# pedropro/UrsoNet

Measured on AMD Instinct MI355X. Metric: images/sec fwd+bwd ResNet50 640x512 bs32/GPU, higher is better.
Workload: dtype bf16; 1 GPU; resnet50 bottleneck=32 ori_resolution=16 soft-class head + loc regression, batch 32/GPU x 512x640x3, full training step (prep+fwd+loss+bwd+clip+SGD); global_batch=32, parallelism=dp1, comm_cus=0, hipgraph=True, runner=Engine, input=uint8 frames in HBM, mean subtraction + cast in the step (molding kernel), gradient_norm_from_finalisation_blocks=True, weight_gradients_on_forked_stream=True

## Files before the change

### ursonet_amd/csrc/common.h

```cpp
#pragma once
#include <hip/hip_runtime.h>
#include <stdint.h>
#include <stdio.h>
#include "../../include/ursonet_hip.h"

typedef __attribute__((ext_vector_type(8))) __bf16 bf16x8_t;
typedef __attribute__((ext_vector_type(8))) _Float16 f16x8_t;
typedef __attribute__((ext_vector_type(4))) float f32x4_t;
typedef __attribute__((ext_vector_type(4))) int i32x4_t;
typedef __attribute__((ext_vector_type(2))) int i32x2_t;

void urso_set_error(const char* fmt, ...);
int  urso_check_launch(const char* what);

#define URSO_OPTION_TABLE(X) \
    X(pw_kernel, 3)         \
    X(pw_small, 5)          \
    X(wgrad_narrow, 1)      \
    X(wgrad_blocks, 512)    \
    X(wgrad_pipe, 1)        \
    X(wgrad_big, 1)         \
    X(wgrad_ring, 0)        \
    X(grid_cap, 0)          \
    X(hconv, 1)             \
    X(pair, 1)              \
    X(pair_single, 3)       \
    X(c3, 1)                \
    X(c3v, 1)               \
    X(stem, 1)              \
    X(stem_pool, 1)         \
    X(cus, 0)               \
    X(hconv2, 1)            \
    X(hconv2_shape, 0)      \
    X(hconv_streamk, 1)     \
    X(hconv_dbg, 0)         \
    X(hwgrad, 1)            \
    X(dense, 1)             \
    X(pwx, 1)               \
    X(pwx_dbg, 0)           \
    X(pwx_bn, 0)            \
    X(mold_scalar, 0)       \
    X(bneck, 3)
struct UrsoOptions {
#define URSO_OPT_FIELD(name, dflt) int name = dflt;
    URSO_OPTION_TABLE(URSO_OPT_FIELD)
#undef URSO_OPT_FIELD
};
extern UrsoOptions g_urso_opt;
int urso_device_cus();
int urso_usable_cus();

#define URSO_FUSE_REDUCE_MAX 16
static __host__ __device__ inline bool urso_fuse_reduce(int splits) { return splits > 1 && splits <= URSO_FUSE_REDUCE_MAX; }

#define URSO_REDUCE_COLS 256
static __host__ __device__ inline int urso_reduce_lanes(int splits) { return splits > 384 ? 16 : (splits > 192 ? 8 : (splits > 96 ? 4 : (splits > 48 ? 2 : 1))); }

void urso_prof_before(hipStream_t s, int kernel_id, double flops, double bytes);
void urso_prof_after(hipStream_t s);

void urso_prof_l2(double l2_bytes);
void urso_prof_symbol(const void* host_fn);
#define URSO_KLAUNCH(kern, grid, blk, shm, st, ...) do { urso_prof_symbol((const void*)(kern)); hipLaunchKernelGGL(kern, grid, blk, shm, st, ##__VA_ARGS__); } while (0)

struct ProfScope {
    hipStream_t s;
    ProfScope(hipStream_t st, int id, double flops, double bytes) : s(st) { urso_prof_before(s, id, flops, bytes); }
    ~ProfScope() { urso_prof_after(s); }
};

static inline size_t dt_size(int dt) { return dt == URSO_F32 ? 4 : 2; }
static __host__ __device__ inline int ceil_div(int a, int b) { return (a + b - 1) / b; }

template <typename T> struct Elem;
template <> struct Elem<float> {
    static constexpr int VE = 4;
    static __device__ __forceinline__ float to_f(float v) { return v; }
    static __device__ __forceinline__ float from_f(float v) { return v; }
};
template <> struct Elem<__bf16> {
    static constexpr int VE = 8;
    static constexpr int ONES = 0x3F803F80;
    static __device__ __forceinline__ float to_f(__bf16 v) { return (float)v; }
    static __device__ __forceinline__ __bf16 from_f(float v) { return (__bf16)v; }
};
template <> struct Elem<_Float16> {
    static constexpr int VE = 8;
    static constexpr int ONES = 0x3C003C00;
    static __device__ __forceinline__ float to_f(_Float16 v) { return (float)v; }
    static __device__ __forceinline__ _Float16 from_f(float v) { return (_Float16)v; }
};

template <typename T> struct Mma;
template <> struct Mma<__bf16> {
// ... 80 lines not shown
```

### ursonet_amd/csrc/conv_c3.hip

```cpp
#include "lds_mfma.h"
#include "internal.h"
#include <utility>

struct C3Args {
    const void* src; const void* wgt; const float* bias; const void* mask; void* dst;
    uint32_t bytes;
    int B, H, W, tiles_x, tiles_y, ntiles;
    int relu;
};

constexpr int C3_TH = 4, C3_TW = 32, C3_HW = C3_TW + 2, C3_HROWS = (C3_TH + 2) * C3_HW;
constexpr int C3_NA = 7;
constexpr int C3_ABUF = 224 * 128, C3_OOFF = 2 * C3_ABUF, C3_BOFF = C3_OOFF + C3_TH * C3_TW * 128, C3_LDS = C3_BOFF + 256;

__device__ __forceinline__ uint32_t c3_rd(int row, int h, int j) {
    const int s = (row >> 1) & 7;
    return (uint32_t)(row * 128 + ((((2 * j + h) ^ s)) << 4));
}

template <typename T, bool MASK>
__global__ __launch_bounds__(256, 2) void c3_kernel(const C3Args a) {
    static_assert(sizeof(T) == 2, "16-bit element types only");
    __shared__ __attribute__((aligned(1024))) char smem[C3_LDS];
    const uint32_t lds0 = (uint32_t)(uintptr_t)(__attribute__((address_space(3))) char*)smem;
    const int tid = threadIdx.x, lane = tid & 63, wave = __builtin_amdgcn_readfirstlane(tid >> 6);
    const int cw = wave & 1, pw = wave >> 1;
    int l31 = lane & 31;
    const int h = lane >> 5;

    const UrsoTileStream ts = urso_tile_stream(a.ntiles);
    const int t_end = ts.t_end, bpx = ts.bpx;
    int tile = ts.tile;
    if (tile >= t_end) return;

    const i32x4_t rs = raw_rsrc(a.src, a.bytes);
    const __amdgpu_buffer_rsrc_t rds = make_rsrc(a.dst, a.bytes);
    const __amdgpu_buffer_rsrc_t rmk = make_rsrc(MASK ? a.mask : a.dst, MASK ? a.bytes : 0u);

    int lane_d = lane;
    auto tile_origin = [&](int t, int& b, int& y0, int& x0) {
        const int tx = t % a.tiles_x, q = t / a.tiles_x;
        const int ty = q % a.tiles_y;
        b = q / a.tiles_y; y0 = ty * C3_TH; x0 = tx * C3_TW;
    };
    auto dma_tile = [&](int t, int buf) {
        int b, y0, x0;
        tile_origin(t, b, y0, x0);
        const int base = ((b * a.H + y0 - 1) * a.W + x0 - 1) * 128;
        asm volatile("" : "+v"(lane_d));
#pragma unroll
        for (int i = 0; i < C3_NA; ++i) {
            const int hr = 8 * (wave + 4 * i) + (lane_d >> 3);
            const int hy = (hr * 241) >> 13, hx = hr - hy * C3_HW;
            const int y = y0 - 1 + hy, x = x0 - 1 + hx;
            const bool ok = hr < C3_HROWS && y >= 0 && y < a.H && x >= 0 && x < a.W;
            const uint32_t off = (uint32_t)(base + (hy * a.W + hx) * 128 + (((lane_d & 7) ^ ((hx >> 1) & 7)) << 4));
            lds_dma16(rs, lds0 + buf * C3_ABUF + (wave + 4 * i) * 1024, ok ? off : URSO_OOB_SHIFT);
        }
    };

    i32x4_t wfr[9][4];
    {
        const int lg = 16 * ((l31 >> 2) & 1) + 4 * (l31 >> 3) + (l31 & 3);
        const char* wrow = (const char*)a.wgt + (size_t)(32 * cw + lg) * (9 * 64 * 2);
#pragma unroll
        for (int t = 0; t < 9; ++t)
#pragma unroll
            for (int j = 0; j < 4; ++j) wfr[t][j] = *(const i32x4_t*)(wrow + (t * 64 + 16 * j + 8 * h) * 2);
    }
    if (tid < 64) *(float*)(smem + C3_BOFF + tid * 4) = a.bias ? a.bias[tid] : 0.f;

    constexpr int NST = 4;
    uint32_t ea[3];
#pragma unroll
    for (int kx = 0; kx < 3; ++kx) ea[kx] = (uint32_t)(l31 * 128 + ((h ^ (((l31 + kx) >> 1) & 7)) << 4));

    dma_tile(tile, 0);
    int buf = 0;
    bool first = true;
    while (true) {
        const bool has_next = tile + bpx < t_end;
        if (first) wait_vm<0>(); else wait_vm<NST>();
        first = false;
        lds_barrier_asm();
        if (has_next) dma_tile(tile + bpx, buf ^ 1);

        f32x16_t acc[2];
        {
            const f32x4_t* bp = (const f32x4_t*)(smem + C3_BOFF + (32 * cw + 16 * h) * 4);
#pragma unroll
            for (int q = 0; q < 4; ++q) {
                const f32x4_t b4 = bp[q];
#pragma unroll
                for (int r = 0; r < 2; ++r) { acc[r][4 * q] = b4.x; acc[r][4 * q + 1] = b4.y; acc[r][4 * q + 2] = b4.z; acc[r][4 * q + 3] = b4.w; }
            }
        }
        i32x4_t f[4];
        uint32_t eb[3];
#pragma unroll
        for (int kx = 0; kx < 3; ++kx) eb[kx] = ea[kx] + (uint32_t)(buf * C3_ABUF + 2 * pw * C3_HW * 128);
        auto rd = [&](i32x4_t& fs, int s) {
            const int hr = s / 12, kx = (s / 4) % 3, j = s & 3;
            if (j == 0) asm volatile("" : "+v"(eb[kx]));
            fs = *(const i32x4_t*)(smem + (hr * C3_HW + kx) * 128 + (eb[kx] ^ (uint32_t)(j << 5)));
        };
        rd(f[0], 0);
        rd(f[1], 1);
        rd(f[2], 2);
#pragma unroll
        for (int s = 0; s < 48; ++s) {
            if (s + 3 < 48) rd(f[(s + 3) & 3], s + 3);
            __builtin_amdgcn_sched_barrier(0);
            const int hr = s / 12, kx = (s / 4) % 3, j = s & 3;
            if (hr <= 2) Mma32<T>::run(wfr[3 * hr + kx][j], f[s & 3], acc[0]);
            if (hr >= 1) Mma32<T>::run(wfr[3 * (hr - 1) + kx][j], f[s & 3], acc[1]);
            __builtin_amdgcn_sched_barrier(0);
        }

        char* sO = smem + C3_OOFF;
#pragma unroll
        for (int r = 0; r < 2; ++r) {
            const int px = (2 * pw + r) * 32 + l31;
#pragma unroll
            for (int v = 0; v < 2; ++v) {
                T o[8];
#pragma unroll
                for (int e = 0; e < 8; ++e) { float y = acc[r][8 * v + e]; y = a.relu ? fmaxf(y, 0.f) : y; o[e] = Elem<T>::from_f(y); }
                i32x4_t ov; __builtin_memcpy(&ov, o, 16);
                *(i32x4_t*)(sO + px * 128 + (((4 * cw + 2 * h + v) ^ ((px >> 1) & 7)) << 4)) = ov;
            }
        }
        int b, y0, x0;
        tile_origin(tile, b, y0, x0);
        uint32_t so[NST];
        i32x4_t mv[NST];
#pragma unroll
        for (int i = 0; i < NST; ++i) {
            const int row = 8 * (wave + 4 * i) + (lane >> 3);
            const int y = y0 + (row >> 5), x = x0 + (row & 31);
            so[i] = (y < a.H && x < a.W) ? (uint32_t)(((b * a.H + y) * a.W + x) * 128 + (((lane & 7) ^ ((row >> 1) & 7)) << 4)) : URSO_OOB_SHIFT;
            if constexpr (MASK) mv[i] = buf_load16(rmk, so[i]);
        }
        lds_barrier_asm();
#pragma unroll
        for (int i = 0; i < NST; ++i) {
            i32x4_t v = *(const i32x4_t*)(sO + (wave + 4 * i) * 1024 + lane * 16);
            if constexpr (MASK) {
                T x[8], m[8];
                __builtin_memcpy(x, &v, 16); __builtin_memcpy(m, &mv[i], 16);
#pragma unroll
                for (int e = 0; e < 8; ++e) x[e] = Elem<T>::to_f(m[e]) > 0.f ? x[e] : Elem<T>::from_f(0.f);
                __builtin_memcpy(&v, x, 16);
            }
            buf_store16(rds, so[i], v);
        }
        if (!has_next) break;
        tile += bpx; buf ^= 1;
    }
}

constexpr int C3W_PATCH = 2 * C3_ABUF;
constexpr int C3W_EOFF = 2 * C3W_PATCH, C3W_BOFF = C3W_EOFF + 8192, C3W_LDS = C3W_BOFF + 512;
constexpr int C3W_NA = 7;

template <typename T, bool MASK, int TW>
__global__ __launch_bounds__(512, 2) void c3w_kernel(const C3Args a) {
    constexpr int TH = 128 / TW, HW = TW + 2, HROWS = (TH + 2) * HW;
    static_assert(TW == 32 || TW == 16, "tile width");
    static_assert(sizeof(T) == 2, "16-bit element types only");
    __shared__ __attribute__((aligned(1024))) char smem[C3W_LDS];
    const uint32_t lds0 = (uint32_t)(uintptr_t)(__attribute__((address_space(3))) char*)smem;
    const int tid = threadIdx.x, lane = tid & 63, wave = __builtin_amdgcn_readfirstlane(tid >> 6);
    const int fq = wave & 3, ch = wave >> 2;
    int l31 = lane & 31;
    const int h = lane >> 5;

    const UrsoTileStream ts = urso_tile_stream(a.ntiles);
    const int t_end = ts.t_end, bpx = ts.bpx;
    int tile = ts.tile;
    if (tile >= t_end) return;

    const i32x4_t rs = raw_rsrc(a.src, a.bytes);
    const __amdgpu_buffer_rsrc_t rds = make_rsrc(a.dst, a.bytes);
    const __amdgpu_buffer_rsrc_t rmk = make_rsrc(MASK ? a.mask : a.dst, MASK ? a.bytes : 0u);

    int lane_d = lane;
    auto tile_origin = [&](int t, int& b, int& y0, int& x0) {
        const int tx = t % a.tiles_x, q = t / a.tiles_x;
        const int ty = q % a.tiles_y;
        b = q / a.tiles_y; y0 = ty * TH; x0 = tx * TW;
    };
    auto dma_tile = [&](int t, int buf) {
        int b, y0, x0;
        tile_origin(t, b, y0, x0);
        const int base = ((b * a.H + y0 - 1) * a.W + x0 - 1) * 256;
        asm volatile("" : "+v"(lane_d));
#pragma unroll
        for (int i = 0; i < C3W_NA; ++i) {
            const int ii = wave + 8 * i, half = ii >= 26 ? 1 : 0, rb = ii - 26 * half;
            const int hr = 8 * rb + (lane_d >> 3);
            const int hy = TW == 32 ? ((hr * 241) >> 13) : ((hr * 3641) >> 16), hx = hr - hy * HW;
            const int y = y0 - 1 + hy, x = x0 - 1 + hx;
            const bool ok = ii < 52 && hr < HROWS && y >= 0 && y < a.H && x >= 0 && x < a.W;
            const int sw = (hx >> 1) & 7;
            const uint32_t off = (uint32_t)(base + (hy * a.W + hx) * 256 + half * 128 + (((lane_d & 7) ^ sw) << 4));
            if (ii < 54) lds_dma16(rs, lds0 + buf * C3W_PATCH + half * C3_ABUF + rb * 1024, ok ? off : URSO_OOB_SHIFT);
        }
    };

    i32x4_t wfr[9][4];
    {
        const int lg = 16 * ((l31 >> 2) & 1) + 4 * (l31 >> 3) + (l31 & 3);
        const char* wrow = (const char*)a.wgt + (size_t)(32 * fq + lg) * (9 * 128 * 2);
#pragma unroll
        for (int t = 0; t < 9; ++t)
#pragma unroll
            for (int j = 0; j < 4; ++j) wfr[t][j] = *(const i32x4_t*)(wrow + (t * 128 + 64 * ch + 16 * j + 8 * h) * 2);
    }
    if (tid < 128) *(float*)(smem + C3W_BOFF + tid * 4) = a.bias ? a.bias[tid] : 0.f;

    constexpr int NST = 4;
    uint32_t ea[3];
    {
        const int prow = TW == 32 ? l31 : (l31 >> 4) * HW + (l31 & 15);
#pragma unroll
        for (int kx = 0; kx < 3; ++kx) ea[kx] = (uint32_t)(prow * 128 + ((h ^ ((((l31 & (TW - 1)) + kx) >> 1) & 7)) << 4));
    }
    dma_tile(tile, 0);
    int buf = 0;
    bool first = true;
    while (true) {
        const bool has_next = tile + bpx < t_end;
        if (first) wait_vm<0>(); else wait_vm<NST>();
        first = false;
        lds_barrier_asm();
        if (has_next) dma_tile(tile + bpx, buf ^ 1);
        f32x16_t acc[4];
// ... 99 lines not shown
        for (int i = 0; i < NST; ++i) {
            const int p = (wave + 8 * i) * 64 + lane, px = p >> 4;
            const int y = y0 + px / TW, x = x0 + px % TW;
            so[i] = (y < a.H && x < a.W) ? (uint32_t)(((b * a.H + y) * a.W + x) * 256 + (((p & 15) ^ (px & 15)) << 4)) : URSO_OOB_SHIFT;
            if constexpr (MASK) mv[i] = buf_load16(rmk, so[i]);
        }
        lds_barrier_asm();
#pragma unroll
        for (int i = 0; i < NST; ++i) {
            i32x4_t v = *(const i32x4_t*)(sO + (wave + 8 * i) * 1024 + lane * 16);
            if constexpr (MASK) {
                T x[8], m[8];
                __builtin_memcpy(x, &v, 16); __builtin_memcpy(m, &mv[i], 16);
#pragma unroll
                for (int e = 0; e < 8; ++e) x[e] = Elem<T>::to_f(m[e]) > 0.f ? x[e] : Elem<T>::from_f(0.f);
                __builtin_memcpy(&v, x, 16);
            }
            buf_store16(rds, so[i], v);
        }
        if (!has_next) break;
        tile += bpx; buf ^= 1;
    }
}


#ifdef C3V_OLD_SWZ
__device__ __forceinline__ uint32_t c3v_swz(int col) { return (uint32_t)(col & 15); }
#else
__device__ __forceinline__ uint32_t c3v_swz(int col) { return (uint32_t)(0xfe64dcba98643210ull >> (4 * (col & 15))) & 15u; }
#endif
constexpr int C3V_HW = 18, C3V_HPIX = 10 * C3V_HW, C3V_PATCH = C3V_HPIX * 256;
constexpr int C3V_NA = 6;
#ifndef C3V_PF
#define C3V_PF 3
#endif
#ifndef C3V_DBG
#define C3V_DBG 0
#endif
#ifdef C3V_SEQ
__host__ __device__ constexpr int c3v_step(int t) { return t; }
#else
__host__ __device__ constexpr int c3v_step(int t) { return (t >> 1) + (t & 1) * 60; }
#endif
#ifdef C3V_NOSB
#define C3V_SB() do {} while (0)
#else
#define C3V_SB() __builtin_amdgcn_sched_barrier(0)
#endif
constexpr int C3V_OOFF = 2 * C3V_PATCH, C3V_BOFF = C3V_OOFF + 2 * 128 * 256, C3V_LDS = C3V_BOFF + 512;

template <class F, int... I> __device__ __forceinline__ void c3_static_for_impl(F&& f, std::integer_sequence<int, I...>) { (f(std::integral_constant<int, I>{}), ...); }
template <int N, class F> __device__ __forceinline__ void c3_static_for(F&& f) { c3_static_for_impl(static_cast<F&&>(f), std::make_integer_sequence<int, N>{}); }

template <typename T, bool MASK>
__global__ __launch_bounds__(512, 2) void c3v_kernel(const C3Args a) {
    static_assert(sizeof(T) == 2, "16-bit element types only");
    __shared__ __attribute__((aligned(1024))) char smem[C3V_LDS];
    const uint32_t lds0 = (uint32_t)(uintptr_t)(__attribute__((address_space(3))) char*)smem;
    const int tid = threadIdx.x, lane = tid & 63, wave = __builtin_amdgcn_readfirstlane(tid >> 6);
    const int fr = lane & 15, fg = lane >> 4;

    const UrsoTileStream ts = urso_tile_stream(a.ntiles);
    const int t_end = ts.t_end, bpx = ts.bpx;
    int tile = ts.tile;
    if (tile >= t_end) return;

    const i32x4_t rs = raw_rsrc(a.src, a.bytes);
    const __amdgpu_buffer_rsrc_t rds = make_rsrc(a.dst, a.bytes);
    const __amdgpu_buffer_rsrc_t rmk = make_rsrc(MASK ? a.mask : a.dst, MASK ? a.bytes : 0u);

    int lane_d = lane;
    auto tile_origin = [&](int t, int& b, int& y0, int& x0) {
        const int tx = t % a.tiles_x, q = t / a.tiles_x;
        const int ty = q % a.tiles_y;
        b = q / a.tiles_y; y0 = ty * 8; x0 = tx * 16;
    };
    auto dma_tile = [&](int t, int buf) {
        int b, y0, x0;
        tile_origin(t, b, y0, x0);
        const int base = ((b * a.H + y0 - 1) * a.W + x0 - 1) * 256;
        asm volatile("" : "+v"(lane_d));
#pragma unroll
        for (int i = 0; i < C3V_NA; ++i) {
            const int ii = wave + 8 * i;
            const int hp = 4 * ii + (lane_d >> 4);
            const int hy = (hp * 3641) >> 16, hx = hp - hy * C3V_HW;
            const int y = y0 - 1 + hy, x = x0 - 1 + hx;
            const bool ok = ii < 45 && y >= 0 && y < a.H && x >= 0 && x < a.W;
            const uint32_t off = (uint32_t)(base + (hy * a.W + hx) * 256 + (((uint32_t)(lane_d & 15) ^ c3v_swz(hx)) << 4));
            if (ii < 45) lds_dma16(rs, lds0 + buf * C3V_PATCH + ii * 1024, ok ? off : URSO_OOB_SHIFT);
        }
    };

    i32x4_t wfr[9][4];
    {
        const char* wrow = (const char*)a.wgt + (size_t)(16 * wave + fr) * (9 * 128 * 2);
#pragma unroll
        for (int t = 0; t < 9; ++t)
#pragma unroll
            for (int j = 0; j < 4; ++j) wfr[t][j] = *(const i32x4_t*)(wrow + (t * 128 + 32 * j + 8 * fg) * 2);
    }
    if (tid < 128) *(float*)(smem + C3V_BOFF + tid * 4) = a.bias ? a.bias[tid] : 0.f;

    uint32_t ea[3];
#pragma unroll
    for (int kx = 0; kx < 3; ++kx) ea[kx] = (uint32_t)((fr + kx) * 256) + (((uint32_t)fg ^ c3v_swz(fr + kx)) << 4);
    constexpr int NST = 4;
    uint32_t so[NST] = {URSO_OOB_SHIFT, URSO_OOB_SHIFT, URSO_OOB_SHIFT, URSO_OOB_SHIFT};
    i32x4_t mv[NST];
    auto flush = [&](int ob) {
        const char* sO = smem + C3V_OOFF + ob * (128 * 256);
#pragma unroll
        for (int i = 0; i < NST; ++i) {
            i32x4_t v = *(const i32x4_t*)(sO + (wave + 8 * i) * 1024 + lane * 16);
            if constexpr (MASK) {
                T x[8], m[8];
                __builtin_memcpy(x, &v, 16); __builtin_memcpy(m, &mv[i], 16);
#pragma unroll
                for (int e = 0; e < 8; ++e) x[e] = Elem<T>::to_f(m[e]) > 0.f ? x[e] : Elem<T>::from_f(0.f);
                __builtin_memcpy(&v, x, 16);
            }
            buf_store16(rds, so[i], v);
        }
    };
    dma_tile(tile, 0);
    int buf = 0, ob = 0;
    bool pend = false;
    while (true) {
        const bool has_next = tile + bpx < t_end;
        wait_vm<0>();
        lds_barrier_asm();
        if (has_next) dma_tile(tile + bpx, buf ^ 1);
        if (pend) flush(ob ^ 1);
        f32x4_t acc[8];
#pragma unroll
        for (int r = 0; r < 8; ++r) acc[r] = f32x4_t{0.f, 0.f, 0.f, 0.f};
        uint32_t eb[3];
#pragma unroll
        for (int kx = 0; kx < 3; ++kx) eb[kx] = ea[kx] + (uint32_t)(buf * C3V_PATCH);
        constexpr int PF = C3V_PF, RING = PF + 1;
        i32x4_t f[RING];
        auto rd = [&](i32x4_t& fs, int s) {
            const int hr = s / 12, kx = (s / 4) % 3, j = s & 3;
            if ((s & 3) == 0) asm volatile("" : "+v"(eb[kx]));
            if (!(C3V_DBG & 2) || s < PF) fs = *(const i32x4_t*)(smem + hr * C3V_HW * 256 + (eb[kx] ^ (uint32_t)(j << 6)));
        };
#pragma unroll
        for (int t = 0; t < PF; ++t) rd(f[t], c3v_step(t));
        c3_static_for<120>([&](auto sc) {
            constexpr int t = decltype(sc)::value, s = c3v_step(t);
            if constexpr (t + PF < 120) rd(f[(t + PF) % RING], c3v_step(t + PF));
            C3V_SB();
            constexpr int hr = s / 12, kx = (s / 4) % 3, j = s & 3;
            if (!(C3V_DBG & 1)) {
                if constexpr (hr >= 0 && hr < 8) Mma<T>::run(wfr[kx][j], f[t % RING], acc[hr]);
                if constexpr (hr - 1 >= 0 && hr - 1 < 8) Mma<T>::run(wfr[3 + kx][j], f[t % RING], acc[hr - 1]);
                if constexpr (hr - 2 >= 0 && hr - 2 < 8) Mma<T>::run(wfr[6 + kx][j], f[t % RING], acc[hr - 2]);
            }
            C3V_SB();
        });
        if (C3V_DBG & 4) { if (!has_next) break; tile += bpx; buf ^= 1; continue; }

        {
            char* sO = smem + C3V_OOFF + ob * (128 * 256);
            const f32x4_t bq = *(const f32x4_t*)(smem + C3V_BOFF + (16 * wave + 4 * fg) * 4);
#pragma unroll
            for (int r = 0; r < 8; ++r) {
                const int px = 16 * r + fr;
                float y0v = acc[r].x + bq.x, y1v = acc[r].y + bq.y, y2v = acc[r].z + bq.z, y3v = acc[r].w + bq.w;
                if (a.relu) { y0v = fmaxf(y0v, 0.f); y1v = fmaxf(y1v, 0.f); y2v = fmaxf(y2v, 0.f); y3v = fmaxf(y3v, 0.f); }
                T o[4] = {Elem<T>::from_f(y0v), Elem<T>::from_f(y1v), Elem<T>::from_f(y2v), Elem<T>::from_f(y3v)};
                i32x2_t ov; __builtin_memcpy(&ov, o, 8);
                *(i32x2_t*)(sO + px * 256 + ((((2 * wave + (fg >> 1)) ^ (px & 15))) << 4) + (fg & 1) * 8) = ov;
            }
        }
        {
            int b, y0, x0;
            tile_origin(tile, b, y0, x0);
#pragma unroll
            for (int i = 0; i < NST; ++i) {
                const int p = (wave + 8 * i) * 64 + lane, px = p >> 4;
                const int y = y0 + (px >> 4), x = x0 + (px & 15);
                so[i] = (y < a.H && x < a.W) ? (uint32_t)(((b * a.H + y) * a.W + x) * 256 + (((p & 15) ^ (px & 15)) << 4)) : URSO_OOB_SHIFT;
                if constexpr (MASK) mv[i] = buf_load16(rmk, so[i]);
            }
        }
        pend = true;
        if (!has_next) break;
        tile += bpx; buf ^= 1; ob ^= 1;
    }
    if constexpr (MASK) wait_vm<0>();
    lds_barrier_asm();
    flush(ob);
}

static int c3w_util(int H, int W, int tw) {
    const int th = 128 / tw;
    return (int)((long long)H * W * 100 / ((long long)ceil_div(H, th) * th * ceil_div(W, tw) * tw));
}
static int c3w_best_tw(int H, int W) { return c3w_util(H, W, 16) > c3w_util(H, W, 32) ? 16 : 32; }

bool urso_c3_fits(const urso_conv_geom* g, int dt, int flags, const void* add) {
    if (!g_urso_opt.c3 || add || (dt != URSO_BF16 && dt != URSO_F16) || (flags & (URSO_EPI_OUT_F32 | URSO_EPI_MASK_BITS | URSO_EPI_EMIT_BITS))) return false;
    if (g->KH != 3 || g->KW != 3 || g->SH != 1 || g->SW != 1 || g->PH != 1 || g->PW != 1 || g->DH != 1 || g->DW != 1 || g->FH > 0) return false;
    if (!((g->C == 64 && g->N == 64) || (g->C == 128 && g->N == 128 && (g_urso_opt.c3 == 1 || g_urso_opt.c3 == 3))) || g->OH != g->H || g->OW != g->W) return false;
    if (g->C == 128 && g_urso_opt.c3 == 1) {
        if (c3w_util(g->H, g->W, c3w_best_tw(g->H, g->W)) < 88) return false;
    }
    return (long long)g->B * g->H * g->W * g->C * 2 < 0x7FFFFF00ll;
}

int urso_c3_launch(const urso_conv_geom* g, int dt, int relu, const void* src, const void* wgt, const float* bias, const void* mask,
                   void* dst, hipStream_t st) {
    C3Args a;
    a.src = src; a.wgt = wgt; a.bias = bias; a.mask = mask; a.dst = dst; a.relu = relu;
    a.B = g->B; a.H = g->H; a.W = g->W;
    a.bytes = (uint32_t)((size_t)g->B * g->H * g->W * g->C * 2);
    const bool wide = g->C == 128;
    const int tw = wide ? c3w_best_tw(g->H, g->W) : C3_TW, th = 128 / tw;
    a.tiles_x = ceil_div(g->W, tw); a.tiles_y = ceil_div(g->H, th); a.ntiles = g->B * a.tiles_y * a.tiles_x;
    const dim3 grid(urso_persistent_grid(a.ntiles, wide ? 1 : 2)), blk(wide ? 512 : 256);
    if (wide) {
#define URSO_C3W(TT, TWV) do { if (mask) URSO_KLAUNCH((c3w_kernel<TT, true, TWV>), grid, blk, 0, st, a); \
                               else URSO_KLAUNCH((c3w_kernel<TT, false, TWV>), grid, blk, 0, st, a); } while (0)
        if (tw == 16 && g_urso_opt.c3v) {
            if (dt == URSO_BF16) { if (mask) URSO_KLAUNCH((c3v_kernel<__bf16, true>), grid, blk, 0, st, a); else URSO_KLAUNCH((c3v_kernel<__bf16, false>), grid, blk, 0, st, a); }
            else { if (mask) URSO_KLAUNCH((c3v_kernel<_Float16, true>), grid, blk, 0, st, a); else URSO_KLAUNCH((c3v_kernel<_Float16, false>), grid, blk, 0, st, a); }
            return urso_check_launch("urso_conv_igemm(3x3, 128 channels, 16-filter waves)");
        }
        if (dt == URSO_BF16) { if (tw == 32) URSO_C3W(__bf16, 32); else URSO_C3W(__bf16, 16); }
        else { if (tw == 32) URSO_C3W(_Float16, 32); else URSO_C3W(_Float16, 16); }
#undef URSO_C3W
        return urso_check_launch("urso_conv_igemm(3x3, 128 channels)");
    }
    if (dt == URSO_BF16) {
        if (mask) URSO_KLAUNCH((c3_kernel<__bf16, true>), grid, blk, 0, st, a);
        else URSO_KLAUNCH((c3_kernel<__bf16, false>), grid, blk, 0, st, a);
    } else {
        if (mask) URSO_KLAUNCH((c3_kernel<_Float16, true>), grid, blk, 0, st, a);
        else URSO_KLAUNCH((c3_kernel<_Float16, false>), grid, blk, 0, st, a);
    }
    return urso_check_launch("urso_conv_igemm(3x3, 64 channels)");
}
```

### ursonet_amd/csrc/conv_halo.hip

```cpp
#include "lds_mfma.h"
#include "internal.h"

struct HcArgs {
    const void* src; const void* wgt; const float* bias; const void* add; const void* mask; void* dst;
    uint32_t src_bytes, wgt_bytes, dst_bytes;
    int H, W, C, N;
    int Vw, Vh, Mv;
    int nchunks;
    int tilesN, ntiles;
    int R, JA;
    int krow;
    float rcp_vw, rcp_vh;
    int relu;
    int dbg;
    int units;
    unsigned int* flags;
    float* part;
};

constexpr int HC_BM = 256, HC_BN = 128, HC_BSLOT = HC_BN * 128, HC_AROWS = 424, HC_ABUF = HC_AROWS * 128;
constexpr int HC_AOFF = 3 * HC_BSLOT, HC_XOFF = HC_AOFF + 2 * HC_ABUF, HC_LDS = 163840, HC_MAXN = (HC_LDS - HC_XOFF) / 4;
constexpr int HC_SC = 17;
constexpr int HC_NST = 8;

// ... 251 lines not shown
                        *(i32x4_t*)(smem + sbase + l31 * 128 + (((4 * j + 2 * hf + h) ^ ((l31 >> 1) & 7)) << 4)) = ov;
                    }
                i32x4_t ov[4], mv[4];
                uint32_t so[4];
#pragma unroll
                for (int q = 0; q < 4; ++q) {
                    const int row = 8 * q + r8;
                    ov[q] = *(const i32x4_t*)(smem + sbase + row * 128 + ((c8 ^ ((row >> 1) & 7)) << 4));
                    const bool ok = vb * a.Vh * a.Vw + vy * a.Vw + vx < a.Mv && vx < a.W && vy < a.H;
                    so[q] = ok ? (uint32_t)((vb * a.H + vy) * a.W + vx) * (uint32_t)a.N * 2u + (uint32_t)(n0 + 64 * wn + 8 * c8) * 2u : URSO_OOB_SHIFT;
                    if (a.mask) mv[q] = buf_load16(rmk, so[q]);
                    vx += 8;
                    if (vx >= a.Vw) { vx -= a.Vw; if (++vy == a.Vh) { vy = 0; ++vb; } }
                }
#pragma unroll
                for (int q = 0; q < 4; ++q) {
                    if (a.mask) {
                        T ev[8], em[8];
                        __builtin_memcpy(ev, &ov[q], 16); __builtin_memcpy(em, &mv[q], 16);
#pragma unroll
                        for (int e = 0; e < 8; ++e) ev[e] = (Elem<T>::to_f(em[e]) > 0.f) ? ev[e] : Elem<T>::from_f(0.f);
                        __builtin_memcpy(&ov[q], ev, 16);
                    }
                    buf_store16(rds, so[q], ov[q]);
                }
            }
        }
        if (!has_next) break;
        gcur += cend - cbeg;
        ++tile;
    }
}

bool urso_hconv_fits(const urso_conv_geom* g, int dt, int flags, const void* add) {
    if (!g_urso_opt.hconv || dt == URSO_F32 || add) return false;
    if (flags & (URSO_EPI_OUT_F32 | URSO_EPI_MASK_BITS | URSO_EPI_EMIT_BITS)) return false;
    if (g->KH != 3 || g->KW != 3 || g->SH != 1 || g->SW != 1 || g->PH != 1 || g->PW != 1 || g->DH != 1 || g->DW != 1) return false;
    if (g->OH != g->H || g->OW != g->W || g->FH > 0) return false;
    if (g->C % 128 || g->N % HC_BN || g->N > HC_MAXN) return false;
    if (HC_BM + 2 * (g->W + 2) > HC_AROWS || g->W + 1 < 8) return false;
    if ((size_t)g->B * (g->H + 1) * (g->W + 1) >= (1u << 24)) return false;
    if (urso_hconv2_pick(g, true)) return true;
    if (g_urso_opt.hconv == 1) {
        const int ntiles = ceil_div(g->B * (g->H + 1) * (g->W + 1), HC_BM) * (g->N / HC_BN), ncu = urso_usable_cus();
        const int blocks = ntiles < ncu ? ntiles : ncu, rounds = ceil_div(ntiles, blocks);
        if (ntiles * 20 < blocks * rounds * 13 && !(ntiles <= ncu && ntiles * 3 >= ncu * 2)) return false;
    }
    return true;
}

size_t urso_hconv_ws_bytes() { return 4096 + (size_t)urso_device_cus() * 512 * 64 * sizeof(float); }

int urso_hconv_launch(const urso_conv_geom* g, int dt, int relu, const void* src, const void* wgt, const float* bias, const void* add,
                      const void* mask, void* dst, uint32_t src_bytes, uint32_t wgt_bytes, uint32_t dst_bytes, void* ws, size_t ws_bytes,
                      hipStream_t st) {
    (void)add;
    {
        const int r2 = urso_hconv2_try_launch(g, dt, relu, src, wgt, bias, mask, dst, src_bytes, wgt_bytes, dst_bytes, ws,
                                              ws && ws_bytes >= urso_hconv_ws_bytes(), st);
        if (r2 != 0) return r2 > 0 ? URSO_OK : r2;
    }
    HcArgs a;
    a.src = src; a.wgt = wgt; a.bias = bias; a.add = add; a.mask = mask; a.dst = dst;
    a.src_bytes = src_bytes; a.wgt_bytes = wgt_bytes; a.dst_bytes = dst_bytes;
    a.H = g->H; a.W = g->W; a.C = g->C; a.N = g->N;
    a.Vw = g->W + 1; a.Vh = g->H + 1; a.Mv = g->B * a.Vh * a.Vw;
    a.nchunks = g->C / 64;
    a.tilesN = g->N / HC_BN; a.ntiles = ceil_div(a.Mv, HC_BM) * a.tilesN;
    a.R = HC_BM + 2 * (a.Vw + 1); a.JA = ceil_div(a.R, 64);
    a.krow = 9 * g->C * 2;
    a.rcp_vw = 1.0f / (float)a.Vw; a.rcp_vh = 1.0f / (float)a.Vh;
    a.relu = relu; a.dbg = g_urso_opt.hconv_dbg;
    dim3 grid(urso_persistent_grid(a.ntiles, 1)); const dim3 blk(512);
    int G = (int)grid.x;
    if (ws && ws_bytes >= urso_hconv_ws_bytes() && !(a.dbg & 4) && g_urso_opt.hconv_streamk && g_urso_opt.grid_cap <= 0 && G < urso_usable_cus()) {
        int G2 = urso_usable_cus(); const int units = a.ntiles * a.nchunks;
        if (G2 > units) G2 = units;
        G2 = G2 / 8 * 8;
        if (G2 > G && G2 <= 1024 && ceil_div(units, G2) < ceil_div(a.ntiles, G) * a.nchunks) { G = G2; grid = dim3(G2); }
    }
    const bool can = ws && ws_bytes >= urso_hconv_ws_bytes() && G <= urso_usable_cus() && G <= 1024 && !(a.dbg & 4) && g_urso_opt.hconv_streamk;
    const bool streamk = can && ((a.dbg & 8) || ceil_div(a.ntiles * a.nchunks, G) < ceil_div(a.ntiles, G) * a.nchunks);
    a.flags = streamk ? (unsigned int*)ws : nullptr;
    a.part = streamk ? (float*)((char*)ws + 4096) : nullptr;
    a.units = streamk ? a.ntiles * a.nchunks : a.ntiles;
    urso_prof_l2((double)a.ntiles * a.nchunks * (9.0 * HC_BSLOT + (double)a.R * 128));
    if (a.dbg & 16) {
        if (dt == URSO_BF16) URSO_KLAUNCH((hconv_kernel<__bf16, 4>), grid, blk, 0, st, a);
        else URSO_KLAUNCH((hconv_kernel<_Float16, 4>), grid, blk, 0, st, a);
    } else {
        if (dt == URSO_BF16) URSO_KLAUNCH((hconv_kernel<__bf16, 8>), grid, blk, 0, st, a);
        else URSO_KLAUNCH((hconv_kernel<_Float16, 8>), grid, blk, 0, st, a);
    }
    return urso_check_launch("urso_conv_igemm(halo)");
}
```

### ursonet_amd/csrc/conv_halo2.hip

```cpp
#include "lds_mfma.h"
#include "internal.h"
#include <type_traits>
#ifndef URSO_HX2_NS1
#define URSO_HX2_NS1 4
#endif

struct Hx2Args {
    const void* src; const void* wgt; const float* bias; const void* mask; void* dst;
    uint32_t src_bytes, wgt_bytes, dst_bytes;
    int H, W, C, N;
    int Vw, Vh, Mv;
    int nchunks;
    int tilesN, ntiles;
    int R, JA;
    int abuf;
    int krow;
    float rcp_vw, rcp_vh;
    int relu;
    unsigned long long* clk;
    int dbg;
};

constexpr int HX_LDS = 163840;
constexpr int HX_ABUF1 = 61440, HX_FOFF = 2 * HX_ABUF1;

template <typename T, int MI, int NJ, int PROBE = 0>
__global__ __launch_bounds__(512, 2) void hconv2_kernel(const Hx2Args a) {
    static_assert(sizeof(T) == 2, "16-bit element types only");
#ifndef URSO_HX2_NS1
#define URSO_HX2_NS1 4
#endif
    constexpr int NS = (NJ == 1) ? URSO_HX2_NS1 : 2;
    constexpr int BM = 128 * MI, BN = 64 * NJ, BSLOT = BN * 128, XOFF = HX_FOFF + NS * BSLOT;
    constexpr int NQ = NJ;
    constexpr int LPR = 4 * NJ, RPI = 64 / LPR, NSI = 32 / RPI;
    constexpr int NST = MI * NSI;
    __shared__ __attribute__((aligned(1024))) char smem[HX_LDS];
    const uint32_t lds0 = (uint32_t)(uintptr_t)(__attribute__((address_space(3))) char*)smem;


    const int tid = threadIdx.x, lane = tid & 63, wave = __builtin_amdgcn_readfirstlane(tid >> 6);
    const int wm = wave & 3, wn = wave >> 2;
    const int l31 = lane & 31, h = lane >> 5, c8 = lane & 7, r8 = lane >> 3;

    const int G = gridDim.x, lid = (blockIdx.x & 7) * (G >> 3) + (blockIdx.x >> 3);
    const int t_begin = (int)(((long long)lid * a.ntiles) / G), t_end = (int)(((long long)(lid + 1) * a.ntiles) / G);
    if (t_begin >= t_end || (a.dbg & 1024)) return;

    const i32x4_t rs = raw_rsrc(a.src, a.src_bytes), rw = raw_rsrc(a.wgt, a.wgt_bytes);
    const __amdgpu_buffer_rsrc_t rmk = make_rsrc(a.mask ? a.mask : a.dst, a.mask ? a.dst_bytes : 0u);
    const __amdgpu_buffer_rsrc_t rds = make_rsrc(a.dst, a.dst_bytes);

    if (tid * 4 < a.N) {
        f32x4_t b = f32x4_t{0.f, 0.f, 0.f, 0.f};
        if (a.bias) b = *(const f32x4_t*)(a.bias + tid * 4);
        *(f32x4_t*)(smem + XOFF + tid * 16) = b;
    }

    uint32_t fb, pb[9];
    fb = HX_FOFF + halo_rd(32 * NJ * wn + l31, h);
#pragma unroll
    for (int t = 0; t < 9; ++t) pb[t] = halo_rd(32 * MI * wm + l31 + (t / 3) * a.Vw + (t % 3), h);

    uint32_t bsrc0[NQ];
#pragma unroll
    for (int q = 0; q < NQ; ++q) {
        const int Rr = 8 * (wave + 8 * q) + r8;
        const int nl = (Rr & ~31) + halo_perm(Rr & 31);
        bsrc0[q] = (uint32_t)nl * (uint32_t)a.krow + (uint32_t)((c8 ^ ((Rr >> 1) & 7)) << 4);
    }

    auto divmod = [](int n, int d, float rcp, int& q, int& r) {
        q = (int)((float)n * rcp);
        r = n - q * d;
        const bool lo = r < 0, hi = r >= d;
        q += hi ? 1 : (lo ? -1 : 0);
        r += hi ? -d : (lo ? d : 0);
    };
    auto real_pixel = [&](int p) -> int {
        const bool in = p >= 0 && p < a.Mv;
        int q1, x, b, y;
        divmod(in ? p : 0, a.Vw, a.rcp_vw, q1, x);
        divmod(q1, a.Vh, a.rcp_vh, b, y);
        return (in && x < a.W && y < a.H) ? (b * a.H + y) * a.W + x : -1;
    };

    const uint32_t TOFF = XOFF + (uint32_t)a.N * 4u;
    auto fill_table = [&](int tile_, int which) {
        const int p0_ = (tile_ / a.tilesN) * BM;
        const int pix = (tid < a.R) ? real_pixel(p0_ - (a.Vw + 1) + tid) : -1;
        *(uint32_t*)(smem + TOFF + which * 2048 + tid * 4) = (pix >= 0) ? (uint32_t)pix * (uint32_t)(a.C * 2) : URSO_OOB_SHIFT;
    };
    const uint32_t aswz = (uint32_t)((c8 ^ ((4 * wave + (r8 >> 1)) & 7)) << 4);
    auto table_entry = [&](int which, int j) -> uint32_t {
        return *(const uint32_t*)(smem + TOFF + which * 2048 + (8 * (wave + 8 * j) + r8) * 4);
    };
    auto dma_a = [&](int j, int cc, int buf, uint32_t rowoff) {
        if (8 * (wave + 8 * j) < a.R)
            lds_dma16_sgpr(rs, lds0 + buf * HX_ABUF1 + (wave + 8 * j) * 1024, rowoff + aswz + (uint32_t)cc * 128u);
    };
    auto dma_b = [&](int n0_, int cc, int t, int slot) {
        const uint32_t koff = (uint32_t)n0_ * (uint32_t)a.krow + (uint32_t)(t * a.C + cc * 64) * 2u;
#pragma unroll
// ... 90 lines not shown
                if constexpr (NS == 2) {
                    if (t == 0 && first_wait_after_epilogue) asm volatile("s_waitcnt vmcnt(%0) lgkmcnt(0)" :: "n"(NST) : "memory");
                    else asm volatile("s_waitcnt vmcnt(0) lgkmcnt(0)" ::: "memory");
                } else {
                    static_assert(NQ == 1, "the four-slot ring is the NJ = 1 form");
                    if (t < 3 && first_wait_after_epilogue) asm volatile("s_waitcnt vmcnt(%0) lgkmcnt(0)" :: "n"(NST + 2) : "memory");
                    else if (t >= 6 && !more_a) { if (t == 6) asm volatile("s_waitcnt vmcnt(1) lgkmcnt(0)" ::: "memory"); else asm volatile("s_waitcnt vmcnt(0) lgkmcnt(0)" ::: "memory"); }
                    else asm volatile("s_waitcnt vmcnt(2) lgkmcnt(0)" ::: "memory");
                }
                if (!(a.dbg & 64)) asm volatile("s_barrier" ::: "memory");
                if (!(a.dbg & 32)) {
                    if constexpr (NS == 2) {
                        if (t < 8 && t < a.JA && more_a) dma_a(t, cca, par ^ 1, acur0);
                        if (t < 7) acur0 = table_entry(tw, t + 1);
                    } else {
                        if (t < 6 && more_a) {
                            const int j0 = piece(t, 0), j1 = piece(t, 1);
                            if (j0 < a.JA) dma_a(j0, cca, par ^ 1, acur0);
                            if (j1 < a.JA) dma_a(j1, cca, par ^ 1, acur1);
                        }
                        if (t < 5) { acur0 = table_entry(tw, min(piece(t + 1, 0), 7)); acur1 = table_entry(tw, min(piece(t + 1, 1), 7)); }
                    }
                    const int t2 = (t + NS) % 9;
                    const bool wrap = t + NS >= 9;
                    const bool okb = !wrap || more_a;
                    if (okb) dma_b((wrap && last) ? n0n : n0, wrap ? cca : cc, t2, (S + sb) & (NS - 1));
                }
                __builtin_amdgcn_sched_barrier(0);
                if (t < 8) rd(fwA, fpA, S1, par, t + 1, 0);
                else rd(fwA, fpA, S1, par ^ 1, 0, 0);
                region_end(); mma(fwB, fpB); region_end();
            }
        };
        if (!(a.dbg & 2))
            for (int cc = 0; cc < a.nchunks; cc += 2) {
                chunk(std::integral_constant<int, 0>{}, cc);
                chunk(std::integral_constant<int, 1>{}, cc + 1);
                if constexpr (NS == 4) { sb ^= 2; set_fbs(); }
            }

        stores_pending = false;
        if (!(a.dbg & 1)) {
            stores_pending = true;
            int lane_e = lane;
            asm volatile("" : "+v"(lane_e));
            const int cl = lane_e % LPR, rl = lane_e / LPR, l31e = lane_e & 31, he = lane_e >> 5;
            const uint32_t sbase = HX_ABUF1 + wave * (32 * 64 * NJ);
            int vx, vy, vb;
            {
                int q1;
                divmod(p0 + 32 * MI * wm + rl, a.Vw, a.rcp_vw, q1, vx);
                divmod(q1, a.Vh, a.rcp_vh, vb, vy);
            }
#pragma unroll
            for (int i = 0; i < MI; ++i) {
#pragma unroll
                for (int j = 0; j < NJ; ++j)
#pragma unroll
                    for (int hf = 0; hf < 2; ++hf) {
                        const int nb = n0 + 32 * NJ * wn + 32 * j + 16 * hf + 8 * he;
                        const f32x4_t b0 = *(const f32x4_t*)(smem + XOFF + nb * 4), b1 = *(const f32x4_t*)(smem + XOFF + nb * 4 + 16);
                        const float bv[8] = {b0.x, b0.y, b0.z, b0.w, b1.x, b1.y, b1.z, b1.w};
                        T eo[8];
#pragma unroll
                        for (int e = 0; e < 8; ++e) {
                            float y = acc[i][j][8 * hf + e] + bv[e];
                            y = a.relu ? fmaxf(y, 0.f) : y;
                            eo[e] = Elem<T>::from_f(y);
                        }
                        i32x4_t ov; __builtin_memcpy(&ov, eo, 16);
                        *(i32x4_t*)(smem + sbase + l31e * (64 * NJ) + (((4 * j + 2 * hf + he) ^ ((l31e >> 1) & (LPR - 1))) << 4)) = ov;
                    }
                i32x4_t ov[NSI], mv[NSI];
                uint32_t so[NSI];
#pragma unroll
                for (int q = 0; q < NSI; ++q) {
                    const int row = RPI * q + rl;
                    ov[q] = *(const i32x4_t*)(smem + sbase + row * (64 * NJ) + ((cl ^ ((row >> 1) & (LPR - 1))) << 4));
                    const bool ok = vb * a.Vh * a.Vw + vy * a.Vw + vx < a.Mv && vx < a.W && vy < a.H;
                    so[q] = ok ? (uint32_t)((vb * a.H + vy) * a.W + vx) * (uint32_t)a.N * 2u + (uint32_t)(n0 + 32 * NJ * wn + 8 * cl) * 2u : URSO_OOB_SHIFT;
                    if (a.mask) mv[q] = buf_load16(rmk, so[q]);
                    vx += RPI;
                    if (vx >= a.Vw) { vx -= a.Vw; if (++vy == a.Vh) { vy = 0; ++vb; } }
                }
#pragma unroll
                for (int q = 0; q < NSI; ++q) {
                    if (a.mask) {
                        T ev[8], em[8];
                        __builtin_memcpy(ev, &ov[q], 16); __builtin_memcpy(em, &mv[q], 16);
#pragma unroll
                        for (int e = 0; e < 8; ++e) ev[e] = (Elem<T>::to_f(em[e]) > 0.f) ? ev[e] : Elem<T>::from_f(0.f);
                        __builtin_memcpy(&ov[q], ev, 16);
                    }
                    buf_store16(rds, so[q], ov[q]);
                }
            }
        }
        if (!has_next) break;
        ++tile;
    }
    if (a.clk && tid == 0) {
        a.clk[2 * lid] = __builtin_readcyclecounter() - clk0;
        a.clk[2 * lid + 1] = __builtin_amdgcn_s_memrealtime() - rt0;
    }
}

struct Hx2Shape { int mi, nj; };
static const Hx2Shape HX2_SHAPES[] = {{3, 2}, {3, 1}, {2, 2}, {2, 1}, {1, 2}, {1, 1}};

static size_t hx2_abuf(int R, int nj) { const size_t a = (size_t)ceil_div(R, 8) * 1024, e = (size_t)8 * 32 * 64 * nj; return a > e ? a : e; }

static bool hx2_shape_fits(const urso_conv_geom* g, int mi, int nj) {
    const int BM = 128 * mi, BN = 64 * nj, Vw = g->W + 1;
    if (g->N % BN) return false;
    const int R = BM + 2 * (Vw + 1), JA = ceil_div(R, 64);
    if (JA > 8) return false;
    if (Vw < 64 / (4 * nj)) return false;
    if (hx2_abuf(R, nj) > (size_t)HX_ABUF1) return false;
    if (R > 512) return false;
    return (size_t)HX_FOFF + (size_t)(nj == 1 ? URSO_HX2_NS1 : 2) * BN * 128 + (size_t)g->N * 4 + 2 * 2048 <= (size_t)HX_LDS;
}

static double hx2_cost(const urso_conv_geom* g, int mi, int nj, int ncu) {
    const int Mv = g->B * (g->H + 1) * (g->W + 1);
    const int tiles = ceil_div(Mv, 128 * mi) * (g->N / (64 * nj));
    const int blocks = tiles < ncu ? tiles : ncu, rounds = ceil_div(tiles, blocks);
    const double kib = (128.0 * nj * 64.0 + (128.0 * mi + 2.0 * (g->W + 2)) * 128.0 / 9.0) / 1024.0;
    const double step = (0.037 * 4.0 * mi * nj + 0.07 + 0.003 * kib) * (0.7 + 0.3 * (double)blocks / ncu);
    return 9.0 + rounds * (g->C / 64) * 9.0 * step + (rounds - 1) * 3.0;
}
static double hx2_cost_halo1(const urso_conv_geom* g, int ncu, bool streamk) {
    const int Mv = g->B * (g->H + 1) * (g->W + 1), tiles = ceil_div(Mv, 256) * (g->N / 128), nch = g->C / 64;
    const int blocks = tiles < ncu ? tiles : ncu;
    double c = 14.0 + ceil_div(tiles, blocks) * nch * 9.0 * 0.75;
    if (streamk) { const double sk = 20.0 + ceil_div(tiles * nch, ncu) * 9.0 * 0.75; if (sk < c) c = sk; }
    return c;
}

int urso_hconv2_pick(const urso_conv_geom* g, bool has_ws) {
    if (!g_urso_opt.hconv2 || g->C % 128) return 0;
    const int ncu = urso_usable_cus();
    int best = -1; double best_cost = 1e30;
    for (int s = 0; s < (int)(sizeof(HX2_SHAPES) / sizeof(HX2_SHAPES[0])); ++s) {
        const int mi = HX2_SHAPES[s].mi, nj = HX2_SHAPES[s].nj;
        if (g_urso_opt.hconv2_shape && g_urso_opt.hconv2_shape != 10 * mi + nj) continue;
        if (!hx2_shape_fits(g, mi, nj)) continue;
        const double c = hx2_cost(g, mi, nj, ncu);
        if (c < best_cost) { best_cost = c; best = s; }
    }
    if (best < 0) return 0;
    if (g_urso_opt.hconv2 == 1 && !g_urso_opt.hconv2_shape && best_cost >= hx2_cost_halo1(g, ncu, has_ws && g_urso_opt.hconv_streamk)) return 0;
    return 10 * HX2_SHAPES[best].mi + HX2_SHAPES[best].nj;
}

int urso_hconv2_try_launch(const urso_conv_geom* g, int dt, int relu, const void* src, const void* wgt, const float* bias, const void* mask,
                           void* dst, uint32_t src_bytes, uint32_t wgt_bytes, uint32_t dst_bytes, void* ws, bool has_ws, hipStream_t st) {
    const int shape = urso_hconv2_pick(g, has_ws);
    if (!shape) return 0;
    const int mi = shape / 10, nj = shape % 10;
    Hx2Args a;
    a.src = src; a.wgt = wgt; a.bias = bias; a.mask = mask; a.dst = dst;
    a.src_bytes = src_bytes; a.wgt_bytes = wgt_bytes; a.dst_bytes = dst_bytes;
    a.H = g->H; a.W = g->W; a.C = g->C; a.N = g->N;
    a.Vw = g->W + 1; a.Vh = g->H + 1; a.Mv = g->B * a.Vh * a.Vw;
    a.nchunks = g->C / 64;
    a.tilesN = g->N / (64 * nj); a.ntiles = ceil_div(a.Mv, 128 * mi) * a.tilesN;
    a.R = 128 * mi + 2 * (a.Vw + 1); a.JA = ceil_div(a.R, 64); a.abuf = (int)hx2_abuf(a.R, nj);
    a.krow = 9 * g->C * 2;
    a.rcp_vw = 1.0f / (float)a.Vw; a.rcp_vh = 1.0f / (float)a.Vh;
    a.relu = relu; a.dbg = g_urso_opt.hconv_dbg;
    a.clk = (ws && has_ws && (a.dbg & 2048)) ? (unsigned long long*)((char*)ws + 8192) : nullptr;
    const dim3 grid(urso_persistent_grid(a.ntiles, 1)), blk(512);
    urso_prof_l2((double)a.ntiles * a.nchunks * (9.0 * 64 * nj * 128 + (double)a.R * 128));
#define HX2_GO(MI_, NJ_) do { if (dt == URSO_BF16) URSO_KLAUNCH((hconv2_kernel<__bf16, MI_, NJ_>), grid, blk, 0, st, a); \
                              else URSO_KLAUNCH((hconv2_kernel<_Float16, MI_, NJ_>), grid, blk, 0, st, a); } while (0)
    if (10 * mi + nj == 32 && dt == URSO_BF16 && (a.dbg & 384)) {
        if (a.dbg & 128) URSO_KLAUNCH((hconv2_kernel<__bf16, 3, 2, 1>), grid, blk, 0, st, a);
        else URSO_KLAUNCH((hconv2_kernel<__bf16, 3, 2, 2>), grid, blk, 0, st, a);
        return urso_check_launch("urso_conv_igemm(halo2 probe)") == URSO_OK ? 1 : URSO_EINVAL;
    }
    switch (10 * mi + nj) {
        case 32: HX2_GO(3, 2); break; case 31: HX2_GO(3, 1); break;
        case 22: HX2_GO(2, 2); break; case 21: HX2_GO(2, 1); break;
        case 12: HX2_GO(1, 2); break; case 11: HX2_GO(1, 1); break;
        default: return 0;
    }
#undef HX2_GO
    const int rc = urso_check_launch("urso_conv_igemm(halo2)");
    return rc == URSO_OK ? 1 : rc;
}
```

### ursonet_amd/csrc/conv_igemm.hip

```cpp
#include "common.h"
#include "internal.h"
#include <stdlib.h>

struct IgemmArgs {
    const void* src; const void* wgt; const float* bias; const void* add; const void* mask; void* dst;
    uint32_t src_bytes, wgt_bytes, dst_bytes;
    int B, H, W, C, OH, OW, N, KH, KW, SH, SW, PH, PW, DHs, DWs;
    int M;
    int Cc;
    int Kc;
    int nkt;
    int tilesN, ntiles;
    int pointwise;
    int FH, FW, OSH, OSW;
    int ksplit, kps;
    float* part;
    int flags;
    void* bits_out;
    uint32_t bits_bytes;
};

template <typename T, int BM, int BN, bool HAS_ADD, int MASK, bool SPLIT, bool EMIT = false>
__global__ __launch_bounds__(256, 2) void igemm_kernel(const IgemmArgs a) {
    constexpr bool HAS_MASK = MASK == 1;
// ... 357 lines not shown
        case 4: if constexpr (sizeof(T) == 2) URSO_IG(BN_, false, 2, false, false); break; \
        case 5: if constexpr (sizeof(T) == 2) URSO_IG(BN_, true, 2, false, false); break; \
        case 8: if constexpr (sizeof(T) == 2) URSO_IG(BN_, false, 0, false, true); break; \
        case 9: if constexpr (sizeof(T) == 2) URSO_IG(BN_, true, 0, false, true); break; \
        default: urso_set_error("urso_conv_igemm: unsupported epilogue combination"); return URSO_EINVAL; }
    if (a.ksplit > 1) { if (small) URSO_IG(64, false, 0, true, false); else URSO_IG(128, false, 0, true, false); }
    else if (small) { URSO_SEL(64) }
    else { URSO_SEL(128) }
#undef URSO_SEL
#undef URSO_IG
    if (a.ksplit > 1) {
        const size_t elems = (size_t)a.M * g->N, n4 = elems / 4;
        int blocks = (int)((n4 + 255) / 256); if (blocks > 2048) blocks = 2048; if (blocks < 1) blocks = 1;
        URSO_KLAUNCH((splitk_finish_kernel<T>), dim3(blocks), dim3(256), 0, st, n4, g->N, a.ksplit, elems, (const float*)a.part, a.bias,
                           (const T*)a.add, (const T*)a.mask, a.dst, flags);
    }
    return urso_check_launch("urso_conv_igemm");
}

extern "C" int urso_conv_igemm_halo_ok(const urso_conv_geom* g, int dt, int flags, int has_add) {
    return (g && urso_hconv_fits(g, dt, flags, has_add ? (const void*)g : nullptr)) ? 1 : 0;
}

extern "C" size_t urso_conv_igemm_halo_ws_bytes(void) { return urso_hconv_ws_bytes(); }

extern "C" int urso_conv_igemm_halo2_shape(const urso_conv_geom* g, int dt, int flags, int has_add, int has_ws) {
    if (!g || !urso_hconv_fits(g, dt, flags, has_add ? (const void*)g : nullptr)) return 0;
    return urso_hconv2_pick(g, has_ws != 0);
}

extern "C" size_t urso_conv_igemm_ws_bytes(const urso_conv_geom* g, int dt) {
    if (!g || g->FH > 0 || (g->N & 3)) return 0;
    const int VE = 16 / (int)dt_size(dt);
    if (g->C % VE) return 0;
    const int M = g->B * g->OH * g->OW, nkt = ceil_div(g->KH * g->KW * (g->C / VE), 8);
    const int bn = (g->N <= 64) ? 64 : 128;
    int S, kps; plan_splitk(ceil_div(M, 128) * ceil_div(g->N, bn), nkt, urso_usable_cus(), S, kps);
    return S > 1 ? (size_t)S * M * g->N * sizeof(float) : 0;
}

extern "C" int urso_conv_igemm(const urso_conv_geom* g, int dt, int flags,
                               const void* src_d, const void* wgt_d, const float* bias_d,
                               const void* add_d, const void* mask_d, void* dst_d, void* stream) {
    return urso_conv_igemm_ws(g, dt, flags, src_d, wgt_d, bias_d, add_d, mask_d, dst_d, nullptr, 0, stream);
}

extern "C" int urso_conv_igemm_ws(const urso_conv_geom* g, int dt, int flags,
                                  const void* src_d, const void* wgt_d, const float* bias_d,
                                  const void* add_d, const void* mask_d, void* dst_d, void* ws_d, size_t ws_bytes, void* stream) {
    return urso_conv_igemm_ex(g, dt, flags & ~(URSO_EPI_MASK_BITS | URSO_EPI_EMIT_BITS), src_d, wgt_d, bias_d, add_d, mask_d, dst_d, nullptr,
                              ws_d, ws_bytes, stream);
}

extern "C" int urso_conv_igemm_bits_ok(const urso_conv_geom* g, int dt, int flags, size_t ws_bytes) {
    if (!g || dt == URSO_F32 || (flags & URSO_EPI_OUT_F32) || (g->N % 8) || (g->C % 8)) return 0;
    if (ws_bytes && urso_conv_igemm_ws_bytes(g, dt)) return 0;
    return 1;
}

extern "C" int urso_conv_igemm_algorithmic(const urso_conv_geom* g, int dt, int flags, int has_add, int has_mask, double* flops_out, double* bytes_out) {
    if (!g || (dt != URSO_F32 && dt != URSO_BF16 && dt != URSO_F16)) { urso_set_error("urso_conv_igemm_algorithmic: bad argument"); return URSO_EINVAL; }
    const double es = (double)dt_size(dt);
    const double M = (double)g->B * g->OH * g->OW;
    double flops = 2.0 * M * (double)g->N * g->KH * g->KW * g->C;
    if (g->DH > 1 || g->DW > 1) flops /= (double)(g->DH * g->DW);
    if (g->C == 8 && g->KH == 7 && g->KW == 4 && g->SH == 2) flops *= 147.0 / 224.0;
    const double src_bytes = (double)g->B * g->H * g->W * g->C * es, wgt_bytes = (double)g->N * g->KH * g->KW * g->C * es;
    const double src_alg = (g->KH == 1 && g->KW == 1 && (g->SH > 1 || g->SW > 1)) ? M * g->C * es : src_bytes;
    const double wr_elems = M * g->N;
    const double bytes = src_alg + wgt_bytes + wr_elems * ((flags & URSO_EPI_OUT_F32) ? 4 : es) +
                         (has_add ? wr_elems * es : 0) + (has_mask ? ((flags & URSO_EPI_MASK_BITS) ? wr_elems / 8 : wr_elems * es) : 0) +
                         ((flags & URSO_EPI_EMIT_BITS) ? wr_elems / 8 : 0);
    if (flops_out) *flops_out = flops;
    if (bytes_out) *bytes_out = bytes;
    return URSO_OK;
}

extern "C" int urso_conv_igemm_ex(const urso_conv_geom* g, int dt, int flags,
                                  const void* src_d, const void* wgt_d, const float* bias_d,
                                  const void* add_d, const void* mask_d, void* dst_d, void* bits_out_d,
                                  void* ws_d, size_t ws_bytes, void* stream) {
    if (!g || !src_d || !wgt_d || !dst_d) { urso_set_error("urso_conv_igemm: null argument"); return URSO_EINVAL; }
    if (dt != URSO_F32 && dt != URSO_BF16 && dt != URSO_F16) { urso_set_error("urso_conv_igemm: bad dtype %d", dt); return URSO_EINVAL; }
    const size_t es = dt_size(dt);
    const int VE = 16 / (int)es;
    if (g->B <= 0 || g->H <= 0 || g->W <= 0 || g->C <= 0 || g->OH <= 0 || g->OW <= 0 || g->N <= 0 || g->KH <= 0 || g->KW <= 0 ||
        g->SH <= 0 || g->SW <= 0) { urso_set_error("urso_conv_igemm: non-positive dimension"); return URSO_EINVAL; }
    if (g->C % VE) { urso_set_error("urso_conv_igemm: C=%d is not a multiple of %d (16-byte vectors)", g->C, VE); return URSO_EINVAL; }
    int dhs = ilog2_exact(g->DH), dws = ilog2_exact(g->DW);
    if (dhs < 0 || dws < 0) { urso_set_error("urso_conv_igemm: D must be 1, 2 or 4"); return URSO_EINVAL; }
    const size_t src_bytes = (size_t)g->B * g->H * g->W * g->C * es;
    const size_t wgt_bytes = (size_t)g->N * g->KH * g->KW * g->C * es;
    const bool scatter = g->FH > 0;
    if (scatter && (g->FW <= 0 || g->OSH <= 0 || g->OSW <= 0 || (g->OH - 1) * g->OSH >= g->FH || (g->OW - 1) * g->OSW >= g->FW)) {
        urso_set_error("urso_conv_igemm: bad destination scatter"); return URSO_EINVAL; }
    const size_t dst_elems = scatter ? (size_t)g->B * g->FH * g->FW * g->N : (size_t)g->B * g->OH * g->OW * g->N;
    if (src_bytes >= 0x7FFFFF00ull || wgt_bytes >= 0x7FFFFF00ull || dst_elems * ((flags & URSO_EPI_OUT_F32) ? 4 : es) >= 0x7FFFFF00ull) {
        urso_set_error("urso_conv_igemm: tensor exceeds the 2 GiB buffer-addressing limit"); return URSO_EINVAL; }
    IgemmArgs a;
    a.src = src_d; a.wgt = wgt_d; a.bias = bias_d; a.add = add_d; a.mask = mask_d; a.dst = dst_d;
    a.src_bytes = (uint32_t)src_bytes; a.wgt_bytes = (uint32_t)wgt_bytes;
    a.dst_bytes = (uint32_t)(dst_elems * ((flags & URSO_EPI_OUT_F32) ? 4 : es));
    a.B = g->B; a.H = g->H; a.W = g->W; a.C = g->C; a.OH = g->OH; a.OW = g->OW; a.N = g->N;
    a.KH = g->KH; a.KW = g->KW; a.SH = g->SH; a.SW = g->SW; a.PH = g->PH; a.PW = g->PW; a.DHs = dhs; a.DWs = dws;
    a.M = g->B * g->OH * g->OW; a.Cc = g->C / VE; a.Kc = g->KH * g->KW * a.Cc; a.nkt = ceil_div(a.Kc, 8);
    a.flags = flags;
    a.bits_out = bits_out_d; a.bits_bytes = (uint32_t)(dst_elems / 8);
    a.FH = scatter ? g->FH : 0; a.FW = g->FW; a.OSH = g->OSH; a.OSW = g->OSW;
    a.pointwise = (g->KH == 1 && g->KW == 1 && g->SH == 1 && g->SW == 1 && g->PH == 0 && g->PW == 0 && g->DH == 1 && g->DW == 1 &&
                   g->H == g->OH && g->W == g->OW) ? 1 : 0;
    hipStream_t st = (hipStream_t)stream;
    double flops, bytes;
    urso_conv_igemm_algorithmic(g, dt, flags, add_d ? 1 : 0, mask_d ? 1 : 0, &flops, &bytes);
    ProfScope ps(st, URSO_K_IGEMM, flops, bytes);
    if (urso_dense_fits(g, dt, flags, a.pointwise, a.M))
        return urso_dense_launch(g, dt, flags, src_d, wgt_d, bias_d, add_d, mask_d, dst_d, a.src_bytes, a.wgt_bytes, a.dst_bytes, st);
    if (urso_bneck_fwd_fits(g, dt, flags, add_d, mask_d))
        return urso_bneck_fwd_launch(g, dt, flags, src_d, wgt_d, bias_d, dst_d, st);
    if (urso_bneck_dgrad_fits(g, dt, flags, add_d, mask_d))
        return urso_bneck_dgrad_launch(g, dt, flags, src_d, wgt_d, mask_d, dst_d, st);
    {
        const int use_pw = g_urso_opt.pw_kernel;
        const bool halo_layer = dt != URSO_F32 && urso_hconv_fits(g, dt, flags, add_d);
        const bool split = ws_d && !halo_layer && urso_conv_igemm_ws_bytes(g, dt) != 0 && urso_conv_igemm_ws_bytes(g, dt) <= ws_bytes;
        const bool wants_bits = (flags & (URSO_EPI_MASK_BITS | URSO_EPI_EMIT_BITS)) != 0;
        const bool s1x1 = g->KH == 1 && g->KW == 1 && g->PH == 0 && g->PW == 0 && g->DH == 1 && g->DW == 1 && g->FH <= 0;
        const bool add_src = (flags & URSO_EPI_ADD_SRCGRID) != 0;
        if (add_src && (!add_d || !s1x1 || dt == URSO_F32 || mask_d || (flags & (URSO_EPI_OUT_F32 | URSO_EPI_MASK_BITS)) || (a.Cc & 7) || (g->N % 8) ||
                        (g->OH - 1) * g->SH >= g->H || (g->OW - 1) * g->SW >= g->W || use_pw < 2 || (size_t)g->B * g->H * g->W * g->N * es >= 0x7FFFFF00ull)) {
            urso_set_error("urso_conv_igemm: ADD_SRCGRID needs a 16-bit unpadded 1x1 layer with C %% 64 == 0, a residual operand on the input grid and no mask");
            return URSO_EINVAL;
        }
        const bool bits_fit = !wants_bits || ((a.pointwise || (s1x1 && !(flags & URSO_EPI_MASK_BITS) && (a.Cc & 7) == 0)) && !((flags & URSO_EPI_EMIT_BITS) && (mask_d || (g->N % 32))) &&
                                              !((flags & URSO_EPI_MASK_BITS) && (!mask_d || (g->N % 32))) && !((flags & URSO_EPI_EMIT_BITS) && !bits_out_d));
        const bool fits = dt != URSO_F32 && !(flags & URSO_EPI_OUT_F32) && bits_fit && (g->N % 8) == 0 &&
                          !split && (size_t)a.M < (1u << 24);
        if (fits && urso_pair_single_fits(g, dt, flags, add_d, mask_d))
            return urso_pair_single_launch(g, dt, flags, src_d, wgt_d, bias_d, add_d, mask_d, dst_d,
                                           (flags & URSO_EPI_EMIT_BITS) ? bits_out_d : nullptr, st);
        if (fits && urso_c3_fits(g, dt, flags, add_d))
            return urso_c3_launch(g, dt, (flags & URSO_EPI_RELU) ? 1 : 0, src_d, wgt_d, bias_d, mask_d, dst_d, st);
        if (fits && urso_hconv_fits(g, dt, flags, add_d))
            return urso_hconv_launch(g, dt, (flags & URSO_EPI_RELU) ? 1 : 0, src_d, wgt_d, bias_d, add_d, mask_d, dst_d,
                                     a.src_bytes, a.wgt_bytes, a.dst_bytes, ws_d, ws_bytes, st);
        const int mbits = (flags & URSO_EPI_MASK_BITS) ? 1 : 0;
        void* bout = (flags & URSO_EPI_EMIT_BITS) ? bits_out_d : nullptr;
        const bool taps_ok = (a.Cc & 7) == 0 && g->DH == 1 && g->DW == 1 && g->KH <= 3 && g->KW <= 3;
        const bool stem_ok = a.Cc == 1 && g->KW == 4 && g->KH <= 8 && g->DH == 1 && g->DW == 1 && g->N <= 64 && !add_d && !mask_d;
        if (fits && !wants_bits && urso_stem_fits(g, dt, flags, add_d, mask_d))
            return urso_stem_launch(g, dt, (flags & URSO_EPI_RELU) ? 1 : 0, src_d, wgt_d, bias_d, dst_d, st);
        if (fits && !wants_bits && use_pw >= 3 && stem_ok)
            return urso_pw_launch(g, dt, 2, dhs, dws, (flags & URSO_EPI_RELU) ? 1 : 0,
                                  src_d, wgt_d, bias_d, add_d, mask_d, dst_d, a.src_bytes, a.wgt_bytes, a.dst_bytes, 0, nullptr, 0, st);
        if (add_src && !fits) { urso_set_error("urso_conv_igemm: ADD_SRCGRID layer does not fit the DMA kernel (split-K workspace given, M >= 2^24 ...)"); return URSO_EINVAL; }
        if (fits && ((use_pw >= 1 && a.pointwise && (a.Cc & 7) == 0) || (use_pw >= 2 && taps_ok && (!wants_bits || s1x1))))
            return urso_pw_launch(g, dt, a.pointwise ? 0 : 1, dhs, dws, (flags & URSO_EPI_RELU) ? 1 : 0,
                                  src_d, wgt_d, bias_d, add_d, mask_d, dst_d, a.src_bytes, a.wgt_bytes, a.dst_bytes, mbits, bout, add_src, st);
    }
    if (dt == URSO_F32) return launch_igemm<float>(g, flags, a, ws_d, ws_bytes, st);
    if (dt == URSO_BF16) return launch_igemm<__bf16>(g, flags, a, ws_d, ws_bytes, st);
    return launch_igemm<_Float16>(g, flags, a, ws_d, ws_bytes, st);
}
```

### ursonet_amd/csrc/conv_pair.hip

```cpp
#include "lds_mfma.h"
#include "internal.h"

struct PairArgs {
    const void* src; const void* w1; const float* bias1; const void* add; void* bits; void* mid;
    const void* w2; const float* bias2; const void* mask2; void* dst;
    uint32_t nar_bytes, wide_bytes, bits_bytes;
    int ntiles;
    int relu1;
    int sp_h, sp_w; uint32_t add_bytes; float rcp_hw, rcp_w;
    void* cmp; uint32_t cmp_bytes;
    uint32_t wide_pitch, bits_pitch, g_w1, g_bias, g_wide, g_bits;
};

template <int CM_, int NW_, int BM_, int NBUF_, int CW_ = 4 * CM_> struct PairShape {
    static constexpr int CM = CM_, CW = CW_, NW = NW_, BM = BM_, NBUF = NBUF_, D = NBUF_ - 1;
    static constexpr int AROW = CM * 2, RROW = CW * 2, BROW = CW / 8;
    static constexpr int ABUF = BM * AROW, RBUF = BM * RROW, ROFF = NBUF * ABUF, LDS = NBUF * (ABUF + RBUF);
    static constexpr int NA = ABUF / (1024 * NW), NR = RBUF / (1024 * NW);
    static constexpr int PT1 = BM / 32, KS1 = CM / 16, PT2 = BM / 16, KS2 = CW / 32;
    static constexpr int C2T = CW / (32 * NW);
    static_assert((C2T == 1 || C2T == 2) && CW == 32 * C2T * NW && NA >= 1 && NR >= 1 && PT1 >= 1, "wave roles");
    static __device__ __forceinline__ int aswz(int row) { return AROW == 128 ? ((row >> 1) & 7) : (row & 15); }
};
using PairS2 = PairShape<64, 4, 64, 2>;
using PairS3 = PairShape<128, 8, 32, 3>;
using PairS4 = PairShape<256, 8, 32, 3, 512>;
using PairS5 = PairShape<512, 8, 32, 3, 256>;

#ifndef PAIR_DBG
#define PAIR_DBG 0
#endif
template <typename T, int MODE, bool EMIT, typename S, int VAR, bool SPARSE = false>
__global__ __launch_bounds__(S::NW * 64, 2) void pair_kernel(const PairArgs a) {
    static_assert(!SPARSE || (MODE == 1 && VAR == 0) || (MODE == 0 && VAR != 0), "SPARSE: compact add operand of the backward pair, or sampled second output of a single forward layer");
    constexpr bool SPADD = SPARSE && MODE == 1, CMPW = SPARSE && MODE == 0;
    static_assert(sizeof(T) == 2, "16-bit element types only");
    constexpr bool G2 = VAR == 0, HAS_ADD = VAR != 2;
    static_assert(!G2 || (S::CM / S::NW == 16 && S::CW == 4 * S::CM), "pair: every wave owns 16 of the CM output channels of GEMM 2");
    static_assert(VAR != 2 || MODE == 0, "the form without a residual operand is forward-only");
    constexpr int BM = S::BM, CM = S::CM, CW = S::CW, NW = S::NW, AROW = S::AROW, RROW = S::RROW, BROW = S::BROW;
    constexpr int NA = S::NA, NR = S::NR, PT1 = S::PT1, KS1 = S::KS1, PT2 = S::PT2, KS2 = S::KS2, D = S::D, NBUF = S::NBUF, C2T = S::C2T;
    static_assert(!G2 || C2T == 2, "pair: every wave owns 64 of the wide channels");
    __shared__ __attribute__((aligned(1024))) char smem[S::LDS];
    const uint32_t lds0 = (uint32_t)(uintptr_t)(__attribute__((address_space(3))) char*)smem;
    const int tid = threadIdx.x, lane = tid & 63, wave = __builtin_amdgcn_readfirstlane(tid >> 6);
    const int l31 = lane & 31, h = lane >> 5, l15 = lane & 15, g = lane >> 4;

    const UrsoTileStream ts = urso_tile_stream(a.ntiles);
    const int t_end = ts.t_end, bpx = ts.bpx;
    int tile = ts.tile;
    if (tile >= t_end) return;

    const uint32_t grp = blockIdx.y, gwide = grp * a.g_wide, gbits = grp * a.g_bits;
    const uint32_t pitch = a.wide_pitch, bpitch = a.bits_pitch;
    const i32x4_t rs = raw_rsrc(a.src, a.nar_bytes), ra = raw_rsrc((const char*)a.add + gwide, (SPADD ? a.add_bytes : a.wide_bytes) - gwide);
    const __amdgpu_buffer_rsrc_t rmid = make_rsrc((char*)a.mid + gwide, a.wide_bytes - gwide), rdst = make_rsrc(a.dst, a.nar_bytes);
    const __amdgpu_buffer_rsrc_t rbit = make_rsrc(a.bits ? (char*)a.bits + gbits : (char*)a.mid, a.bits ? a.bits_bytes - gbits : 0u);
    const __amdgpu_buffer_rsrc_t rmk2 = make_rsrc(MODE == 1 ? a.mask2 : a.dst, MODE == 1 ? a.nar_bytes : 0u);

    uint32_t aoff[NA], roff[NR];
#pragma unroll
    for (int i = 0; i < NA; ++i) {
        const int row = (1024 / AROW) * (wave + NW * i) + lane / (AROW / 16), p = lane % (AROW / 16);
        aoff[i] = (uint32_t)(row * AROW + ((p ^ S::aswz(row)) << 4));
    }
#pragma unroll
    for (int i = 0; i < NR; ++i) {
        const int row = (1024 / RROW) * (wave + NW * i) + lane / (RROW / 16), p = lane % (RROW / 16);
        roff[i] = (uint32_t)(row * RROW + ((p ^ (row & 15)) << 4));
    }
    uint32_t rgo[NR];
#pragma unroll
    for (int i = 0; i < NR; ++i) rgo[i] = (roff[i] / (uint32_t)RROW) * pitch + (roff[i] & (uint32_t)(RROW - 1));
    auto dma_tile = [&](int t, int buf) {
        const uint32_t nb = (uint32_t)t * (uint32_t)(BM * AROW), wb = (uint32_t)t * (uint32_t)BM * pitch;
#pragma unroll
        for (int i = 0; i < NA; ++i) lds_dma16(rs, lds0 + buf * S::ABUF + (wave + NW * i) * 1024, nb + aoff[i]);
        if constexpr (HAS_ADD && !SPADD) {
#pragma unroll
            for (int i = 0; i < NR; ++i) lds_dma16(ra, lds0 + S::ROFF + buf * S::RBUF + (wave + NW * i) * 1024, (PAIR_DBG & 4) ? URSO_OOB_SHIFT : wb + rgo[i]);
        }
        if constexpr (SPADD) {
            const int hw = a.sp_h * a.sp_w, w2 = a.sp_w >> 1, hw4 = (a.sp_h >> 1) * w2;
#pragma unroll
            for (int i = 0; i < NR; ++i) {
                const int row = (1024 / RROW) * (wave + NW * i) + lane / (RROW / 16);
                const int p = t * BM + row;
                int b = (int)((float)p * a.rcp_hw), rem = p - b * hw;
                { const bool lo = rem < 0, hi = rem >= hw; b += hi ? 1 : (lo ? -1 : 0); rem += hi ? -hw : (lo ? hw : 0); }
                int y = (int)((float)rem * a.rcp_w), x = rem - y * a.sp_w;
                { const bool lo = x < 0, hi = x >= a.sp_w; y += hi ? 1 : (lo ? -1 : 0); x += hi ? -a.sp_w : (lo ? a.sp_w : 0); }
                const uint32_t off = (uint32_t)((b * hw4 + (y >> 1) * w2 + (x >> 1)) * RROW) + (roff[i] & (uint32_t)(RROW - 1));
                lds_dma16(ra, lds0 + S::ROFF + buf * S::RBUF + (wave + NW * i) * 1024, ((y | x) & 1) ? URSO_OOB_SHIFT : off);
            }
        }
    };
    constexpr int NDMA = NA + (HAS_ADD ? NR : 0);

    i32x4_t w1f[C2T][KS1], w2f[KS2];
    {
        const int lg = 16 * ((l31 >> 2) & 1) + 4 * (l31 >> 3) + (l31 & 3);
#pragma unroll
        for (int c2 = 0; c2 < C2T; ++c2)
#pragma unroll
            for (int j = 0; j < KS1; ++j)
                w1f[c2][j] = *(const i32x4_t*)((const char*)a.w1 + (size_t)grp * a.g_w1 + ((size_t)(32 * C2T * wave + 32 * c2 + lg) * CM + 16 * j + 8 * h) * 2);
        if constexpr (G2) {
#pragma unroll
            for (int j = 0; j < KS2; ++j)
                w2f[j] = *(const i32x4_t*)((const char*)a.w2 + ((size_t)(16 * wave + l15) * CW + 32 * j + 8 * g) * 2);
        }
    }
    float b1[C2T][16], b2[4];
    if constexpr (MODE == 0) {
#pragma unroll
        for (int c2 = 0; c2 < C2T; ++c2)
#pragma unroll
            for (int r = 0; r < 16; ++r) b1[c2][r] = a.bias1 ? a.bias1[grp * a.g_bias + 32 * C2T * wave + 32 * c2 + 16 * h + r] : 0.f;
        if constexpr (G2) {
#pragma unroll
            for (int r = 0; r < 4; ++r) b2[r] = a.bias2 ? a.bias2[16 * wave + 4 * g + r] : 0.f;
        }
    }

    uint32_t g1rd[PT1][2];
#pragma unroll
    for (int pt = 0; pt < PT1; ++pt) {
        const int row = 32 * pt + l31;
        g1rd[pt][0] = (uint32_t)(row * AROW);
        g1rd[pt][1] = (uint32_t)S::aswz(row);
    }
    uint32_t e1[PT1][C2T];
#pragma unroll
    for (int pt = 0; pt < PT1; ++pt)
#pragma unroll
        for (int c2 = 0; c2 < C2T; ++c2)
            e1[pt][c2] = (uint32_t)((32 * pt + l31) * RROW + (((4 * C2T * wave + 4 * c2 + 2 * h) ^ (l31 & 15)) << 4));
    uint32_t g2rd[PT2];
#pragma unroll
    for (int pt = 0; pt < PT2; ++pt) g2rd[pt] = (uint32_t)((16 * pt + l15) * RROW + ((g ^ l15) << 4));
    uint32_t e2[PT2];
#pragma unroll
    for (int pt = 0; pt < PT2; ++pt) {
        const int row = 16 * pt + l15, slot = 2 * wave + (g >> 1);
        e2[pt] = (uint32_t)(row * AROW + ((slot ^ S::aswz(row)) << 4) + 8 * (g & 1));
    }
    const uint32_t bitoff = (uint32_t)l31 * bpitch + 4u * C2T * wave;

    constexpr int NST = NR + (G2 ? NA : 0) + ((MODE == 0 && EMIT) ? PT1 : 0) + (CMPW ? NR : 0);

    i32x2_t pbits[PT1];
    i32x4_t pm2[NA];
    auto prefetch = [&](int t) {
        if constexpr (MODE == 1) {
#pragma unroll
            for (int pt = 0; pt < PT1; ++pt)
            {
                const uint32_t bo = (uint32_t)t * (uint32_t)BM * bpitch + pt * 32u * bpitch + bitoff;
                if constexpr (C2T == 2) pbits[pt] = __builtin_bit_cast(i32x2_t, __builtin_amdgcn_raw_buffer_load_b64(rbit, bo, 0, 0));
                else pbits[pt] = i32x2_t{(int)__builtin_amdgcn_raw_buffer_load_b32(rbit, bo, 0, 0), 0};
            }
            if constexpr (G2) {
#pragma unroll
                for (int i = 0; i < NA; ++i) pm2[i] = buf_load16(rmk2, (uint32_t)t * (uint32_t)(BM * AROW) + aoff[i]);
            }
        }
    };

    prefetch(tile);
    dma_tile(tile, 0);
    if constexpr (D == 2) { if (tile + bpx < t_end) dma_tile(tile + bpx, 1); }
    int buf = 0;
    bool first = true;
    while (true) {
        const bool has_next = tile + bpx < t_end;
        const bool has_far = tile + D * bpx < t_end;
        if constexpr (D == 1) { if (first) wait_vm<0>(); else wait_vm<NST>(); }
        else {
            if (first) { if (has_next) wait_vm<NDMA>(); else wait_vm<0>(); }
            else { if (has_next) wait_vm<NST + NDMA>(); else wait_vm<NST>(); }
        }
        first = false;
        lds_barrier_asm();
        i32x2_t cbits[PT1]; i32x4_t cm2[NA];
        if constexpr (MODE == 1) {
#pragma unroll
            for (int i = 0; i < PT1; ++i) { cbits[i] = pbits[i]; asm volatile("" : "+v"(cbits[i])); }
            if constexpr (G2) {
#pragma unroll
                for (int i = 0; i < NA; ++i) { cm2[i] = pm2[i]; asm volatile("" : "+v"(cm2[i])); }
            }
        }
        if (has_next) prefetch(tile + bpx);
        if (has_far) { int nb_ = buf + D; if (nb_ >= NBUF) nb_ -= NBUF; dma_tile(tile + D * bpx, nb_); }
        const char* sA = smem + buf * S::ABUF;
        char* sR = smem + S::ROFF + buf * S::RBUF;

        f32x16_t acc[PT1][C2T];
#pragma unroll
        for (int pt = 0; pt < PT1; ++pt)
#pragma unroll
            for (int c2 = 0; c2 < C2T; ++c2)
// ... 71 lines not shown
                    { const bool lo = x < 0, hi = x >= a.sp_w; y += hi ? 1 : (lo ? -1 : 0); x += hi ? -a.sp_w : (lo ? a.sp_w : 0); }
                    const uint32_t off = (uint32_t)(b * hw4 + (y >> 1) * w2 + (x >> 1)) * pitch + (roff[i] & (uint32_t)(RROW - 1));
                    buf_store16(rcmp, ((y | x) & 1) ? URSO_OOB_SHIFT : off, v[i]);
                }
            }
        }
        if constexpr (!G2) {
            if (!has_next) break;
            tile += bpx;
            buf = (buf + 1 == NBUF) ? 0 : buf + 1;
            continue;
        }
        f32x4_t acc2[PT2];
#pragma unroll
        for (int pt = 0; pt < PT2; ++pt)
#pragma unroll
            for (int r = 0; r < 4; ++r) acc2[pt][r] = (MODE == 0) ? b2[r] : 0.f;
#pragma unroll
        for (int j = 0; j < KS2; ++j) {
            i32x4_t px[PT2];
#pragma unroll
            for (int pt = 0; pt < PT2; ++pt) px[pt] = *(const i32x4_t*)(sR + (g2rd[pt] ^ (uint32_t)(j << 6)));
#pragma unroll
            for (int pt = 0; pt < PT2; ++pt) Mma<T>::run(w2f[j], px[pt], acc2[pt]);
        }
        char* sO = smem + buf * S::ABUF;
#pragma unroll
        for (int pt = 0; pt < PT2; ++pt) {
            T out[4];
#pragma unroll
            for (int r = 0; r < 4; ++r) {
                float x = acc2[pt][r];
                if constexpr (MODE == 0) x = fmaxf(x, 0.f);
                out[r] = Elem<T>::from_f(x);
            }
            i32x2_t pk;
            __builtin_memcpy(&pk, out, 8);
            *(i32x2_t*)(sO + e2[pt]) = pk;
        }
        lds_barrier_asm();
        {
            const uint32_t nb = (uint32_t)tile * (uint32_t)(BM * AROW);
#pragma unroll
            for (int i = 0; i < NA; ++i) {
                i32x4_t v = *(const i32x4_t*)(sO + (wave + NW * i) * 1024 + lane * 16);
                if constexpr (MODE == 1) {
                    T x[8], m[8];
                    __builtin_memcpy(x, &v, 16); __builtin_memcpy(m, &cm2[i], 16);
#pragma unroll
                    for (int e = 0; e < 8; ++e) x[e] = Elem<T>::to_f(m[e]) > 0.f ? x[e] : Elem<T>::from_f(0.f);
                    __builtin_memcpy(&v, x, 16);
                }
                buf_store16(rdst, nb + aoff[i], v);
            }
        }
        if (!has_next) break;
        tile += bpx;
        buf = (buf + 1 == NBUF) ? 0 : buf + 1;
    }
}

extern "C" int urso_conv_pair_ok(long long M, int dt, int c_narrow, int c_wide) {
    if (M <= 0 || !(dt == URSO_BF16 || dt == URSO_F16) || c_wide != 4 * c_narrow) return 0;
    const int bm = c_narrow == PairS2::CM ? PairS2::BM : (c_narrow == PairS3::CM ? PairS3::BM : 0);
    return (bm && M % bm == 0 && M * c_wide * 2 < 0x7FFFFF00ll) ? 1 : 0;
}

template <typename S, int VAR>
static void pr_launch(const PairArgs& a, int dt, int mode, bool emit, int blocks_per_cu, hipStream_t st, bool sparse = false, int groups = 1) {
    const dim3 grid(urso_persistent_grid(a.ntiles, blocks_per_cu, groups), groups), blk(S::NW * 64);
    if constexpr (VAR == 0) {
        if (sparse && mode == 1) {
            if (dt == URSO_BF16) URSO_KLAUNCH((pair_kernel<__bf16, 1, false, S, 0, true>), grid, blk, 0, st, a);
            else URSO_KLAUNCH((pair_kernel<_Float16, 1, false, S, 0, true>), grid, blk, 0, st, a);
        } else if (dt == URSO_BF16) {
            if (mode == 1) URSO_KLAUNCH((pair_kernel<__bf16, 1, false, S, 0>), grid, blk, 0, st, a);
            else if (emit) URSO_KLAUNCH((pair_kernel<__bf16, 0, true, S, 0>), grid, blk, 0, st, a);
            else URSO_KLAUNCH((pair_kernel<__bf16, 0, false, S, 0>), grid, blk, 0, st, a);
        } else {
            if (mode == 1) URSO_KLAUNCH((pair_kernel<_Float16, 1, false, S, 0>), grid, blk, 0, st, a);
            else if (emit) URSO_KLAUNCH((pair_kernel<_Float16, 0, true, S, 0>), grid, blk, 0, st, a);
            else URSO_KLAUNCH((pair_kernel<_Float16, 0, false, S, 0>), grid, blk, 0, st, a);
        }
    } else {
        if (mode == 1) {
            if constexpr (VAR == 1) {
                if (dt == URSO_BF16) URSO_KLAUNCH((pair_kernel<__bf16, 1, false, S, 1>), grid, blk, 0, st, a);
                else URSO_KLAUNCH((pair_kernel<_Float16, 1, false, S, 1>), grid, blk, 0, st, a);
            }
        } else if (sparse) {
            if (dt == URSO_BF16) { if (emit) URSO_KLAUNCH((pair_kernel<__bf16, 0, true, S, VAR, true>), grid, blk, 0, st, a); else URSO_KLAUNCH((pair_kernel<__bf16, 0, false, S, VAR, true>), grid, blk, 0, st, a); }
            else { if (emit) URSO_KLAUNCH((pair_kernel<_Float16, 0, true, S, VAR, true>), grid, blk, 0, st, a); else URSO_KLAUNCH((pair_kernel<_Float16, 0, false, S, VAR, true>), grid, blk, 0, st, a); }
        } else if (dt == URSO_BF16) {
            if (emit) URSO_KLAUNCH((pair_kernel<__bf16, 0, true, S, VAR>), grid, blk, 0, st, a);
            else URSO_KLAUNCH((pair_kernel<__bf16, 0, false, S, VAR>), grid, blk, 0, st, a);
        } else {
            if (emit) URSO_KLAUNCH((pair_kernel<_Float16, 0, true, S, VAR>), grid, blk, 0, st, a);
            else URSO_KLAUNCH((pair_kernel<_Float16, 0, false, S, VAR>), grid, blk, 0, st, a);
        }
    }
}

bool urso_pair_single_fits(const urso_conv_geom* g, int dt, int flags, const void* add, const void* mask) {
    if (!g_urso_opt.pair || (flags & URSO_EPI_OUT_F32) || (dt != URSO_BF16 && dt != URSO_F16)) return false;
    const bool mbits = (flags & URSO_EPI_MASK_BITS) != 0;
    if (mask && !mbits) return false;
    if (mbits && (!mask || !add || (flags & (URSO_EPI_EMIT_BITS | URSO_EPI_RELU)))) return false;
    if (g->KH != 1 || g->KW != 1 || g->SH != 1 || g->SW != 1 || g->PH || g->PW || g->DH != 1 || g->DW != 1 || g->FH > 0 ||
        g->OH != g->H || g->OW != g->W) return false;
    const long long M = (long long)g->B * g->OH * g->OW;
    if (M <= 0 || M * g->N * 2 >= 0x7FFFFF00ll) return false;
    if (g->C == PairS4::CM) return (g_urso_opt.pair_single & 1) && g->N >= PairS4::CW && g->N % PairS4::CW == 0 && M % PairS4::BM == 0;
    if (g->C == PairS5::CM) return (g_urso_opt.pair_single & 2) && g->N >= PairS5::CW && g->N % PairS5::CW == 0 && M % PairS5::BM == 0;
    if (mbits) return false;
    return g->N == 4 * g->C && urso_conv_pair_ok(M, dt, g->C, g->N) != 0;
}
static int pair_single_launch(const urso_conv_geom* g, int dt, int flags, const void* src, const void* wgt, const float* bias, const void* add,
                              const void* mask_bits, void* dst, void* bits_out, void* dst_sampled, hipStream_t st) {
    const long long M = (long long)g->B * g->OH * g->OW;
    const int cm = g->C, cw = g->N;
    const int mode = (flags & URSO_EPI_MASK_BITS) ? 1 : 0;
    PairArgs a;
    a.src = src; a.w1 = wgt; a.bias1 = bias; a.add = add ? add : dst; a.bits = mode ? const_cast<void*>(mask_bits) : bits_out; a.mid = dst;
    a.w2 = nullptr; a.bias2 = nullptr; a.mask2 = nullptr; a.dst = dst; a.relu1 = (flags & URSO_EPI_RELU) ? 1 : 0;
    a.sp_h = a.sp_w = 0; a.add_bytes = 0; a.rcp_hw = a.rcp_w = 0.f;
    a.nar_bytes = (uint32_t)(M * cm * 2); a.wide_bytes = (uint32_t)(M * cw * 2); a.bits_bytes = (uint32_t)(M * (cw / 8));
    a.wide_pitch = (uint32_t)cw * 2u; a.bits_pitch = (uint32_t)cw / 8u; a.g_w1 = a.g_bias = a.g_wide = a.g_bits = 0;
    const bool emit = !mode && bits_out != nullptr;
    const bool smp = dst_sampled != nullptr;
    a.cmp = dst_sampled; a.cmp_bytes = (uint32_t)(M / 4 * cw * 2);
    if (smp) { a.sp_h = g->OH; a.sp_w = g->OW; a.rcp_hw = 1.0f / (float)(g->OH * g->OW); a.rcp_w = 1.0f / (float)g->OW; }
    if (cm == PairS4::CM) {
        const int groups = cw / PairS4::CW;
        a.g_w1 = (uint32_t)PairS4::CW * cm * 2u; a.g_bias = PairS4::CW; a.g_wide = PairS4::CW * 2u; a.g_bits = PairS4::CW / 8u;
        a.ntiles = (int)(M / PairS4::BM);
        if (add) pr_launch<PairS4, 1>(a, dt, mode, emit, 1, st, smp, groups); else pr_launch<PairS4, 2>(a, dt, 0, emit, 1, st, smp, groups);
    } else if (cm == PairS5::CM) {
        const int groups = cw / PairS5::CW;
        a.g_w1 = (uint32_t)PairS5::CW * cm * 2u; a.g_bias = PairS5::CW; a.g_wide = PairS5::CW * 2u; a.g_bits = PairS5::CW / 8u;
        a.ntiles = (int)(M / PairS5::BM);
        if (add) pr_launch<PairS5, 1>(a, dt, mode, emit, 1, st, smp, groups); else pr_launch<PairS5, 2>(a, dt, 0, emit, 1, st, smp, groups);
    } else if (cm == PairS2::CM) {
        a.ntiles = (int)(M / PairS2::BM);
        if (add) pr_launch<PairS2, 1>(a, dt, 0, emit, 2, st, smp); else pr_launch<PairS2, 2>(a, dt, 0, emit, 2, st, smp);
    } else {
        a.ntiles = (int)(M / PairS3::BM);
        if (add) pr_launch<PairS3, 1>(a, dt, 0, emit, 1, st, smp); else pr_launch<PairS3, 2>(a, dt, 0, emit, 1, st, smp);
    }
    return urso_check_launch("urso_conv_igemm(wide pointwise)");
}
int urso_pair_single_launch(const urso_conv_geom* g, int dt, int flags, const void* src, const void* wgt, const float* bias, const void* add,
                            const void* mask_bits, void* dst, void* bits_out, hipStream_t st) {
    return pair_single_launch(g, dt, flags, src, wgt, bias, add, mask_bits, dst, bits_out, nullptr, st);
}

extern "C" int urso_conv_pointwise_sampled_ok(const urso_conv_geom* g, int dt, int flags, int has_add) {
    if (!g || (flags & URSO_EPI_MASK_BITS) || (g->OH & 1) || (g->OW & 1) || g->C >= PairS5::CM) return 0;
    return urso_pair_single_fits(g, dt, flags, has_add ? (const void*)g : nullptr, nullptr) ? 1 : 0;
}
extern "C" int urso_conv_pointwise_sampled(const urso_conv_geom* g, int dt, int flags, const void* src_d, const void* wgt_d, const float* bias_d,
                                           const void* add_d, void* dst_d, void* bits_out_d, void* dst_sampled_d, void* stream) {
    if (!g || !src_d || !wgt_d || !dst_d || !dst_sampled_d || ((flags & URSO_EPI_EMIT_BITS) && !bits_out_d)) { urso_set_error("urso_conv_pointwise_sampled: null argument"); return URSO_EINVAL; }
    if (!urso_conv_pointwise_sampled_ok(g, dt, flags, add_d != nullptr)) { urso_set_error("urso_conv_pointwise_sampled: the layer does not take the register-filter kernel (urso_conv_pointwise_sampled_ok)"); return URSO_EINVAL; }
    if ((((uintptr_t)src_d) | ((uintptr_t)wgt_d) | ((uintptr_t)add_d) | ((uintptr_t)dst_d) | ((uintptr_t)bits_out_d) | ((uintptr_t)dst_sampled_d)) & 15) {
        urso_set_error("urso_conv_pointwise_sampled: pointers must be 16-byte aligned"); return URSO_EINVAL;
    }
    hipStream_t st = (hipStream_t)stream;
    const double M = (double)g->B * g->OH * g->OW;
    ProfScope ps(st, URSO_K_IGEMM, 2.0 * M * g->C * g->N, M * 2.0 * (g->C + g->N * (add_d ? 2.25 : 1.25)) + ((flags & URSO_EPI_EMIT_BITS) ? M * g->N / 8 : 0.0));
    return pair_single_launch(g, dt, flags, src_d, wgt_d, bias_d, add_d, nullptr, dst_d, (flags & URSO_EPI_EMIT_BITS) ? bits_out_d : nullptr, dst_sampled_d, st);
}

extern "C" int urso_conv_pair(long long M, int c_narrow, int dt, int mode, const void* src_d, const void* w1_d, const float* bias1_d,
                              const void* add_d, void* bits_d, void* mid_d, const void* w2_d, const float* bias2_d, const void* mask2_d,
                              void* dst_d, int add_h, int add_w, void* stream) {
    const int cm = c_narrow, cw = 4 * c_narrow;
    if (!urso_conv_pair_ok(M, dt, cm, cw)) {
        urso_set_error("urso_conv_pair: needs 16-bit dt, (64, 256) channels with M %% 64 == 0 or (128, 512) with M %% 32 == 0, tensors < 2 GiB");
        return URSO_EINVAL;
    }
    if (!src_d || !w1_d || !add_d || !mid_d || !w2_d || !dst_d || (mode != 0 && mode != 1) || (mode == 1 && (!bits_d || !mask2_d))) {
        urso_set_error("urso_conv_pair: bad argument"); return URSO_EINVAL;
    }
    const bool sparse = add_h > 0 || add_w > 0;
    if (sparse && (mode != 1 || add_h <= 0 || add_w <= 0 || (add_h & 1) || (add_w & 1) || M % ((long long)add_h * add_w))) {
        urso_set_error("urso_conv_pair: a compact add operand needs mode 1, even add_h / add_w and M = B * add_h * add_w"); return URSO_EINVAL;
    }
    if ((((uintptr_t)src_d) | ((uintptr_t)w1_d) | ((uintptr_t)add_d) | ((uintptr_t)mid_d) | ((uintptr_t)w2_d) | ((uintptr_t)dst_d) |
         ((uintptr_t)bits_d) | ((uintptr_t)mask2_d)) & 15) { urso_set_error("urso_conv_pair: pointers must be 16-byte aligned"); return URSO_EINVAL; }
    hipStream_t st = (hipStream_t)stream;
    PairArgs a;
    a.src = src_d; a.w1 = w1_d; a.bias1 = bias1_d; a.add = add_d; a.bits = bits_d; a.mid = mid_d; a.w2 = w2_d; a.bias2 = bias2_d;
    a.mask2 = mask2_d; a.dst = dst_d; a.relu1 = 1;
    a.sp_h = add_h; a.sp_w = add_w; a.add_bytes = (uint32_t)(M / 4 * cw * 2);
    a.wide_pitch = (uint32_t)cw * 2u; a.bits_pitch = (uint32_t)cw / 8u; a.g_w1 = a.g_bias = a.g_wide = a.g_bits = 0;
    a.rcp_hw = sparse ? 1.0f / (float)(add_h * add_w) : 0.f; a.rcp_w = sparse ? 1.0f / (float)add_w : 0.f;
    a.nar_bytes = (uint32_t)(M * cm * 2); a.wide_bytes = (uint32_t)(M * cw * 2); a.bits_bytes = (uint32_t)(M * (cw / 8));
    const double flops = 2.0 * (double)M * cm * cw * 2.0;
    const double bytes = (double)M * (2.0 * cm * 2 + (sparse ? 1.25 : 2.0) * cw * 2) + (double)M * (cw / 8) * ((mode == 1 || bits_d) ? 1 : 0) +
                         (mode == 1 ? (double)M * cm * 2 : 0.0) + 2.0 * cm * cw * 2;
    ProfScope ps(st, URSO_K_IGEMM, flops, bytes);
    if (cm == PairS2::CM) { a.ntiles = (int)(M / PairS2::BM); pr_launch<PairS2, 0>(a, dt, mode, bits_d != nullptr, 2, st, sparse); }
    else { a.ntiles = (int)(M / PairS3::BM); pr_launch<PairS3, 0>(a, dt, mode, bits_d != nullptr, 1, st, sparse); }
    return urso_check_launch("urso_conv_pair");
}
```

### ursonet_amd/csrc/conv_pwx.hip

```cpp
#include "lds_mfma.h"
#include "internal.h"
#include <string.h>

struct PxArgs {
    const void* src; const void* wgt; const float* bias; const void* add; const void* mask; void* dst; void* bits_out;
    uint32_t src_bytes, wgt_bytes, dst_bytes;
    int M, C, N, Kc, nkt, tilesN, ntiles;
    int OH, OW, FH, FW, OSH, OSW;
    float rcp_ohw, rcp_ow;
    int relu;
    int dbg;
    const void* src1; const void* wgt1; uint32_t src1_bytes, wgt1_bytes; int C1, Kc1, nkt0;
};

template <typename T, int TMW, int BN, int NST, bool HAS_ADD, int MASKK, bool EMIT, bool SEG2 = false>
__global__ __launch_bounds__(512, 2) void pwx_kernel(const PxArgs a) {
    static_assert(sizeof(T) == 2, "16-bit element types only");
    constexpr bool HAS_MASK = MASKK == 1;
    constexpr int VE = 8;
    constexpr int WM = 16 * TMW, BM = 2 * WM, WN = BN / 4, TM = TMW, TN = WN / 16;
    constexpr int GA = BM / 8, RA = (GA + 7) / 8, RB = BN / 64, NDMA = RA + RB;
    static_assert(GA % 8 == 0 || GA % 8 == 4, "pixel-tile row groups: whole or half rounds of the 8 waves");
    constexpr int STAGE = (BM + BN) * 128, BIAS_OFF = NST * STAGE, LDS = BIAS_OFF + 4 * 1024;
    static_assert(LDS <= 163840, "LDS budget");
// ... 221 lines not shown
                    eo[e] = Elem<T>::from_f(y);
                    if constexpr (EMIT) mbits |= (Elem<T>::to_f(eo[e]) > 0.f) ? (1u << e) : 0u;
                }
                i32x4_t ov; __builtin_memcpy(&ov, eo, 16);
                const uint32_t so = voff(eo_cur[i], tile, v);
                buf_store16(rds, so, ov);
                if constexpr (EMIT) {
                    const uint32_t x = (uint32_t)__shfl_xor((int)mbits, 16, 64);
                    const uint32_t pr = (fg & 1) ? (x | (mbits << 8)) : (mbits | (x << 8));
                    const uint32_t y2 = (uint32_t)__shfl_xor((int)pr, 32, 64);
                    const uint32_t dw = (fg & 2) ? (y2 | (pr << 16)) : (pr | (y2 << 16));
                    __builtin_amdgcn_raw_buffer_store_b32(dw, rmo, (fg == 0) ? (so >> 4) : URSO_OOB_SHIFT, 0, 0);
                }
                {
                    const uint32_t o = voff(eo_nxt[i], next, v);
                    if constexpr (HAS_ADD) radd[i * NV + v] = buf_load16(rad, o);
                    if constexpr (HAS_MASK) rmsk[i * NV + v] = buf_load16(rmk, o);
                    if constexpr (MASKK == 2) rbit[i * NV + v] = __builtin_amdgcn_raw_buffer_load_b32(rmk, (o >> 4) & ~3u, 0, 0);
                }
            }
        }
        if (!has_next) break;
        tile = next; ++tcnt;
#pragma unroll
        for (int i = 0; i < TM; ++i) eo_cur[i] = eo_nxt[i];
    }
    wait_vm<0>();
}

static int pwx_try_impl(const urso_conv_geom* g, int dt, int relu, const void* src, const void* wgt, const float* bias, const void* add,
                        const void* mask, void* dst, uint32_t src_bytes, uint32_t wgt_bytes, uint32_t dst_bytes, int mask_bits, void* bits_out,
                        const void* src1, const void* wgt1, int C1, uint32_t src1_bytes, uint32_t wgt1_bytes, bool dry, hipStream_t st);
int urso_pwx_try(const urso_conv_geom* g, int dt, int relu, const void* src, const void* wgt, const float* bias, const void* add,
                 const void* mask, void* dst, uint32_t src_bytes, uint32_t wgt_bytes, uint32_t dst_bytes, int mask_bits, void* bits_out,
                 hipStream_t st) {
    return pwx_try_impl(g, dt, relu, src, wgt, bias, add, mask, dst, src_bytes, wgt_bytes, dst_bytes, mask_bits, bits_out, nullptr, nullptr, 0, 0, 0, false, st);
}
int urso_pwx_try2(const urso_conv_geom* g, int dt, int relu, const void* src, const void* wgt, const void* src1, const void* wgt1, int C1,
                  const float* bias, const void* mask, void* dst, uint32_t src_bytes, uint32_t wgt_bytes, uint32_t src1_bytes, uint32_t wgt1_bytes,
                  uint32_t dst_bytes, int mask_bits, void* bits_out, bool dry, hipStream_t st) {
    if (C1 <= 0 || (C1 % 64) || (mask && !mask_bits) || (mask && bits_out)) return 0;
    return pwx_try_impl(g, dt, relu, src, wgt, bias, nullptr, mask, dst, src_bytes, wgt_bytes, dst_bytes, mask_bits, bits_out, src1, wgt1, C1, src1_bytes, wgt1_bytes, dry, st);
}
static int pwx_try_impl(const urso_conv_geom* g, int dt, int relu, const void* src, const void* wgt, const float* bias, const void* add,
                        const void* mask, void* dst, uint32_t src_bytes, uint32_t wgt_bytes, uint32_t dst_bytes, int mask_bits, void* bits_out,
                        const void* src1, const void* wgt1, int C1, uint32_t src1_bytes, uint32_t wgt1_bytes, bool dry, hipStream_t st) {
    const int mode = g_urso_opt.pwx;
    if (!mode) return 0;
    const bool seg2 = C1 > 0;
    const int maskk = mask ? (mask_bits ? 2 : 1) : 0;
    const bool emit = bits_out != nullptr;
    const int form = (!add && !maskk && !emit) ? 0 : (add && !maskk && emit) ? 1 : (!add && maskk == 1 && !emit) ? 2 :
                     (add && maskk == 2 && !emit) ? 3 : (!add && maskk == 2 && !emit) ? 4 : (add && !maskk && !emit) ? 5 :
                     (seg2 && !add && !maskk && emit) ? 6 : -1;
    if (form < 0 || (g->C % 64) || (g->N % 8)) return 0;
    if (seg2 && form != 0 && form != 4 && form != 6) return 0;
    if (emit && (g->N % 32)) return 0;
    const long long M = (long long)g->B * g->OH * g->OW;
    const int K = g->C + (seg2 ? C1 : 0), N = g->N;
    if (mode == 1) {
        const bool s4_wide = K == 256 && N >= 1024 && !(g_urso_opt.pair_single & 1);
        if ((K < 512 && !s4_wide) || N < 128 || M < 160 * 32) return 0;
    }
    if (dry) return 1;
    PxArgs a;
    a.src = src; a.wgt = wgt; a.bias = bias; a.add = add; a.mask = mask; a.dst = dst; a.bits_out = bits_out;
    a.src_bytes = src_bytes; a.wgt_bytes = wgt_bytes; a.dst_bytes = dst_bytes;
    a.M = (int)M; a.C = g->C; a.N = N; a.Kc = g->C / 8; a.nkt = a.Kc / 8;
    a.src1 = src1; a.wgt1 = wgt1; a.src1_bytes = src1_bytes; a.wgt1_bytes = wgt1_bytes; a.C1 = C1; a.Kc1 = C1 / 8; a.nkt0 = a.nkt;
    if (seg2) a.nkt += a.Kc1 / 8;
    a.OH = g->OH; a.OW = g->OW; a.FH = g->FH > 0 ? g->FH : 0; a.FW = g->FW; a.OSH = g->OSH; a.OSW = g->OSW;
    a.rcp_ohw = 1.0f / (float)(g->OH * g->OW); a.rcp_ow = 1.0f / (float)g->OW; a.relu = relu; a.dbg = g_urso_opt.pwx_dbg;
    const int cus = urso_usable_cus();
    const int tm = ceil_div((int)M, 160);
    auto cost = [&](int bn) { const long long nt = (long long)tm * ceil_div(N, bn); return ((nt + cus - 1) / cus) * (long long)bn; };
    int bn = (N > 128 && cost(256) <= cost(128)) ? 256 : 128;
    if (g_urso_opt.pwx_bn == 128 || g_urso_opt.pwx_bn == 256) bn = g_urso_opt.pwx_bn;
    a.tilesN = ceil_div(N, bn); a.ntiles = tm * a.tilesN;
    const dim3 grid(urso_persistent_grid(a.ntiles, 1)), blk(512);
    urso_prof_l2((double)a.ntiles * K * 2.0 * (160 + bn));
#define URSO_PX(TT, BN_, NST_, AD_, MK_, EM_) URSO_KLAUNCH((pwx_kernel<TT, 5, BN_, NST_, AD_, MK_, EM_>), grid, blk, 0, st, a)
#define URSO_PXF(TT, BN_, NST_) switch (form) { case 0: URSO_PX(TT, BN_, NST_, false, 0, false); break; case 1: URSO_PX(TT, BN_, NST_, true, 0, true); break; \
                                                case 2: URSO_PX(TT, BN_, NST_, false, 1, false); break; case 3: URSO_PX(TT, BN_, NST_, true, 2, false); break; \
                                                case 4: URSO_PX(TT, BN_, NST_, false, 2, false); break; default: URSO_PX(TT, BN_, NST_, true, 0, false); }
#define URSO_PX2(TT, BN_, NST_) do { if (form == 4) URSO_KLAUNCH((pwx_kernel<TT, 5, BN_, NST_, false, 2, false, true>), grid, blk, 0, st, a); \
                                     else if (form == 6) URSO_KLAUNCH((pwx_kernel<TT, 5, BN_, NST_, false, 0, true, true>), grid, blk, 0, st, a); \
                                     else URSO_KLAUNCH((pwx_kernel<TT, 5, BN_, NST_, false, 0, false, true>), grid, blk, 0, st, a); } while (0)
    if (seg2) {
        if (dt == URSO_BF16) { if (bn == 256) URSO_PX2(__bf16, 256, 3); else URSO_PX2(__bf16, 128, 4); }
        else { if (bn == 256) URSO_PX2(_Float16, 256, 3); else URSO_PX2(_Float16, 128, 4); }
    }
    else if (dt == URSO_BF16) { if (bn == 256) { URSO_PXF(__bf16, 256, 3) } else { URSO_PXF(__bf16, 128, 4) } }
    else { if (bn == 256) { URSO_PXF(_Float16, 256, 3) } else { URSO_PXF(_Float16, 128, 4) } }
#undef URSO_PX2
#undef URSO_PXF
#undef URSO_PX
    const int rc = urso_check_launch("urso_conv_igemm(pwx)");
    return rc == URSO_OK ? 1 : rc;
}

static int pw2_check(int B, int OH, int OW, int C0, int C1, int N, int dt, int flags, const void* mask_d, const void* bits_out_d) {
    if (B <= 0 || OH <= 0 || OW <= 0 || C0 <= 0 || C1 <= 0 || N <= 0) return URSO_EINVAL;
    if ((dt != URSO_BF16 && dt != URSO_F16) || (C0 % 64) || (C1 % 64) || (N % 8)) return URSO_EINVAL;
    if (flags & ~(URSO_EPI_RELU | URSO_EPI_MASK_BITS | URSO_EPI_EMIT_BITS)) return URSO_EINVAL;
    if ((flags & URSO_EPI_MASK_BITS) && (flags & URSO_EPI_EMIT_BITS)) return URSO_EINVAL;
    if ((mask_d != nullptr) != ((flags & URSO_EPI_MASK_BITS) != 0) || (bits_out_d != nullptr) != ((flags & URSO_EPI_EMIT_BITS) != 0)) return URSO_EINVAL;
    if ((flags & (URSO_EPI_MASK_BITS | URSO_EPI_EMIT_BITS)) && (N % 32)) return URSO_EINVAL;
    const size_t M = (size_t)B * OH * OW;
    if (M * (size_t)(C0 > C1 ? C0 : C1) * 2 >= 0x7FFFFF00ull || M * (size_t)N * 2 >= 0x7FFFFF00ull) return URSO_EINVAL;
    return URSO_OK;
}
static urso_conv_geom pw2_geom(int B, int OH, int OW, int C0, int N) {
    urso_conv_geom g;
    memset(&g, 0, sizeof(g));
    g.B = B; g.H = OH; g.W = OW; g.C = C0; g.OH = OH; g.OW = OW; g.N = N; g.KH = g.KW = 1; g.SH = g.SW = 1; g.DH = g.DW = 1;
    return g;
}
extern "C" int urso_conv_pointwise2_ok(int B, int OH, int OW, int C0, int C1, int N, int dt, int flags) {
    const void* one = (const void*)1;
    if (pw2_check(B, OH, OW, C0, C1, N, dt, flags, (flags & URSO_EPI_MASK_BITS) ? one : nullptr, (flags & URSO_EPI_EMIT_BITS) ? one : nullptr) != URSO_OK) return 0;
    const urso_conv_geom g = pw2_geom(B, OH, OW, C0, N);
    return urso_pwx_try2(&g, dt, 0, nullptr, nullptr, nullptr, nullptr, C1, nullptr, (flags & URSO_EPI_MASK_BITS) ? one : nullptr, nullptr,
                         0, 0, 0, 0, 0, (flags & URSO_EPI_MASK_BITS) ? 1 : 0, (flags & URSO_EPI_EMIT_BITS) ? (void*)1 : nullptr, true, nullptr) == 1;
}
extern "C" int urso_conv_pointwise2(int B, int OH, int OW, int C0, int C1, int N, int dt, int flags,
                                    const void* src0_d, const void* wgt0_d, const void* src1_d, const void* wgt1_d,
                                    const float* bias_d, const void* mask_d, void* dst_d, void* bits_out_d, void* stream) {
    if (!src0_d || !wgt0_d || !src1_d || !wgt1_d || !dst_d) { urso_set_error("urso_conv_pointwise2: null argument"); return URSO_EINVAL; }
    const int rc0 = pw2_check(B, OH, OW, C0, C1, N, dt, flags, mask_d, bits_out_d);
    if (rc0 != URSO_OK) { urso_set_error("urso_conv_pointwise2: unsupported arguments (16-bit, C0 %% 64 == C1 %% 64 == 0, N %% 8 == 0 (32 with a bit mask), flags RELU | MASK_BITS | EMIT_BITS)"); return rc0; }
    hipStream_t st = (hipStream_t)stream;
    const urso_conv_geom g = pw2_geom(B, OH, OW, C0, N);
    const size_t M = (size_t)B * OH * OW;
    const double es = 2.0;
    ProfScope ps(st, URSO_K_IGEMM, 2.0 * (double)M * N * (C0 + C1),
                 (double)M * (C0 + C1) * es + (double)N * (C0 + C1) * es + (double)M * N * es + ((mask_d || bits_out_d) ? (double)M * N / 8 : 0.0));
    const int rc = urso_pwx_try2(&g, dt, (flags & URSO_EPI_RELU) ? 1 : 0, src0_d, wgt0_d, src1_d, wgt1_d, C1, bias_d, mask_d, dst_d,
// ... 6 lines not shown
```

### ursonet_amd/csrc/internal.h

```cpp
#pragma once
#include "common.h"

int urso_pw_launch(const urso_conv_geom* g, int dt, int conv, int dhs, int dws, int relu,
                   const void* src, const void* wgt, const float* bias, const void* add, const void* mask, void* dst,
                   uint32_t src_bytes, uint32_t wgt_bytes, uint32_t dst_bytes, int mask_bits, void* bits_out, int add_src, hipStream_t st);
int urso_pwx_try(const urso_conv_geom* g, int dt, int relu, const void* src, const void* wgt, const float* bias, const void* add,
                 const void* mask, void* dst, uint32_t src_bytes, uint32_t wgt_bytes, uint32_t dst_bytes, int mask_bits, void* bits_out,
                 hipStream_t st);
bool urso_pair_single_fits(const urso_conv_geom* g, int dt, int flags, const void* add, const void* mask);
int urso_pair_single_launch(const urso_conv_geom* g, int dt, int flags, const void* src, const void* wgt, const float* bias, const void* add,
                            const void* mask_bits, void* dst, void* bits_out, hipStream_t st);
bool urso_stem_fits(const urso_conv_geom* g, int dt, int flags, const void* add, const void* mask);
int urso_stem_launch(const urso_conv_geom* g, int dt, int relu, const void* src, const void* wgt, const float* bias, void* dst, hipStream_t st);
bool urso_c3_fits(const urso_conv_geom* g, int dt, int flags, const void* add);
int urso_c3_launch(const urso_conv_geom* g, int dt, int relu, const void* src, const void* wgt, const float* bias, const void* mask,
                   void* dst, hipStream_t st);
bool urso_hconv_fits(const urso_conv_geom* g, int dt, int flags, const void* add);
int urso_hconv_launch(const urso_conv_geom* g, int dt, int relu, const void* src, const void* wgt, const float* bias, const void* add,
                      const void* mask, void* dst, uint32_t src_bytes, uint32_t wgt_bytes, uint32_t dst_bytes, void* ws, size_t ws_bytes,
                      hipStream_t st);
size_t urso_hconv_ws_bytes();
int urso_hconv2_pick(const urso_conv_geom* g, bool has_ws);
int urso_hconv2_try_launch(const urso_conv_geom* g, int dt, int relu, const void* src, const void* wgt, const float* bias, const void* mask,
                           void* dst, uint32_t src_bytes, uint32_t wgt_bytes, uint32_t dst_bytes, void* ws, bool has_ws, hipStream_t st);
bool urso_bneck_fwd_fits(const urso_conv_geom* g, int dt, int flags, const void* add, const void* mask);
int urso_bneck_fwd_launch(const urso_conv_geom* g, int dt, int flags, const void* src, const void* wgt, const float* bias, void* dst, hipStream_t st);
bool urso_bneck_dgrad_fits(const urso_conv_geom* g, int dt, int flags, const void* add, const void* mask);
int urso_bneck_dgrad_launch(const urso_conv_geom* g, int dt, int flags, const void* dz, const void* wd, const void* mask, void* dst, hipStream_t st);
bool urso_dense_fits(const urso_conv_geom* g, int dt, int flags, int pointwise, long long M);
int urso_dense_launch(const urso_conv_geom* g, int dt, int flags, const void* src, const void* wgt, const float* bias, const void* add,
                      const void* mask, void* dst, uint32_t src_bytes, uint32_t wgt_bytes, uint32_t dst_bytes, hipStream_t st);

bool urso_c3g_fits(const urso_conv_geom* g, int dt);
int urso_c3g_splits(const urso_conv_geom* g);
int urso_c3g_launch(const urso_conv_geom* g, int dt, const void* x, const void* dz, float* part, float* colpart, size_t part_stride, hipStream_t st);
bool urso_hwg_fits(const urso_conv_geom* g, int dt);
int urso_hwg_splits(const urso_conv_geom* g);
int urso_hwg_launch(const urso_conv_geom* g, int dt, const void* x, const void* dz, float* part, float* colpart, size_t part_stride, hipStream_t st);
bool urso_hwg_pair_splits(const urso_conv_geom* g0, const urso_conv_geom* g1, int dt, int* s0, int* s1);
int urso_hwg_launch2(const urso_conv_geom* g0, const urso_conv_geom* g1, int dt, const void* x0, const void* dz0, float* part0, float* colpart0,
                     const void* x1, const void* dz1, float* part1, float* colpart1, hipStream_t st);
bool urso_stemw_fits(const urso_conv_geom* g, int dt);
int urso_stemw_splits(const urso_conv_geom* g, bool pooled);
int urso_stemw_launch(const urso_conv_geom* g, int dt, const void* x, const void* dz, const void* dpool, const uint8_t* am,
                      float* part, float* colpart, size_t part_stride, hipStream_t st);
void urso_reduce_partials_batch_launch(const urso_param_desc* descs_d, const int32_t* blockmap_d, int nblocks, hipStream_t st);
```

### ursonet_amd/csrc/lds_mfma.h

```cpp
#pragma once
#include "common.h"

typedef __attribute__((ext_vector_type(16))) float f32x16_t;
typedef short s16x4_t __attribute__((ext_vector_type(4)));

template <typename T> struct Mma32;
template <> struct Mma32<__bf16> {
    static __device__ __forceinline__ void run(const i32x4_t& a, const i32x4_t& b, f32x16_t& c) {
        c = __builtin_amdgcn_mfma_f32_32x32x16_bf16(__builtin_bit_cast(bf16x8_t, a), __builtin_bit_cast(bf16x8_t, b), c, 0, 0, 0);
    }
    static __device__ __forceinline__ f32x16_t mad(const i32x4_t& a, const i32x4_t& b, const f32x16_t& c) {
        return __builtin_amdgcn_mfma_f32_32x32x16_bf16(__builtin_bit_cast(bf16x8_t, a), __builtin_bit_cast(bf16x8_t, b), c, 0, 0, 0);
    }
};
template <> struct Mma32<_Float16> {
    static __device__ __forceinline__ void run(const i32x4_t& a, const i32x4_t& b, f32x16_t& c) {
        c = __builtin_amdgcn_mfma_f32_32x32x16_f16(__builtin_bit_cast(f16x8_t, a), __builtin_bit_cast(f16x8_t, b), c, 0, 0, 0);
    }
    static __device__ __forceinline__ f32x16_t mad(const i32x4_t& a, const i32x4_t& b, const f32x16_t& c) {
        return __builtin_amdgcn_mfma_f32_32x32x16_f16(__builtin_bit_cast(f16x8_t, a), __builtin_bit_cast(f16x8_t, b), c, 0, 0, 0);
    }
};

__device__ __forceinline__ void lds_dma16(const i32x4_t& rsrc, uint32_t lds_byte, uint32_t voff) {
    asm volatile("s_mov_b32 m0, %1\n\ts_nop 0\n\tbuffer_load_dwordx4 %0, %2, 0 offen lds" :: "v"(voff), "s"(lds_byte), "s"(rsrc) : "memory");
}
__device__ __forceinline__ void lds_dma16_sgpr(const i32x4_t& rsrc, uint32_t lds_byte, uint32_t voff) {
    asm volatile("s_mov_b32 m0, %1\n\ts_nop 0\n\tbuffer_load_dwordx4 %0, %2, 0 offen lds" :: "v"(voff), "s"(__builtin_amdgcn_readfirstlane(lds_byte)), "s"(rsrc) : "memory");
}

__device__ __forceinline__ i32x4_t raw_rsrc(const void* p, uint32_t bytes) {
    const uint64_t a = (uint64_t)p;
    return i32x4_t{(int)(uint32_t)a, (int)(uint32_t)((a >> 32) & 0xFFFFu), (int)bytes, 0x00020000};
}
__device__ __forceinline__ i32x4_t raw_rsrc_sgpr(const void* p, uint32_t bytes) {
    const uint64_t a = (uint64_t)p;
    return i32x4_t{__builtin_amdgcn_readfirstlane((int)(uint32_t)a), __builtin_amdgcn_readfirstlane((int)(uint32_t)((a >> 32) & 0xFFFFu)),
                   __builtin_amdgcn_readfirstlane((int)bytes), 0x00020000};
}

template <int N> __device__ __forceinline__ void wait_vm() { asm volatile("s_waitcnt vmcnt(%0)" :: "n"(N) : "memory"); }

__device__ __forceinline__ void lds_barrier_asm() { asm volatile("s_waitcnt lgkmcnt(0)\n\ts_barrier" ::: "memory"); }

__device__ __forceinline__ i32x2_t lds_read_tr16(const char* p) {
    return __builtin_bit_cast(i32x2_t, __builtin_amdgcn_ds_read_tr16_b64_v4i16((__attribute__((address_space(3))) s16x4_t*)p));
}

__device__ __forceinline__ uint32_t halo_rd(int row, int h) {
    const int s = (row >> 1) & 7;
    return (uint32_t)(row * 128 + ((s >> 1) << 5) + ((h ^ (s & 1)) << 4));
}
__device__ __forceinline__ int halo_perm(int rho) {
    const int g = rho >> 3, hh = (rho >> 2) & 1, e = rho & 3;
    return 16 * (g >> 1) + 8 * hh + 4 * (g & 1) + e;
}
```

### ursonet_amd/engine.py

```python
import math
import os
import re
from collections import OrderedDict

import numpy as np
import torch

from . import grad_accum, hip, lars, loss_scale, loss_weights, weight_ema
from .config import compute_dtype_name
from .graph import BN_EPS, build_graph, conv_flops
from .plan_state import _Act, _Conv, _Launch, _PendingLaunches, _round_up

BN_MOMENTUM = 0.99

_DT = {"float32": hip.F32, "bfloat16": hip.BF16, "float16": hip.F16}


_SIDE_STREAMS = {}


def _side_stream(device):
    key = torch.device(device).index or 0
    if key not in _SIDE_STREAMS:
        _SIDE_STREAMS[key] = torch.cuda.Stream(device=device)
# ... 600 lines not shown
        if node.name in self._last_of_group:
            q.flush_bucket()
            k = self._last_of_group[node.name]
            for kind in self._BUCKET_PHASES:
                self.bwd_ops.append(_Launch(None, kind, "%s:bucket%d" % (kind, k), done=tuple(self._bucket_groups[k]), bucket=k))

    def _plan_residual_handover(self, c, Gsum):
        if c.res is None or not self.grad_needed[c.res.spec.id]:
            return
        B, node = self.B, c.node
        R = c.res
        if R.grad_written or R.pending is not None:
            raise AssertionError("unexpected second residual consumer for %s" % node.name)
        if R.spec.relu and c.dst.compact is not None and c.dst.residual_needs_dense:
            c.dst.grad_dense = torch.zeros(c.dst.numel, dtype=self.tdt, device=self.device)
            self.bwd_ops.append(_Launch(lambda X=c.dst: hip.rows_scatter2(B, X.compact[0], X.compact[1], X.spec.c * 2, X.grad, X.grad_dense),
                                        "expand", "expand:" + node.name))
            R.pending = c.dst.grad_dense
        elif R.spec.relu:
            R.pending = Gsum
            R.pending_hw = c.dst.compact
        else:
            assert c.dst.compact is None
            R.grad, R.grad_written = Gsum, True

    def _plan_dgrad(self, c, G, q, lvl_n):
        node = c.node
        if c.dgrad_done_by_pair or node.stem or not self.grad_needed[c.src.spec.id]:
            return
        B, dt = self.B, self.dt
        X = c.src
        add = X.grad if X.grad_written else X.pending
        if c.solo:
            assert add is None
            dstg = X.grad_buf()
            self.bwd_ops.append(_Launch(lambda c=c, G=G, X=X, dstg=dstg, Ms=B * node.dst.h * node.dst.w:
                                        hip.conv_dgrad_wgrad_pw(Ms, dt, G, c.wd, X.data, X.spec.relu, dstg, c.wg_ws, c.wg_ws[c.wg_npart:],
                                                                c.K_raw * c.npad + hip.WGRAD_PART_PAD),
                                        "dgrad+wgrad", "dgrad+wgrad:" + node.name, dgrad=(node.name,), wgrad=(node.name,), done=(node.name,)))
            X.grad_written = True
            return
        if X.compact is not None:
            self._dgrad_compact(c, G, X)
            return
        A = self.pair_first.get(node.name)
        if (A is not None and X.spec.relu and X.bits is not None and X.pending is not None and not X.grad_written and
                self.grad_needed[A.src.spec.id] and A.src.spec.relu and A.src.bits is None and not A.src.grad_written and A.src.pending is None):
            self._dgrad_pair(c, A, G, X, add)
            return
        assert X.pending_hw is None or X.grad_written, "compact residual gradient reached a non-fused data gradient (%s)" % node.name
        dstg = X.grad_buf()
        mask = (X.bits if X.bits is not None else X.data) if X.spec.relu else None
        mflag = hip.EPI_MASK_BITS if (X.spec.relu and X.bits is not None) else 0
        if lvl_n is not None and mflag == 0 and not c.gd_scatter and self._dense_multi_ok(c):
            q.add_dense_dgrad(dict(names=(node.name,), level=lvl_n, src0=G, wgt0=c.wd, K0=c.npad, N=node.cin, M=B, add=add, mask=mask, dst=dstg, flags=0))
            X.grad_written, X.pending = True, None
            return
        if c.gd_scatter:
            if add is None:
                self._clear_scattered_dgrad(c, X, dstg)
            elif add is not dstg:
                raise AssertionError("scattered dgrad into %s needs an in-place accumulate" % node.name)
        self._emit_dgrad(lambda c=c, G=G, add=add, mask=mask, dstg=dstg, mflag=mflag:
                         hip.conv_igemm_ex(c.gd, dt, mflag, G, c.wd, None, add, mask, dstg, None,
                                           self.halo_ws if (c.halo_d and add is None and not mflag) else (self.igemm_ws if c.ws_d else None)), (node.name,))
        X.grad_written, X.pending = True, None

    def _emit_dgrad(self, run, dgrad, wgrad=()):
        label = "dgrad:" + "+".join(dgrad) + ("+wgrad:" + "+".join(wgrad) if wgrad else "")
        self.bwd_ops.append(_Launch(run, "dgrad", label, dgrad=dgrad, wgrad=wgrad))
        return self.bwd_ops[-1]

    def _dgrad_compact(self, c, G, X):
        B, dt, node = self.B, self.dt, c.node
        if not X.grad_written and not X.fwd_sampled:
            self.bwd_ops.append(_Launch(lambda X=X: hip.rows_subsample2(B, X.compact[0], X.compact[1], X.spec.c // 8, X.bits, X.bits_compact),
                                        "bits_subsample"))
        gq = c.gd_compact
        first = X._compact_first
        if (first is not None and X.grad_written and
                hip.conv_pointwise2_ok(B, gq.OH, gq.OW, first[1].npad, c.npad, node.cin, dt, hip.EPI_MASK_BITS)):
            launch0, c0, G0 = first
            self.bwd_ops.remove(launch0)
            self._emit_dgrad(lambda c=c, c0=c0, G0=G0, G=G, X=X, gq=gq, N=node.cin:
                             hip.conv_pointwise2(B, gq.OH, gq.OW, c0.npad, c.npad, N, dt, hip.EPI_MASK_BITS, G0, c0.wd, G, c.wd, None,
                                                 X.bits_compact, X.grad), (c0.name, node.name))
            X._compact_first = None
            self.n_entry_dgrad2 += 1
            return
        launch = self._emit_dgrad(lambda c=c, G=G, X=X, add=(X.grad if X.grad_written else None):
                                  hip.conv_igemm_ex(c.gd_compact, dt, hip.EPI_MASK_BITS, G, c.wd, None, add, X.bits_compact, X.grad, None, None),
                                  (node.name,))
        X._compact_first = (launch, c, G) if not X.grad_written else None
        X.grad_written = True

    def _dgrad_pair(self, c, A, G, X, add):
        dt, node = self.dt, c.node
        dstg, dst2 = X.grad_buf(), A.src.grad_buf()
        a_tr = self.layer_trainable[A.name] or bool(A.node.bn and not A.batch_bn and self.layer_trainable[A.node.bn])
        wsplits = hip.conv_pair_wgrad_splits(A.Mpix, dt) if (A.node.cin == 64 and hip.get_option("pair") == 1) else 0
        if a_tr and wsplits > 1 and A.gf_compact is None:
            A.splits = A.desc.splits = wsplits
            A.wgrad_by_pair = True
            Sc = self._pair_entry_shortcut(A, X)
            if Sc is not None:
                Sc.splits = Sc.desc.splits = wsplits
                Sc.wgrad_by_pair = Sc.dgrad_done_by_pair = True
                dxin = Sc.src.grad_buf()
                Sc.src.grad_written = True
                dstg.zero_()
                dstg._urso_on_chip = True
                self._emit_dgrad(lambda c=c, A=A, Sc=Sc, G=G, add=add, X=X, dst2=dst2, dxin=dxin:
                                 hip.conv_pair_wgrad_entry(A.Mpix, dt, G, c.wd, add, X.bits, A.wd, A.src.data, dst2, Sc.wd, Sc.src.data, Sc.src.spec.relu, dxin,
                                                           A.wg_ws, A.wg_ws[A.wg_npart:], Sc.wg_ws, Sc.wg_ws[Sc.wg_npart:],
                                                           A.K_raw * A.npad + hip.WGRAD_PART_PAD), (node.name, A.name, Sc.name), (A.name, Sc.name))
            else:
                self._emit_dgrad(lambda c=c, A=A, G=G, add=add, X=X, dstg=dstg, dst2=dst2, hw=X.pending_hw:
                                 hip.conv_pair_wgrad(A.Mpix, dt, G, c.wd, add, X.bits, dstg, A.wd, A.src.data, dst2,
# ... 181 lines not shown

        def joined(op):
            def run():
                self._join_weight_gradients()
                self._main_moved = True
                return op()
            return run

        def on_main(op):
            def run():
                self._main_moved = True
                return op()
            return run
        for l in self.bwd_ops:
            l.run = (on_side if l in side else joined if l.kind in fin else on_main)(l.run)
        self.opt_ops[0].run = joined(self.opt_ops[0].run)

    def _stream_edge(self, src, dst):
        ev = torch.cuda.Event()
        ev.record(src)
        dst.wait_event(ev)
        if torch.cuda.is_current_stream_capturing():
            self._graph_events.append(ev)

    def _join_weight_gradients(self):
        if self.wgrad_stream is not None and self._side_open:
            self._stream_edge(self.wgrad_stream, torch.cuda.current_stream(self.device))
            self._side_open = False

    def _plan_relu_bitmasks(self):
        dt = self.dt
        for X in self.acts.values():
            X.bits = None
            if not X.spec.relu or X.numel % 8:
                continue
            prod = [c for c in self.convs.values() if c.dst is X]
            cons = [c for c in self.convs.values() if c.src is X and c.gd is not None]
            if len(prod) != 1 or not cons or not prod[0].node.relu:
                continue
            P = prod[0]
            if P.batch_bn:
                continue
            pw = lambda n: (not n.dense) and n.kh == 1 and n.kw == 1
            bn_ = lambda c: (hip.get_option("bneck") and not c.node.dense and c.node.kh == 3 and c.node.kw == 3 and c.node.stride == 2 and
                             c.npad == 32 and c.node.cin % 64 == 0 and not c.batch_bn)
            if not (pw(P.node) and P.node.stride == 1 and P.N % 32 == 0 and all(pw(c.node) or bn_(c) for c in cons)):
                continue
            if P.res is None:
                continue
            if not hip.conv_igemm_bits_ok(P.gf, dt, P.fwd_flags, P.ws_f):
                continue
            if all(hip.conv_igemm_bits_ok(c.gd, dt, 0, c.ws_d) for c in cons):
                X.bits = torch.empty(X.numel // 8, dtype=torch.uint8, device=self.device)

    def _upload_param_table(self):
        self.pbatch = hip.ParamBatch(self._descs, self.device) if self._descs else None
        if self.pbatch is not None:
            self.pbatch.plan(hip.PB_PREP, "all", list(range(len(self._descs))))

    def _build_heads_io(self):
        cfg, B, dev = self.config, self.B, self.device
        self.quat_head = bool(cfg.REGRESS_ORI and cfg.ORIENTATION_PARAM == "quaternion" and not cfg.REGRESS_KEYPOINTS)
        if self.quat_head:
            self.q_out = torch.zeros(B, 4, dtype=torch.float32, device=dev)
            if self.mode == "inference":
                x = self.out_ori
                self.fwd_ops.append(_Launch(lambda: hip.absdot(B, 4, 8, 1, None, x.data, 1.0, self.dt, self.q_out, None, None), "quat"))

    def _build_losses(self):
        cfg, g, B, dt, dev = self.config, self.graph, self.B, self.dt, self.device
        lw = cfg.LOSS_WEIGHTS
        self.loss_buf = torch.zeros(4, dtype=torch.float32, device=dev)
        self.rel_norms = torch.zeros(2, dtype=torch.float32, device=dev)
        loc, ori = self.out_loc, self.out_ori
        nloc = g.outputs["loc"].c
        nori = g.outputs["ori"].c if "ori" in g.outputs else 0
        self.row_ws = torch.empty(B, dtype=torch.float32, device=dev)
        if cfg.REGRESS_KEYPOINTS:
            self.gt_loc = torch.zeros(B, 3, dtype=torch.float32, device=dev)
            self.gt_ori = torch.zeros(B, 3, dtype=torch.float32, device=dev)
            self.gt_k3 = torch.zeros(B, 3, dtype=torch.float32, device=dev)
            for key, gt, wname, li in (("k1", self.gt_loc, "loc_loss", 0), ("k2", self.gt_ori, "k2_loss", 2), ("k3", self.gt_k3, "k3_loss", 3)):
                a = self.acts[g.outputs[key].id]
                gzt = torch.empty(a.numel, dtype=self.tdt, device=dev)
                a.grad, a.grad_written = gzt, True
                self.loss_ops.append(_Launch(lambda a=a, gt=gt, w=float(lw.get(wname, 1.)), li=li, gzt=gzt:
                                             hip.mse(B, 3, 8, gt, a.data, w, dt, self.loss_buf[li:li + 1], gzt, ls=self.ls_state), "loss"))
            return
        if (not cfg.REGRESS_LOC and nloc % 8) or (not cfg.REGRESS_ORI and nori % 8):
            raise ValueError("classification heads need a bin count that is a multiple of 8 (got %d / %d)" % (nloc, nori))
        gz_loc = torch.empty(loc.numel, dtype=self.tdt, device=dev)
        loc.grad, loc.grad_written = gz_loc, True
        wl = float(lw.get("loc_loss", 1.))
        lw_loc, lw_ori = self._lw_views("loc_weight"), self._lw_views("ori_weight")
        if cfg.REGRESS_LOC:
            self.gt_loc = torch.zeros(B, 3, dtype=torch.float32, device=dev)
            self.rel_exact = bool(getattr(cfg, "DP_EXACT_REL_LOSS", False))
            if self.rel_exact:
                if self.rel_scale is None:
                    self.rel_scale = torch.ones(1, dtype=torch.float32, device=dev)
                self.loss_pre_ops.append(_Launch(lambda: hip.rel_l2_norms(B, 3, 8, self.gt_loc, loc.data, self.rel_norms), "loss"))
                self.loss_ops.append(_Launch(lambda: hip.rel_l2_from_norms(B, 3, 8, self.gt_loc, loc.data, wl, self.rel_scale, dt, self.rel_norms,
                                                                           self.loss_buf[0:1], gz_loc), "loss"))
            else:
                self.loss_ops.append(_Launch(lambda: hip.rel_l2(B, 3, 8, self.gt_loc, loc.data, wl, dt, self.loss_buf[0:1], gz_loc, self.rel_norms,
                                                                ls=self.ls_state, lw=lw_loc), "loss"))
# ... 168 lines not shown
        convs = [self.convs[nm] for nm in lv]
        pos = [self.fwd_ops.index(c.fwd) if c.fwd is not None and c.fwd.computes_only(c) else -1 for c in convs]
        if (len(convs) < 2 or min(pos) < 0 or sorted(pos) != list(range(min(pos), min(pos) + len(pos))) or
                not all(self._dense_multi_ok(c) for c in convs)):
            self.dense_multi = False
            return
        ops = []
        for depth in sorted(set(lv.values())):
            cs = [c for c in convs if lv[c.name] == depth]
            for i in range(0, len(cs), hip.DENSE_MULTI_MAX):
                part = cs[i:i + hip.DENSE_MULTI_MAX]
                m = hip.DenseMulti([dict(src0=c.xin, wgt0=c.wf, K0=c.node.cin, N=c.npad, M=self.B, bias=c.biasf, dst=c.dst.data, flags=c.fwd_flags)
                                    for c in part], self.dt)
                ops.append(_Launch(m.run, "fwd", "fwd:" + "+".join(c.name for c in part), fwd=tuple(c.name for c in part)))
                for c in part:
                    c.fwd = ops[-1]
        self.fwd_ops[min(pos):max(pos) + 1] = ops

    def _fuse_pointwise_pairs(self):
        self.pair_first = {}
        self.shortcut_folded = []
        g, dt = self.graph, self.dt
        if dt == hip.F32 or not hip.get_option("pair"):
            return
        convs = [n for n in g.nodes if n.op != "pool"]
        for a_node, b_node in zip(convs[:-1], convs[1:]):
            A, Bc = self.convs[a_node.name], self.convs[b_node.name]

            def plain(n, c):
                return (not n.stem and not n.dense and n.kh == 1 and n.kw == 1 and n.stride == 1 and n.relu and not n.out_f32 and
                        not c.batch_bn and c.npad == c.N and c.fwd is not None)
            if not (plain(a_node, A) and plain(b_node, Bc)):
                continue
            if a_node.residual is None or b_node.residual is not None or b_node.src.id != a_node.dst.id:
                continue
            M = self.B * a_node.dst.h * a_node.dst.w
            if not (a_node.cin == b_node.cout and hip.conv_pair_ok(M, dt, a_node.cin, a_node.cout)):
                continue
            A.Mpix = M
            S = [self.convs[n.name] for n in convs if n.dst.id == a_node.residual.id]
            readers = [n for n in g.nodes if (n.op == "pool" and n.src.id == a_node.residual.id) or
                       (n.op != "pool" and (n.src.id == a_node.residual.id or (n.residual is not None and n.residual.id == a_node.residual.id)))]
            if (len(S) == 1 and hip.get_option("pair") in (1, 2) and a_node.cin == 64 and M % 64 == 0 and len(readers) == 1 and
                    (lambda n, c: not n.stem and not n.dense and n.kh == 1 and n.kw == 1 and n.stride == 1 and not n.relu and not n.out_f32 and
                     n.residual is None and n.cin == 64 and n.cout == a_node.cout and not c.batch_bn and c.npad == c.N and
                     c.fwd is not None)(S[0].node, S[0])):
                Sc = S[0]
                A.fwd.run = (lambda A=A, Bc=Bc, Sc=Sc: hip.conv_pair_shortcut(
                    A.Mpix, dt, A.src.data, A.wf, A.biasf, Sc.src.data, Sc.wf, Sc.biasf, A.dst.bits, A.dst.data, Bc.wf, Bc.biasf, Bc.dst.data))
                self._share_forward(A, Sc, Bc)
                self.shortcut_folded.append(Sc.name)
            else:
                A.fwd.run = (lambda A=A, Bc=Bc: hip.conv_pair(A.Mpix, A.node.cin, dt, 0, A.src.data, A.wf, A.biasf, A.res.data, A.dst.bits,
                                                             A.dst.data, Bc.wf, Bc.biasf, None, Bc.dst.data))
                self._share_forward(A, Bc)
            self.pair_first[b_node.name] = A

    def _share_forward(self, A, *others):
        A.fwd.fwd = (A.name,) + tuple(c.name for c in others)
        A.fwd.label = "fwd:" + "+".join(A.fwd.fwd)
        for c in others:
            self.fwd_ops.remove(c.fwd)
            c.fwd = A.fwd

    def _fuse_entry_shortcuts(self):
        g, dt, B = self.graph, self.dt, self.B
        self.n_entry_fwd2 = 0
        if dt == hip.F32:
            return
        convs = [n for n in g.nodes if n.op != "pool"]
        alone = lambda c: c.fwd is not None and c.fwd.computes_only(c)
        outs = set(t.id for t in g.outputs.values()) | ({g.feat.id} if getattr(g, "feat", None) is not None and hasattr(g.feat, "id") else set())
        for a_node in convs:
            A = self.convs[a_node.name]
            if (a_node.stem or a_node.dense or a_node.kh != 1 or a_node.kw != 1 or a_node.stride != 1 or not a_node.relu or a_node.out_f32 or
                    a_node.residual is None or A.batch_bn or A.npad != A.N or not alone(A) or A.dst.fwd_sampled):
                continue
            S = [self.convs[n.name] for n in convs if n.dst.id == a_node.residual.id]
            if len(S) != 1:
                continue
            Sc, sn = S[0], S[0].node
            readers = [n for n in g.nodes if (n.op == "pool" and n.src.id == a_node.residual.id) or
                       (n.op != "pool" and (n.src.id == a_node.residual.id or (n.residual is not None and n.residual.id == a_node.residual.id)))]
            M = B * a_node.dst.h * a_node.dst.w
            if (len(readers) != 1 or a_node.residual.id in outs or sn.stem or sn.dense or sn.kh != 1 or sn.kw != 1 or sn.relu or sn.out_f32 or
                    sn.residual is not None or Sc.batch_bn or Sc.npad != Sc.N or Sc.N != A.N or not alone(Sc) or
                    sn.dst.h != a_node.dst.h or sn.dst.w != a_node.dst.w or
                    Sc.xin.numel() != M * sn.cin or A.xin.numel() != M * a_node.cin):
                continue
            fl = hip.EPI_RELU
            if not (hip.conv_pointwise2_ok(B, a_node.dst.h, a_node.dst.w, a_node.cin, sn.cin, A.N, dt, fl) and
                    (A.N % 32 == 0 and hip.conv_pointwise2_ok(B, a_node.dst.h, a_node.dst.w, a_node.cin, sn.cin, A.N, dt, fl | hip.EPI_EMIT_BITS))):
                continue
            A.fwd.run = (lambda A=A, Sc=Sc, oh=a_node.dst.h, ow=a_node.dst.w, c0=a_node.cin, c1=sn.cin: hip.conv_pointwise2(
                B, oh, ow, c0, c1, A.N, dt, hip.EPI_RELU | (hip.EPI_EMIT_BITS if A.dst.bits is not None else 0),
                A.xin, A.wf, Sc.xin, Sc.wf, A.biasf, None, A.dst.data, A.dst.bits))
            self._share_forward(A, Sc)
            A.desc.bias_from = Sc.desc_id + 1
            self.shortcut_folded.append(Sc.name)
            Sc.dst.data = torch.empty(0, dtype=self.tdt, device=self.device)
            self.n_entry_fwd2 += 1

    def run_prep(self):
        for op in self.prep_ops:
            op()

    def run_forward(self):
        for op in self.fwd_ops:
            op()

    def run_backward(self):
        for op in self.loss_pre_ops + self.loss_ops:
            op()
        for op in self.bwd_ops:
            op()

    def run_optimizer(self):
        for op in self.opt_ops:
            op()

    PLAN_OPTIONS = ("cus", "wgrad_blocks", "wgrad_narrow", "wgrad_big", "hwgrad", "grid_cap", "pair", "stem", "stem_pool", "c3", "bneck", "dense",
                    "pwx")

    def check_cleared_once(self):
        bad = []
        for name, buf, h, w, c, sy, sx in self._cleared_once:
            t = buf[:self.B * h * w * c].view(self.B, h, w, c)
            off = t.clone()
            off[:, ::sy, ::sx, :] = 0
            if bool(off.any()):
                bad.append(name)
        return bad

    def _planning_options(self):
        return tuple(hip.get_option(o) for o in self.PLAN_OPTIONS)

    def _check_plan_options(self):
        now = self._planning_options()
        if now != self._plan_options:
            diff = ", ".join("%s %d -> %d" % (o, a, b) for o, a, b in zip(self.PLAN_OPTIONS, self._plan_options, now) if a != b)
            raise RuntimeError("kernel-policy options changed since this engine planned its step (%s): the split counts and partial workspaces of the "
                               "weight-gradient launches are sized at plan time -- build the Engine under the options it runs with" % diff)

    def step_eager(self):
        self._check_plan_options()
        if self.accum_k > 1:
            self._run_micro(self._accum_roles[self.accum_micro])
            self.accum_micro = (self.accum_micro + 1) % self.accum_k
            return
        self.run_prep(); self.run_forward(); self.run_backward(); self.run_optimizer()

    def _run_micro(self, role):
        assert role in grad_accum.ROLES and self.accum_k > 1
        self._accum_role = role
        self.run_prep(); self.run_forward(); self.run_backward()
        for op in (self.opt_ops if role == "close" else self.accum_ops):
            op()

    def param_pass_bytes(self, launch):
        FUSE_MAX = 16
        es = 4 if self.dt == hip.F32 else 2
        kind = launch.kind
        if launch.bucket is None or kind not in ("prep", "reduce", "finalize_mat"):
            return None
        ds = self._descs if kind == "prep" else [self.convs[nm].desc for nm in self._bucket_groups[launch.bucket]]
        total = 0.0
        for d in ds:
            K, N, npad, sp = int(d.K), int(d.N), int(d.npad), max(int(d.splits), 1)
            if kind == "prep":
                total += K * N * 4 + K * npad * es * (2 if d.wd else 1)
            elif kind == "reduce":
                if sp > FUSE_MAX:
                    total += (sp + 1) * K * npad * 4
            else:
                total += 2 * K * N * 4 + (sp if 1 < sp <= FUSE_MAX else 1) * K * npad * 4
# ... 321 lines not shown
```

### ursonet_amd/hip.py

```python
import ctypes as C
import os

import numpy as np
import torch

_HERE = os.path.dirname(os.path.abspath(__file__))
_VARIANT = os.environ.get("URSO_LIB_VARIANT", "")
LIB_PATH = os.path.join(_HERE, "lib", "liburso_hip%s.so" % (("_" + _VARIANT) if _VARIANT else ""))
EXT_LIB_PATH = os.path.join(_HERE, "lib", "liburso_ext.so")

F32, BF16, F16 = 0, 1, 2
EPI_RELU, EPI_OUT_F32, EPI_MASK_BITS, EPI_EMIT_BITS, EPI_ADD_SRCGRID = 1, 2, 4, 8, 16
K_IGEMM, K_WGRAD, K_PREP, K_FINALIZE, K_POOL, K_LOSS, K_OPTIM, K_DECODE, K_MOLD = range(1, 10)
KERNEL_NAMES = {K_IGEMM: "conv_igemm", K_WGRAD: "conv_wgrad", K_PREP: "weight_prep", K_FINALIZE: "param_grad_finalize",
                K_POOL: "maxpool", K_LOSS: "loss", K_OPTIM: "optimizer", K_DECODE: "quat_decode", K_MOLD: "mold"}

TORCH_DT = {F32: torch.float32, BF16: torch.bfloat16, F16: torch.float16}
DT_OF_TORCH = {v: k for k, v in TORCH_DT.items()}
DT_NAME = {F32: "f32", BF16: "bf16", F16: "f16"}


class ConvGeom(C.Structure):
    _fields_ = [(n, C.c_int32) for n in
                ("B", "H", "W", "C", "OH", "OW", "N", "KH", "KW", "SH", "SW", "PH", "PW", "DH", "DW",
# ... 349 lines not shown


def bucket_round_ef(g, resid, c, stream=None):
    assert g.dtype == torch.float32 and resid.dtype == torch.float32 and c.dtype == torch.bfloat16 and g.numel() == resid.numel() == c.numel()
    _chk(_lib.urso_bucket_round_ef(g.numel(), ptr(g), ptr(resid), ptr(c), stream_ptr(stream)), "urso_bucket_round_ef")


def bucket_expand_bf16(c, g, stream=None):
    assert g.dtype == torch.float32 and c.dtype == torch.bfloat16 and g.numel() == c.numel()
    _chk(_lib.urso_bucket_expand_bf16(g.numel(), ptr(c), ptr(g), stream_ptr(stream)), "urso_bucket_expand_bf16")


def conv_winograd_ws_bytes(g, dt):
    return int(_lib.urso_conv_winograd_ws_bytes(C.byref(g), dt))


def conv_winograd_fwd(g, dt, flags, src, wgt, bias, dst, ws, stream=None):
    _chk(_lib.urso_conv_winograd_fwd(C.byref(g), dt, flags, ptr(src), ptr(wgt), ptr(bias), ptr(dst), ptr(ws), ws.numel() * ws.element_size(),
                                     stream_ptr(stream)), "urso_conv_winograd_fwd")


def conv_igemm_ws_bytes(g, dt):
    return int(_lib.urso_conv_igemm_ws_bytes(C.byref(g), dt))


def conv_igemm_ws(g, dt, flags, src, wgt, bias, add, mask, dst, ws, stream=None):
    _chk(_lib.urso_conv_igemm_ws(C.byref(g), dt, flags, ptr(src), ptr(wgt), ptr(bias), ptr(add), ptr(mask), ptr(dst),
                                 ptr(ws), ws.numel() * ws.element_size() if ws is not None else 0, stream_ptr(stream)),
         "urso_conv_igemm_ws")


def conv_igemm_bits_ok(g, dt, flags, ws_bytes=0):
    return bool(_lib.urso_conv_igemm_bits_ok(C.byref(g), dt, flags, ws_bytes))


def conv_igemm_halo_ws_bytes():
    return int(_lib.urso_conv_igemm_halo_ws_bytes())


def conv_igemm_halo_ok(g, dt, flags, has_add=False):
    return bool(_lib.urso_conv_igemm_halo_ok(C.byref(g), dt, flags, int(bool(has_add))))


def conv_igemm_algorithmic(g, dt, flags, has_add=False, has_mask=False):
    fl, by = C.c_double(0), C.c_double(0)
    _chk(_lib.urso_conv_igemm_algorithmic(C.byref(g), dt, flags, int(bool(has_add)), int(bool(has_mask)), C.byref(fl), C.byref(by)), "urso_conv_igemm_algorithmic")
    return float(fl.value), float(by.value)


def conv_igemm_halo2_shape(g, dt, flags, has_add=False, has_ws=False):
    return int(_lib.urso_conv_igemm_halo2_shape(C.byref(g), dt, flags, int(bool(has_add)), int(bool(has_ws))))


def conv_igemm_ex(g, dt, flags, src, wgt, bias, add, mask, dst, bits_out=None, ws=None, stream=None):
    _chk(_lib.urso_conv_igemm_ex(C.byref(g), dt, flags, ptr(src), ptr(wgt), ptr(bias), ptr(add), ptr(mask), ptr(dst), ptr(bits_out),
                                 ptr(ws), (ws.numel() * ws.element_size()) if ws is not None else 0, stream_ptr(stream)), "urso_conv_igemm_ex")


def conv_pointwise2_ok(B, OH, OW, C0, C1, N, dt, flags):
    return bool(_lib.urso_conv_pointwise2_ok(B, OH, OW, C0, C1, N, dt, flags))


def conv_pointwise2(B, OH, OW, C0, C1, N, dt, flags, src0, wgt0, src1, wgt1, bias, mask, dst, bits_out=None, stream=None):
    _chk(_lib.urso_conv_pointwise2(B, OH, OW, C0, C1, N, dt, flags, ptr(src0), ptr(wgt0), ptr(src1), ptr(wgt1), ptr(bias), ptr(mask), ptr(dst),
                                   ptr(bits_out), stream_ptr(stream)), "urso_conv_pointwise2")


def conv_wgrad_ws_bytes(g, dt):
    return int(_lib.urso_conv_wgrad_ws_bytes(C.byref(g), dt))


def conv_wgrad(g, dt, x, dz, ws, dw_raw, colsum, stream=None):
    _chk(_lib.urso_conv_wgrad(C.byref(g), dt, ptr(x), ptr(dz), ptr(ws), ws.numel() * ws.element_size(), ptr(dw_raw),
                              ptr(colsum), stream_ptr(stream)), "urso_conv_wgrad")


def conv_wgrad_splits(g, dt):
    return int(_lib.urso_conv_wgrad_splits(C.byref(g), dt))


def conv_wgrad_partial(g, dt, x, dz, ws, stream=None):
    _chk(_lib.urso_conv_wgrad_partial(C.byref(g), dt, ptr(x), ptr(dz), ptr(ws), ws.numel() * ws.element_size(), stream_ptr(stream)),
         "urso_conv_wgrad_partial")


def param_desc_init(d, KH, KW, Cin, N, npad, splits, eps, weight_decay):
    _chk(_lib.urso_param_desc_init(C.byref(d), KH, KW, Cin, N, npad, splits, eps, weight_decay), "urso_param_desc_init")


class ParamBatch(object):

    def __init__(self, descs, device):
        self.n = len(descs)
        self.host = (ParamDesc * self.n)(*descs)
        raw = torch.frombuffer(bytearray(bytes(self.host)), dtype=torch.uint8)
        self.dev = raw.to(device)
        self.maps = {}

    def plan(self, phase, key, layer_ids):
        ids = (C.c_int32 * len(layer_ids))(*layer_ids)
        nb = _lib.urso_param_batch_plan(phase, self.host, ids, len(layer_ids), None, 0)
        if nb < 0:
            raise UrsoHipError("urso_param_batch_plan: " + last_error())
        buf = (C.c_int32 * (2 * max(nb, 1)))()
        _lib.urso_param_batch_plan(phase, self.host, ids, len(layer_ids), buf, nb)
        t = torch.frombuffer(bytearray(bytes(buf)), dtype=torch.int32).to(self.dev.device)
# ... 360 lines not shown
    a.loc_map_rows = 0 if loc_map is None else loc_map.shape[0]
    a.loc_bins = loc.shape[1] if loc_mode == EVAL_LOC_CLASS else 0
    return a


def pose_eval(B, n, row0, loc_mode, ori_mode, loc, ori, loc_gt, q_gt, table, ori2=None, loc_map=None, ori_map=None, enc_loc=None,
              enc_ori=None, gmm_mean=None, gmm_nmodes=None, stream=None):
    a = _pose_args(PoseEvalArgs(), B, n, row0, loc_mode, ori_mode, loc, ori, ori2, loc_map, table)
    a.ori_map = ptr(ori_map)
    a.ori_map_rows = 0 if ori_map is None else ori_map.shape[0]
    a.ori_bins = 0 if enc_ori is None else enc_ori.shape[1]
    a.enc_loc, a.enc_ori, a.loc_gt, a.q_gt = ptr(enc_loc), ptr(enc_ori), ptr(loc_gt), ptr(q_gt)
    a.gmm_mean, a.gmm_nmodes = ptr(gmm_mean), ptr(gmm_nmodes)
    a.gmm_modes = 0 if gmm_mean is None else gmm_mean.shape[1]
    _chk(_lib.urso_pose_eval(C.byref(a), stream_ptr(stream)), "urso_pose_eval")


def pose_decode(B, n, row0, loc_mode, ori_mode, loc, ori, table, ori2=None, loc_map=None, ori_logits=None, ori_map_rows=0, ori_scatter=None,
                stream=None):
    a = _pose_args(PoseDecodeArgs(), B, n, row0, loc_mode, ori_mode, loc, ori, ori2, loc_map, table)
    a.ori_logits, a.ori_logits_ld = _rows(ori_logits)
    a.ori_bins = 0 if ori_logits is None else ori_logits.shape[1]
    a.ori_map_rows = int(ori_map_rows)
    a.ori_scatter = ptr(ori_scatter)
    _chk(_lib.urso_pose_decode(C.byref(a), stream_ptr(stream)), "urso_pose_decode")


def pose_fuse_views(B, n, row0, est, r, qr, table, loc_gt=None, q_gt=None, est_view_rows=None, stream=None):
    assert est.dtype == torch.float64 and r.dtype == torch.float64 and qr.dtype == torch.float64 and table.dtype == torch.float64
    assert r.is_contiguous() and qr.is_contiguous() and table.is_contiguous() and r.shape[0] == qr.shape[0]
    a = PoseFuseViewsArgs()
    a.B, a.n, a.row0, a.V = int(B), int(n), int(row0), int(r.shape[0])
    a.est, a.est_ld = _rows(est)
    a.est_view_rows = int(B if est_view_rows is None else est_view_rows)
    assert est.shape[0] >= (a.V - 1) * a.est_view_rows + a.B and table.shape[0] >= a.row0 + a.n and table.shape[1] == FUSE_COLS
    a.r, a.qr, a.loc_gt, a.q_gt, a.table = ptr(r), ptr(qr), ptr(loc_gt), ptr(q_gt), ptr(table)
    _chk(ext_lib().urso_pose_fuse_views(C.byref(a), stream_ptr(stream)), "urso_pose_fuse_views")


def warp_perspective(B, H, W, Cc, interp, src, m, dst, stream=None):
    assert src.dtype == torch.uint8 and dst.dtype == torch.uint8 and m.dtype == torch.float64
    _chk(_lib.urso_warp_perspective(B, H, W, Cc, int(interp), ptr(src), ptr(m), ptr(dst), stream_ptr(stream)), "urso_warp_perspective")


def encode_ori(B, K, q, hquat, redundant, var, out, stream=None):
    assert q.dtype == torch.float64 and redundant.dtype == torch.uint8
    _chk(_lib.urso_encode_ori(B, K, ptr(q), ptr(hquat), ptr(redundant), float(var), ptr(out), stream_ptr(stream)), "urso_encode_ori")


def conv_pair_ok(M, dt, c_narrow, c_wide):
    return bool(_lib.urso_conv_pair_ok(int(M), dt, int(c_narrow), int(c_wide)))


def conv_pair(M, c_narrow, dt, mode, src, w1, bias1, add, bits, mid, w2, bias2, mask2, dst, add_hw=None, stream=None):
    ah, aw = add_hw if add_hw else (0, 0)
    _chk(_lib.urso_conv_pair(int(M), int(c_narrow), dt, int(mode), ptr(src), ptr(w1), ptr(bias1), ptr(add), ptr(bits), ptr(mid), ptr(w2), ptr(bias2),
                             ptr(mask2), ptr(dst), int(ah), int(aw), stream_ptr(stream)), "urso_conv_pair")


def conv_pair_shortcut(M, dt, src, w1, bias1, xin, ws, bias_s, bits, mid, w2, bias2, dst, stream=None):
    _chk(_lib.urso_conv_pair_shortcut(int(M), dt, ptr(src), ptr(w1), ptr(bias1), ptr(xin), ptr(ws), ptr(bias_s), ptr(bits), ptr(mid), ptr(w2),
                                      ptr(bias2), ptr(dst), stream_ptr(stream)), "urso_conv_pair_shortcut")


def conv_dgrad_wgrad_pw(M, dt, dz, wd, x, mask_by_x, dx, part, colpart, part_stride, stream=None):
    _chk(_lib.urso_conv_dgrad_wgrad_pw(int(M), dt, ptr(dz), ptr(wd), ptr(x), int(bool(mask_by_x)), ptr(dx), ptr(part), ptr(colpart),
                                       int(part_stride), stream_ptr(stream)), "urso_conv_dgrad_wgrad_pw")


def conv_pair_wgrad_entry(M, dt, src, w1, add, bits, w2, u, dst, ws, xin, mask_by_xin, dxin, part, colpart, part_s, colpart_s, part_stride, stream=None):
    _chk(_lib.urso_conv_pair_wgrad_entry(int(M), dt, ptr(src), ptr(w1), ptr(add), ptr(bits), ptr(w2), ptr(u), ptr(dst), ptr(ws), ptr(xin), int(bool(mask_by_xin)), ptr(dxin),
                                         ptr(part), ptr(colpart), ptr(part_s), ptr(colpart_s), int(part_stride), stream_ptr(stream)),
         "urso_conv_pair_wgrad_entry")


def stem_conv_pool_ok(g, dt):
    return bool(_lib.urso_stem_conv_pool_ok(C.byref(g), dt))


def stem_conv_pool(g, dt, x, wf, bias, y_pooled, argmax, stream=None):
    _chk(_lib.urso_stem_conv_pool(C.byref(g), dt, ptr(x), ptr(wf), ptr(bias), ptr(y_pooled), ptr(argmax), stream_ptr(stream)), "urso_stem_conv_pool")


def stem_wgrad_pooled(g, dt, x, dpool, argmax, ws, dw_raw, colsum, stream=None):
    _chk(_lib.urso_stem_wgrad_pooled(C.byref(g), dt, ptr(x), ptr(dpool), ptr(argmax), ptr(ws), ws.numel() * ws.element_size(), ptr(dw_raw),
                                     ptr(colsum), stream_ptr(stream)), "urso_stem_wgrad_pooled")


def conv_pair_wgrad_splits(M, dt):
    return int(_lib.urso_conv_pair_wgrad_splits(int(M), dt))


def conv_pair_wgrad(M, dt, src, w1, add, bits, mid, w2, u, dst, part, colpart, part_stride, add_hw=None, stream=None):
    ah, aw = add_hw if add_hw else (0, 0)
    _chk(_lib.urso_conv_pair_wgrad(int(M), dt, ptr(src), ptr(w1), ptr(add), ptr(bits), ptr(mid), ptr(w2), ptr(u), ptr(dst), int(ah), int(aw),
                                   ptr(part), ptr(colpart), int(part_stride), stream_ptr(stream)), "urso_conv_pair_wgrad")


def conv_pointwise_sampled_ok(g, dt, flags, has_add=False):
    return bool(_lib.urso_conv_pointwise_sampled_ok(C.byref(g), dt, flags, int(bool(has_add))))


def conv_pointwise_sampled(g, dt, flags, src, wgt, bias, add, dst, bits_out, dst_sampled, stream=None):
    _chk(_lib.urso_conv_pointwise_sampled(C.byref(g), dt, flags, ptr(src), ptr(wgt), ptr(bias), ptr(add), ptr(dst), ptr(bits_out), ptr(dst_sampled),
                                          stream_ptr(stream)), "urso_conv_pointwise_sampled")


def zero_fill(t, stream=None):
# ... 163 lines not shown
```

Baseline: 4672 images/sec.

## Use 1-bit ReLU masks for in-block 3x3 data gradients

Adds a planner path that gives in-block ReLU activations between a 1x1 producer and a 3x3 consumer a packed bitmask. The forward producer (including the paired 1x1 kernel) emits the bits, and the 3x3 dgrad kernels (c3, c3v, halo2) read one bit per element instead of the full 16-bit activation. The goal is less HBM traffic in the backward mask epilogue. In exchange it adds bit-emission work in the forward pass, extra template variants and new constraints, such as no residual add on that path.

```diff
diff --git a/ursonet_amd/csrc/common.h b/ursonet_amd/csrc/common.h
--- a/ursonet_amd/csrc/common.h
+++ b/ursonet_amd/csrc/common.h
@@ -40,6 +40,7 @@
     X(pwx_dbg, 0)           \
     X(pwx_bn, 0)            \
     X(mold_scalar, 0)       \
+    X(inblock_bits, 5)      \
     X(bneck, 3)
 struct UrsoOptions {
 #define URSO_OPT_FIELD(name, dflt) int name = dflt;
diff --git a/ursonet_amd/csrc/conv_c3.hip b/ursonet_amd/csrc/conv_c3.hip
--- a/ursonet_amd/csrc/conv_c3.hip
+++ b/ursonet_amd/csrc/conv_c3.hip
@@ -5,6 +5,7 @@
 struct C3Args {
     const void* src; const void* wgt; const float* bias; const void* mask; void* dst;
     uint32_t bytes;
+    uint32_t mbytes;
     int B, H, W, tiles_x, tiles_y, ntiles;
     int relu;
 };
@@ -18,7 +19,7 @@
     return (uint32_t)(row * 128 + ((((2 * j + h) ^ s)) << 4));
 }
 
-template <typename T, bool MASK>
+template <typename T, int MASK>
 __global__ __launch_bounds__(256, 2) void c3_kernel(const C3Args a) {
     static_assert(sizeof(T) == 2, "16-bit element types only");
     __shared__ __attribute__((aligned(1024))) char smem[C3_LDS];
@@ -35,7 +36,7 @@
 
     const i32x4_t rs = raw_rsrc(a.src, a.bytes);
     const __amdgpu_buffer_rsrc_t rds = make_rsrc(a.dst, a.bytes);
-    const __amdgpu_buffer_rsrc_t rmk = make_rsrc(MASK ? a.mask : a.dst, MASK ? a.bytes : 0u);
+    const __amdgpu_buffer_rsrc_t rmk = make_rsrc(MASK ? a.mask : a.dst, MASK ? a.mbytes : 0u);
 
     int lane_d = lane;
     auto tile_origin = [&](int t, int& b, int& y0, int& x0) {
@@ -84,6 +85,17 @@
         first = false;
         lds_barrier_asm();
         if (has_next) dma_tile(tile + bpx, buf ^ 1);
+        uint32_t mb[NST];
+        if constexpr (MASK == 2) {
+            int b, y0, x0;
+            tile_origin(tile, b, y0, x0);
+#pragma unroll
+            for (int i = 0; i < NST; ++i) {
+                const int row = 8 * (wave + 4 * i) + (lane_d >> 3);
+                const int y = y0 + (row >> 5), x = x0 + (row & 31);
+                mb[i] = relu_bits_load(rmk, (y < a.H && x < a.W) ? (uint32_t)(((b * a.H + y) * a.W + x) * 128 + (((lane_d & 7) ^ ((row >> 1) & 7)) << 4)) : URSO_OOB_SHIFT);
+            }
+        }
 
         f32x16_t acc[2];
         {
@@ -139,19 +151,14 @@
             const int row = 8 * (wave + 4 * i) + (lane >> 3);
             const int y = y0 + (row >> 5), x = x0 + (row & 31);
             so[i] = (y < a.H && x < a.W) ? (uint32_t)(((b * a.H + y) * a.W + x) * 128 + (((lane & 7) ^ ((row >> 1) & 7)) << 4)) : URSO_OOB_SHIFT;
-            if constexpr (MASK) mv[i] = buf_load16(rmk, so[i]);
+            if constexpr (MASK == 1) mv[i] = buf_load16(rmk, so[i]);
         }
         lds_barrier_asm();
 #pragma unroll
         for (int i = 0; i < NST; ++i) {
             i32x4_t v = *(const i32x4_t*)(sO + (wave + 4 * i) * 1024 + lane * 16);
-            if constexpr (MASK) {
-                T x[8], m[8];
-                __builtin_memcpy(x, &v, 16); __builtin_memcpy(m, &mv[i], 16);
-#pragma unroll
-                for (int e = 0; e < 8; ++e) x[e] = Elem<T>::to_f(m[e]) > 0.f ? x[e] : Elem<T>::from_f(0.f);
-                __builtin_memcpy(&v, x, 16);
-            }
+            if constexpr (MASK == 1) v = relu_mask_apply<T>(v, mv[i]);
+            if constexpr (MASK == 2) v = relu_bits_apply<T>(v, relu_bits_byte(mb[i], so[i]));
             buf_store16(rds, so[i], v);
         }
         if (!has_next) break;
@@ -182,7 +189,7 @@
 
     const i32x4_t rs = raw_rsrc(a.src, a.bytes);
     const __amdgpu_buffer_rsrc_t rds = make_rsrc(a.dst, a.bytes);
-    const __amdgpu_buffer_rsrc_t rmk = make_rsrc(MASK ? a.mask : a.dst, MASK ? a.bytes : 0u);
+    const __amdgpu_buffer_rsrc_t rmk = make_rsrc(MASK ? a.mask : a.dst, MASK ? a.mbytes : 0u);
 
     int lane_d = lane;
     auto tile_origin = [&](int t, int& b, int& y0, int& x0) {
@@ -388,7 +395,7 @@
 template <class F, int... I> __device__ __forceinline__ void c3_static_for_impl(F&& f, std::integer_sequence<int, I...>) { (f(std::integral_constant<int, I>{}), ...); }
 template <int N, class F> __device__ __forceinline__ void c3_static_for(F&& f) { c3_static_for_impl(static_cast<F&&>(f), std::make_integer_sequence<int, N>{}); }
 
-template <typename T, bool MASK>
+template <typename T, int MASK>
 __global__ __launch_bounds__(512, 2) void c3v_kernel(const C3Args a) {
     static_assert(sizeof(T) == 2, "16-bit element types only");
     __shared__ __attribute__((aligned(1024))) char smem[C3V_LDS];
@@ -403,7 +410,7 @@
 
     const i32x4_t rs = raw_rsrc(a.src, a.bytes);
     const __amdgpu_buffer_rsrc_t rds = make_rsrc(a.dst, a.bytes);
-    const __amdgpu_buffer_rsrc_t rmk = make_rsrc(MASK ? a.mask : a.dst, MASK ? a.bytes : 0u);
+    const __amdgpu_buffer_rsrc_t rmk = make_rsrc(MASK ? a.mask : a.dst, MASK ? a.mbytes : 0u);
 
     int lane_d = lane;
     auto tile_origin = [&](int t, int& b, int& y0, int& x0) {
@@ -449,13 +456,8 @@
 #pragma unroll
         for (int i = 0; i < NST; ++i) {
             i32x4_t v = *(const i32x4_t*)(sO + (wave + 8 * i) * 1024 + lane * 16);
-            if constexpr (MASK) {
-                T x[8], m[8];
-                __builtin_memcpy(x, &v, 16); __builtin_memcpy(m, &mv[i], 16);
-#pragma unroll
-                for (int e = 0; e < 8; ++e) x[e] = Elem<T>::to_f(m[e]) > 0.f ? x[e] : Elem<T>::from_f(0.f);
-                __builtin_memcpy(&v, x, 16);
-            }
+            if constexpr (MASK == 1) v = relu_mask_apply<T>(v, mv[i]);
+            if constexpr (MASK == 2) v = relu_bits_apply<T>(v, relu_bits_byte((uint32_t)mv[i].x, so[i]));
             buf_store16(rds, so[i], v);
         }
     };
@@ -468,6 +470,16 @@
         lds_barrier_asm();
         if (has_next) dma_tile(tile + bpx, buf ^ 1);
         if (pend) flush(ob ^ 1);
+        if constexpr (MASK == 2) {
+            int b, y0, x0;
+            tile_origin(tile, b, y0, x0);
+#pragma unroll
+            for (int i = 0; i < NST; ++i) {
+                const int p = (wave + 8 * i) * 64 + lane_d, px = p >> 4;
+                const int y = y0 + (px >> 4), x = x0 + (px & 15);
+                mv[i].x = (int)relu_bits_load(rmk, (y < a.H && x < a.W) ? (uint32_t)(((b * a.H + y) * a.W + x) * 256 + (((p & 15) ^ (px & 15)) << 4)) : URSO_OOB_SHIFT);
+            }
+        }
         f32x4_t acc[8];
 #pragma unroll
         for (int r = 0; r < 8; ++r) acc[r] = f32x4_t{0.f, 0.f, 0.f, 0.f};
@@ -518,7 +530,7 @@
                 const int p = (wave + 8 * i) * 64 + lane, px = p >> 4;
                 const int y = y0 + (px >> 4), x = x0 + (px & 15);
                 so[i] = (y < a.H && x < a.W) ? (uint32_t)(((b * a.H + y) * a.W + x) * 256 + (((p & 15) ^ (px & 15)) << 4)) : URSO_OOB_SHIFT;
-                if constexpr (MASK) mv[i] = buf_load16(rmk, so[i]);
+                if constexpr (MASK == 1) mv[i] = buf_load16(rmk, so[i]);
             }
         }
         pend = true;
@@ -537,7 +549,7 @@
 static int c3w_best_tw(int H, int W) { return c3w_util(H, W, 16) > c3w_util(H, W, 32) ? 16 : 32; }
 
 bool urso_c3_fits(const urso_conv_geom* g, int dt, int flags, const void* add) {
-    if (!g_urso_opt.c3 || add || (dt != URSO_BF16 && dt != URSO_F16) || (flags & (URSO_EPI_OUT_F32 | URSO_EPI_MASK_BITS | URSO_EPI_EMIT_BITS))) return false;
+    if (!g_urso_opt.c3 || add || (dt != URSO_BF16 && dt != URSO_F16) || (flags & (URSO_EPI_OUT_F32 | URSO_EPI_EMIT_BITS))) return false;
     if (g->KH != 3 || g->KW != 3 || g->SH != 1 || g->SW != 1 || g->PH != 1 || g->PW != 1 || g->DH != 1 || g->DW != 1 || g->FH > 0) return false;
     if (!((g->C == 64 && g->N == 64) || (g->C == 128 && g->N == 128 && (g_urso_opt.c3 == 1 || g_urso_opt.c3 == 3))) || g->OH != g->H || g->OW != g->W) return false;
     if (g->C == 128 && g_urso_opt.c3 == 1) {
@@ -545,23 +557,30 @@
     }
     return (long long)g->B * g->H * g->W * g->C * 2 < 0x7FFFFF00ll;
 }
-
-int urso_c3_launch(const urso_conv_geom* g, int dt, int relu, const void* src, const void* wgt, const float* bias, const void* mask,
+bool urso_c3_bits_ok(const urso_conv_geom* g) {
+    return g->C == 64 || (g->C == 128 && c3w_best_tw(g->H, g->W) == 16 && g_urso_opt.c3v);
+}
+
+int urso_c3_launch(const urso_conv_geom* g, int dt, int relu, const void* src, const void* wgt, const float* bias, const void* mask, int mask_bits,
                    void* dst, hipStream_t st) {
     C3Args a;
     a.src = src; a.wgt = wgt; a.bias = bias; a.mask = mask; a.dst = dst; a.relu = relu;
     a.B = g->B; a.H = g->H; a.W = g->W;
     a.bytes = (uint32_t)((size_t)g->B * g->H * g->W * g->C * 2);
+    const int mk = mask ? (mask_bits ? 2 : 1) : 0;
+    a.mbytes = mk == 2 ? a.bytes / 16 : a.bytes;
     const bool wide = g->C == 128;
+    if (mk == 2 && !urso_c3_bits_ok(g)) { urso_set_error("urso_conv_igemm(3x3, 128 channels): this tile form takes no bit mask (urso_c3_bits_ok)"); return URSO_EINVAL; }
     const int tw = wide ? c3w_best_tw(g->H, g->W) : C3_TW, th = 128 / tw;
     a.tiles_x = ceil_div(g->W, tw); a.tiles_y = ceil_div(g->H, th); a.ntiles = g->B * a.tiles_y * a.tiles_x;
     const dim3 grid(urso_persistent_grid(a.ntiles, wide ? 1 : 2)), blk(wide ? 512 : 256);
+#define URSO_C3M(KERN, TT) do { if (mk == 2) URSO_KLAUNCH((KERN<TT, 2>), grid, blk, 0, st, a); else if (mk == 1) URSO_KLAUNCH((KERN<TT, 1>), grid, blk, 0, st, a); \
+                                else URSO_KLAUNCH((KERN<TT, 0>), grid, blk, 0, st, a); } while (0)
     if (wide) {
 #define URSO_C3W(TT, TWV) do { if (mask) URSO_KLAUNCH((c3w_kernel<TT, true, TWV>), grid, blk, 0, st, a); \
                                else URSO_KLAUNCH((c3w_kernel<TT, false, TWV>), grid, blk, 0, st, a); } while (0)
         if (tw == 16 && g_urso_opt.c3v) {
-            if (dt == URSO_BF16) { if (mask) URSO_KLAUNCH((c3v_kernel<__bf16, true>), grid, blk, 0, st, a); else URSO_KLAUNCH((c3v_kernel<__bf16, false>), grid, blk, 0, st, a); }
-            else { if (mask) URSO_KLAUNCH((c3v_kernel<_Float16, true>), grid, blk, 0, st, a); else URSO_KLAUNCH((c3v_kernel<_Float16, false>), grid, blk, 0, st, a); }
+            if (dt == URSO_BF16) URSO_C3M(c3v_kernel, __bf16); else URSO_C3M(c3v_kernel, _Float16);
             return urso_check_launch("urso_conv_igemm(3x3, 128 channels, 16-filter waves)");
         }
         if (dt == URSO_BF16) { if (tw == 32) URSO_C3W(__bf16, 32); else URSO_C3W(__bf16, 16); }
@@ -569,12 +588,7 @@
 #undef URSO_C3W
         return urso_check_launch("urso_conv_igemm(3x3, 128 channels)");
     }
-    if (dt == URSO_BF16) {
-        if (mask) URSO_KLAUNCH((c3_kernel<__bf16, true>), grid, blk, 0, st, a);
-        else URSO_KLAUNCH((c3_kernel<__bf16, false>), grid, blk, 0, st, a);
-    } else {
-        if (mask) URSO_KLAUNCH((c3_kernel<_Float16, true>), grid, blk, 0, st, a);
-        else URSO_KLAUNCH((c3_kernel<_Float16, false>), grid, blk, 0, st, a);
-    }
+    if (dt == URSO_BF16) URSO_C3M(c3_kernel, __bf16); else URSO_C3M(c3_kernel, _Float16);
+#undef URSO_C3M
     return urso_check_launch("urso_conv_igemm(3x3, 64 channels)");
 }
diff --git a/ursonet_amd/csrc/conv_halo.hip b/ursonet_amd/csrc/conv_halo.hip
--- a/ursonet_amd/csrc/conv_halo.hip
+++ b/ursonet_amd/csrc/conv_halo.hip
@@ -327,14 +327,15 @@
 size_t urso_hconv_ws_bytes() { return 4096 + (size_t)urso_device_cus() * 512 * 64 * sizeof(float); }
 
 int urso_hconv_launch(const urso_conv_geom* g, int dt, int relu, const void* src, const void* wgt, const float* bias, const void* add,
-                      const void* mask, void* dst, uint32_t src_bytes, uint32_t wgt_bytes, uint32_t dst_bytes, void* ws, size_t ws_bytes,
+                      const void* mask, int mask_bits, void* dst, uint32_t src_bytes, uint32_t wgt_bytes, uint32_t dst_bytes, void* ws, size_t ws_bytes,
                       hipStream_t st) {
     (void)add;
     {
-        const int r2 = urso_hconv2_try_launch(g, dt, relu, src, wgt, bias, mask, dst, src_bytes, wgt_bytes, dst_bytes, ws,
+        const int r2 = urso_hconv2_try_launch(g, dt, relu, src, wgt, bias, mask, mask_bits, dst, src_bytes, wgt_bytes, dst_bytes, ws,
                                               ws && ws_bytes >= urso_hconv_ws_bytes(), st);
         if (r2 != 0) return r2 > 0 ? URSO_OK : r2;
     }
+    if (mask && mask_bits) { urso_set_error("urso_conv_igemm(halo): only conv_halo2.hip takes a bit mask (urso_conv_igemm_bits_native)"); return URSO_EINVAL; }
     HcArgs a;
     a.src = src; a.wgt = wgt; a.bias = bias; a.add = add; a.mask = mask; a.dst = dst;
     a.src_bytes = src_bytes; a.wgt_bytes = wgt_bytes; a.dst_bytes = dst_bytes;
diff --git a/ursonet_amd/csrc/conv_halo2.hip b/ursonet_amd/csrc/conv_halo2.hip
--- a/ursonet_amd/csrc/conv_halo2.hip
+++ b/ursonet_amd/csrc/conv_halo2.hip
@@ -17,6 +17,7 @@
     int krow;
     float rcp_vw, rcp_vh;
     int relu;
+    int mbits;
     unsigned long long* clk;
     int dbg;
 };
@@ -48,7 +49,7 @@
     if (t_begin >= t_end || (a.dbg & 1024)) return;
 
     const i32x4_t rs = raw_rsrc(a.src, a.src_bytes), rw = raw_rsrc(a.wgt, a.wgt_bytes);
-    const __amdgpu_buffer_rsrc_t rmk = make_rsrc(a.mask ? a.mask : a.dst, a.mask ? a.dst_bytes : 0u);
+    const __amdgpu_buffer_rsrc_t rmk = make_rsrc(a.mask ? a.mask : a.dst, a.mask ? (a.mbits ? a.dst_bytes / 16 : a.dst_bytes) : 0u);
     const __amdgpu_buffer_rsrc_t rds = make_rsrc(a.dst, a.dst_bytes);
 
     if (tid * 4 < a.N) {
@@ -245,6 +246,17 @@
                 divmod(p0 + 32 * MI * wm + rl, a.Vw, a.rcp_vw, q1, vx);
                 divmod(q1, a.Vh, a.rcp_vh, vb, vy);
             }
+            uint32_t mbq[NST];
+            if (a.mask && a.mbits) {
+                int wx = vx, wy = vy, wb = vb;
+#pragma unroll
+                for (int k = 0; k < NST; ++k) {
+                    const bool ok = wb * a.Vh * a.Vw + wy * a.Vw + wx < a.Mv && wx < a.W && wy < a.H;
+                    mbq[k] = relu_bits_load(rmk, ok ? (uint32_t)((wb * a.H + wy) * a.W + wx) * (uint32_t)a.N * 2u + (uint32_t)(n0 + 32 * NJ * wn + 8 * cl) * 2u : URSO_OOB_SHIFT);
+                    wx += RPI;
+                    if (wx >= a.Vw) { wx -= a.Vw; if (++wy == a.Vh) { wy = 0; ++wb; } }
+                }
+            }
 #pragma unroll
             for (int i = 0; i < MI; ++i) {
 #pragma unroll
@@ -272,19 +284,13 @@
                     ov[q] = *(const i32x4_t*)(smem + sbase + row * (64 * NJ) + ((cl ^ ((row >> 1) & (LPR - 1))) << 4));
                     const bool ok = vb * a.Vh * a.Vw + vy * a.Vw + vx < a.Mv && vx < a.W && vy < a.H;
                     so[q] = ok ? (uint32_t)((vb * a.H + vy) * a.W + vx) * (uint32_t)a.N * 2u + (uint32_t)(n0 + 32 * NJ * wn + 8 * cl) * 2u : URSO_OOB_SHIFT;
-                    if (a.mask) mv[q] = buf_load16(rmk, so[q]);
+                    if (a.mask && !a.mbits) mv[q] = buf_load16(rmk, so[q]);
                     vx += RPI;
                     if (vx >= a.Vw) { vx -= a.Vw; if (++vy == a.Vh) { vy = 0; ++vb; } }
                 }
 #pragma unroll
                 for (int q = 0; q < NSI; ++q) {
-                    if (a.mask) {
-                        T ev[8], em[8];
-                        __builtin_memcpy(ev, &ov[q], 16); __builtin_memcpy(em, &mv[q], 16);
-#pragma unroll
-                        for (int e = 0; e < 8; ++e) ev[e] = (Elem<T>::to_f(em[e]) > 0.f) ? ev[e] : Elem<T>::from_f(0.f);
-                        __builtin_memcpy(&ov[q], ev, 16);
-                    }
+                    if (a.mask) ov[q] = a.mbits ? relu_bits_apply<T>(ov[q], relu_bits_byte(mbq[i * NSI + q], so[q])) : relu_mask_apply<T>(ov[q], mv[q]);
                     buf_store16(rds, so[q], ov[q]);
                 }
             }
@@ -346,7 +352,7 @@
     return 10 * HX2_SHAPES[best].mi + HX2_SHAPES[best].nj;
 }
 
-int urso_hconv2_try_launch(const urso_conv_geom* g, int dt, int relu, const void* src, const void* wgt, const float* bias, const void* mask,
+int urso_hconv2_try_launch(const urso_conv_geom* g, int dt, int relu, const void* src, const void* wgt, const float* bias, const void* mask, int mask_bits,
                            void* dst, uint32_t src_bytes, uint32_t wgt_bytes, uint32_t dst_bytes, void* ws, bool has_ws, hipStream_t st) {
     const int shape = urso_hconv2_pick(g, has_ws);
     if (!shape) return 0;
@@ -361,7 +367,7 @@
     a.R = 128 * mi + 2 * (a.Vw + 1); a.JA = ceil_div(a.R, 64); a.abuf = (int)hx2_abuf(a.R, nj);
     a.krow = 9 * g->C * 2;
     a.rcp_vw = 1.0f / (float)a.Vw; a.rcp_vh = 1.0f / (float)a.Vh;
-    a.relu = relu; a.dbg = g_urso_opt.hconv_dbg;
+    a.relu = relu; a.mbits = (mask && mask_bits) ? 1 : 0; a.dbg = g_urso_opt.hconv_dbg;
     a.clk = (ws && has_ws && (a.dbg & 2048)) ? (unsigned long long*)((char*)ws + 8192) : nullptr;
     const dim3 grid(urso_persistent_grid(a.ntiles, 1)), blk(512);
     urso_prof_l2((double)a.ntiles * a.nchunks * (9.0 * 64 * nj * 128 + (double)a.R * 128));
diff --git a/ursonet_amd/csrc/conv_igemm.hip b/ursonet_amd/csrc/conv_igemm.hip
--- a/ursonet_amd/csrc/conv_igemm.hip
+++ b/ursonet_amd/csrc/conv_igemm.hip
@@ -433,8 +433,19 @@
                               ws_d, ws_bytes, stream);
 }
 
+static int bits_native_3x3(const urso_conv_geom* g, int dt, int flags_nobits, bool has_halo_ws) {
+    if (dt != URSO_BF16 && dt != URSO_F16) return 0;
+    if (urso_c3_fits(g, dt, flags_nobits, nullptr)) return urso_c3_bits_ok(g) ? 1 : 0;
+    if (urso_hconv_fits(g, dt, flags_nobits, nullptr) && urso_hconv2_pick(g, has_halo_ws)) return 2;
+    return 0;
+}
+
 extern "C" int urso_conv_igemm_bits_ok(const urso_conv_geom* g, int dt, int flags, size_t ws_bytes) {
     if (!g || dt == URSO_F32 || (flags & URSO_EPI_OUT_F32) || (g->N % 8) || (g->C % 8)) return 0;
+    if ((flags & URSO_EPI_MASK_BITS) && g->KH == 3 && g->KW == 3) {
+        const int nat = (flags & URSO_EPI_EMIT_BITS) ? 0 : bits_native_3x3(g, dt, flags & ~URSO_EPI_MASK_BITS, true);
+        return nat == 2 ? 2 : ((nat == 1 && !(ws_bytes && urso_conv_igemm_ws_bytes(g, dt))) ? 1 : 0);
+    }
     if (ws_bytes && urso_conv_igemm_ws_bytes(g, dt)) return 0;
     return 1;
 }
@@ -502,7 +513,10 @@
         return urso_bneck_dgrad_launch(g, dt, flags, src_d, wgt_d, mask_d, dst_d, st);
     {
         const int use_pw = g_urso_opt.pw_kernel;
-        const bool halo_layer = dt != URSO_F32 && urso_hconv_fits(g, dt, flags, add_d);
+        const bool want_mb3 = (flags & URSO_EPI_MASK_BITS) && !(flags & (URSO_EPI_EMIT_BITS | URSO_EPI_OUT_F32)) && mask_d && !add_d && g->KH == 3;
+        const int mb3 = want_mb3 ? bits_native_3x3(g, dt, flags & ~URSO_EPI_MASK_BITS, ws_d && ws_bytes >= urso_hconv_ws_bytes()) : 0;
+        const int kflags = mb3 ? (flags & ~URSO_EPI_MASK_BITS) : flags;
+        const bool halo_layer = dt != URSO_F32 && urso_hconv_fits(g, dt, kflags, add_d);
         const bool split = ws_d && !halo_layer && urso_conv_igemm_ws_bytes(g, dt) != 0 && urso_conv_igemm_ws_bytes(g, dt) <= ws_bytes;
         const bool wants_bits = (flags & (URSO_EPI_MASK_BITS | URSO_EPI_EMIT_BITS)) != 0;
         const bool s1x1 = g->KH == 1 && g->KW == 1 && g->PH == 0 && g->PW == 0 && g->DH == 1 && g->DW == 1 && g->FH <= 0;
@@ -512,17 +526,17 @@
             urso_set_error("urso_conv_igemm: ADD_SRCGRID needs a 16-bit unpadded 1x1 layer with C %% 64 == 0, a residual operand on the input grid and no mask");
             return URSO_EINVAL;
         }
-        const bool bits_fit = !wants_bits || ((a.pointwise || (s1x1 && !(flags & URSO_EPI_MASK_BITS) && (a.Cc & 7) == 0)) && !((flags & URSO_EPI_EMIT_BITS) && (mask_d || (g->N % 32))) &&
+        const bool bits_fit = !wants_bits || mb3 || ((a.pointwise || (s1x1 && !(flags & URSO_EPI_MASK_BITS) && (a.Cc & 7) == 0)) && !((flags & URSO_EPI_EMIT_BITS) && (mask_d || (g->N % 32))) &&
                                               !((flags & URSO_EPI_MASK_BITS) && (!mask_d || (g->N % 32))) && !((flags & URSO_EPI_EMIT_BITS) && !bits_out_d));
         const bool fits = dt != URSO_F32 && !(flags & URSO_EPI_OUT_F32) && bits_fit && (g->N % 8) == 0 &&
                           !split && (size_t)a.M < (1u << 24);
         if (fits && urso_pair_single_fits(g, dt, flags, add_d, mask_d))
             return urso_pair_single_launch(g, dt, flags, src_d, wgt_d, bias_d, add_d, mask_d, dst_d,
                                            (flags & URSO_EPI_EMIT_BITS) ? bits_out_d : nullptr, st);
-        if (fits && urso_c3_fits(g, dt, flags, add_d))
-            return urso_c3_launch(g, dt, (flags & URSO_EPI_RELU) ? 1 : 0, src_d, wgt_d, bias_d, mask_d, dst_d, st);
-        if (fits && urso_hconv_fits(g, dt, flags, add_d))
-            return urso_hconv_launch(g, dt, (flags & URSO_EPI_RELU) ? 1 : 0, src_d, wgt_d, bias_d, add_d, mask_d, dst_d,
+        if (fits && (!(flags & URSO_EPI_MASK_BITS) || mb3 == 1) && urso_c3_fits(g, dt, kflags, add_d))
+            return urso_c3_launch(g, dt, (flags & URSO_EPI_RELU) ? 1 : 0, src_d, wgt_d, bias_d, mask_d, mb3 == 1, dst_d, st);
+        if (fits && urso_hconv_fits(g, dt, kflags, add_d))
+            return urso_hconv_launch(g, dt, (flags & URSO_EPI_RELU) ? 1 : 0, src_d, wgt_d, bias_d, add_d, mask_d, mb3 == 2, dst_d,
                                      a.src_bytes, a.wgt_bytes, a.dst_bytes, ws_d, ws_bytes, st);
         const int mbits = (flags & URSO_EPI_MASK_BITS) ? 1 : 0;
         void* bout = (flags & URSO_EPI_EMIT_BITS) ? bits_out_d : nullptr;
diff --git a/ursonet_amd/csrc/conv_pair.hip b/ursonet_amd/csrc/conv_pair.hip
--- a/ursonet_amd/csrc/conv_pair.hip
+++ b/ursonet_amd/csrc/conv_pair.hip
@@ -4,6 +4,7 @@
 struct PairArgs {
     const void* src; const void* w1; const float* bias1; const void* add; void* bits; void* mid;
     const void* w2; const float* bias2; const void* mask2; void* dst;
+    void* bits2;
     uint32_t nar_bytes, wide_bytes, bits_bytes;
     int ntiles;
     int relu1;
@@ -30,12 +31,13 @@
 #ifndef PAIR_DBG
 #define PAIR_DBG 0
 #endif
-template <typename T, int MODE, bool EMIT, typename S, int VAR, bool SPARSE = false>
+template <typename T, int MODE, bool EMIT, typename S, int VAR, bool SPARSE = false, bool EMIT2 = false>
 __global__ __launch_bounds__(S::NW * 64, 2) void pair_kernel(const PairArgs a) {
     static_assert(!SPARSE || (MODE == 1 && VAR == 0) || (MODE == 0 && VAR != 0), "SPARSE: compact add operand of the backward pair, or sampled second output of a single forward layer");
     constexpr bool SPADD = SPARSE && MODE == 1, CMPW = SPARSE && MODE == 0;
     static_assert(sizeof(T) == 2, "16-bit element types only");
     constexpr bool G2 = VAR == 0, HAS_ADD = VAR != 2;
+    static_assert(!EMIT2 || (G2 && MODE == 0 && !SPARSE), "EMIT2: the forward pair");
     static_assert(!G2 || (S::CM / S::NW == 16 && S::CW == 4 * S::CM), "pair: every wave owns 16 of the CM output channels of GEMM 2");
     static_assert(VAR != 2 || MODE == 0, "the form without a residual operand is forward-only");
     constexpr int BM = S::BM, CM = S::CM, CW = S::CW, NW = S::NW, AROW = S::AROW, RROW = S::RROW, BROW = S::BROW;
@@ -57,6 +59,7 @@
     const __amdgpu_buffer_rsrc_t rmid = make_rsrc((char*)a.mid + gwide, a.wide_bytes - gwide), rdst = make_rsrc(a.dst, a.nar_bytes);
     const __amdgpu_buffer_rsrc_t rbit = make_rsrc(a.bits ? (char*)a.bits + gbits : (char*)a.mid, a.bits ? a.bits_bytes - gbits : 0u);
     const __amdgpu_buffer_rsrc_t rmk2 = make_rsrc(MODE == 1 ? a.mask2 : a.dst, MODE == 1 ? a.nar_bytes : 0u);
+    const __amdgpu_buffer_rsrc_t rbit2 = make_rsrc(EMIT2 ? a.bits2 : a.dst, EMIT2 ? a.nar_bytes / 16u : 0u);
 
     uint32_t aoff[NA], roff[NR];
 #pragma unroll
@@ -147,7 +150,7 @@
     }
     const uint32_t bitoff = (uint32_t)l31 * bpitch + 4u * C2T * wave;
 
-    constexpr int NST = NR + (G2 ? NA : 0) + ((MODE == 0 && EMIT) ? PT1 : 0) + (CMPW ? NR : 0);
+    constexpr int NST = NR + (G2 ? NA : 0) + ((MODE == 0 && EMIT) ? PT1 : 0) + (CMPW ? NR : 0) + (EMIT2 ? NA : 0);
 
     i32x2_t pbits[PT1];
     i32x4_t pm2[NA];
@@ -325,6 +328,7 @@
                     __builtin_memcpy(&v, x, 16);
                 }
                 buf_store16(rdst, nb + aoff[i], v);
+                if constexpr (EMIT2) relu_bits_store(rbit2, nb + aoff[i], relu_bits8<T>(v), lane);
             }
         }
         if (!has_next) break;
@@ -348,10 +352,12 @@
             else URSO_KLAUNCH((pair_kernel<_Float16, 1, false, S, 0, true>), grid, blk, 0, st, a);
         } else if (dt == URSO_BF16) {
             if (mode == 1) URSO_KLAUNCH((pair_kernel<__bf16, 1, false, S, 0>), grid, blk, 0, st, a);
+            else if (emit && a.bits2) URSO_KLAUNCH((pair_kernel<__bf16, 0, true, S, 0, false, true>), grid, blk, 0, st, a);
             else if (emit) URSO_KLAUNCH((pair_kernel<__bf16, 0, true, S, 0>), grid, blk, 0, st, a);
             else URSO_KLAUNCH((pair_kernel<__bf16, 0, false, S, 0>), grid, blk, 0, st, a);
         } else {
             if (mode == 1) URSO_KLAUNCH((pair_kernel<_Float16, 1, false, S, 0>), grid, blk, 0, st, a);
+            else if (emit && a.bits2) URSO_KLAUNCH((pair_kernel<_Float16, 0, true, S, 0, false, true>), grid, blk, 0, st, a);
             else if (emit) URSO_KLAUNCH((pair_kernel<_Float16, 0, true, S, 0>), grid, blk, 0, st, a);
             else URSO_KLAUNCH((pair_kernel<_Float16, 0, false, S, 0>), grid, blk, 0, st, a);
         }
@@ -395,7 +401,7 @@
     const int mode = (flags & URSO_EPI_MASK_BITS) ? 1 : 0;
     PairArgs a;
     a.src = src; a.w1 = wgt; a.bias1 = bias; a.add = add ? add : dst; a.bits = mode ? const_cast<void*>(mask_bits) : bits_out; a.mid = dst;
-    a.w2 = nullptr; a.bias2 = nullptr; a.mask2 = nullptr; a.dst = dst; a.relu1 = (flags & URSO_EPI_RELU) ? 1 : 0;
+    a.w2 = nullptr; a.bias2 = nullptr; a.mask2 = nullptr; a.dst = dst; a.bits2 = nullptr; a.relu1 = (flags & URSO_EPI_RELU) ? 1 : 0;
     a.sp_h = a.sp_w = 0; a.add_bytes = 0; a.rcp_hw = a.rcp_w = 0.f;
     a.nar_bytes = (uint32_t)(M * cm * 2); a.wide_bytes = (uint32_t)(M * cw * 2); a.bits_bytes = (uint32_t)(M * (cw / 8));
     a.wide_pitch = (uint32_t)cw * 2u; a.bits_pitch = (uint32_t)cw / 8u; a.g_w1 = a.g_bias = a.g_wide = a.g_bits = 0;
@@ -447,6 +453,8 @@
 extern "C" int urso_conv_pair(long long M, int c_narrow, int dt, int mode, const void* src_d, const void* w1_d, const float* bias1_d,
                               const void* add_d, void* bits_d, void* mid_d, const void* w2_d, const float* bias2_d, const void* mask2_d,
                               void* dst_d, int add_h, int add_w, void* stream) {
+    void* dst_bits_d = mode == 0 ? const_cast<void*>(mask2_d) : nullptr;
+    if (dst_bits_d && !bits_d) { urso_set_error("urso_conv_pair: the bit mask of dst (mode 0, mask2_d) is written beside that of mid: bits_d is missing"); return URSO_EINVAL; }
     const int cm = c_narrow, cw = 4 * c_narrow;
     if (!urso_conv_pair_ok(M, dt, cm, cw)) {
         urso_set_error("urso_conv_pair: needs 16-bit dt, (64, 256) channels with M %% 64 == 0 or (128, 512) with M %% 32 == 0, tensors < 2 GiB");
@@ -464,13 +472,13 @@
     hipStream_t st = (hipStream_t)stream;
     PairArgs a;
     a.src = src_d; a.w1 = w1_d; a.bias1 = bias1_d; a.add = add_d; a.bits = bits_d; a.mid = mid_d; a.w2 = w2_d; a.bias2 = bias2_d;
-    a.mask2 = mask2_d; a.dst = dst_d; a.relu1 = 1;
+    a.mask2 = mode == 1 ? mask2_d : nullptr; a.dst = dst_d; a.bits2 = dst_bits_d; a.relu1 = 1;
     a.sp_h = add_h; a.sp_w = add_w; a.add_bytes = (uint32_t)(M / 4 * cw * 2);
     a.wide_pitch = (uint32_t)cw * 2u; a.bits_pitch = (uint32_t)cw / 8u; a.g_w1 = a.g_bias = a.g_wide = a.g_bits = 0;
     a.rcp_hw = sparse ? 1.0f / (float)(add_h * add_w) : 0.f; a.rcp_w = sparse ? 1.0f / (float)add_w : 0.f;
     a.nar_bytes = (uint32_t)(M * cm * 2); a.wide_bytes = (uint32_t)(M * cw * 2); a.bits_bytes = (uint32_t)(M * (cw / 8));
     const double flops = 2.0 * (double)M * cm * cw * 2.0;
-    const double bytes = (double)M * (2.0 * cm * 2 + (sparse ? 1.25 : 2.0) * cw * 2) + (double)M * (cw / 8) * ((mode == 1 || bits_d) ? 1 : 0) +
+    const double bytes = (double)M * (2.0 * cm * 2 + (sparse ? 1.25 : 2.0) * cw * 2) + (double)M * (cw / 8) * ((mode == 1 || bits_d) ? 1 : 0) + (dst_bits_d ? (double)M * (cm / 8) : 0.0) +
                          (mode == 1 ? (double)M * cm * 2 : 0.0) + 2.0 * cm * cw * 2;
     ProfScope ps(st, URSO_K_IGEMM, flops, bytes);
     if (cm == PairS2::CM) { a.ntiles = (int)(M / PairS2::BM); pr_launch<PairS2, 0>(a, dt, mode, bits_d != nullptr, 2, st, sparse); }
diff --git a/ursonet_amd/csrc/conv_pwx.hip b/ursonet_amd/csrc/conv_pwx.hip
--- a/ursonet_amd/csrc/conv_pwx.hip
+++ b/ursonet_amd/csrc/conv_pwx.hip
@@ -297,7 +297,8 @@
     const bool emit = bits_out != nullptr;
     const int form = (!add && !maskk && !emit) ? 0 : (add && !maskk && emit) ? 1 : (!add && maskk == 1 && !emit) ? 2 :
                      (add && maskk == 2 && !emit) ? 3 : (!add && maskk == 2 && !emit) ? 4 : (add && !maskk && !emit) ? 5 :
-                     (seg2 && !add && !maskk && emit) ? 6 : -1;
+                     (seg2 && !add && !maskk && emit) ? 6 :
+                     (!seg2 && !add && !maskk && emit) ? 7 : -1;
     if (form < 0 || (g->C % 64) || (g->N % 8)) return 0;
     if (seg2 && form != 0 && form != 4 && form != 6) return 0;
     if (emit && (g->N % 32)) return 0;
@@ -327,7 +328,7 @@
 #define URSO_PX(TT, BN_, NST_, AD_, MK_, EM_) URSO_KLAUNCH((pwx_kernel<TT, 5, BN_, NST_, AD_, MK_, EM_>), grid, blk, 0, st, a)
 #define URSO_PXF(TT, BN_, NST_) switch (form) { case 0: URSO_PX(TT, BN_, NST_, false, 0, false); break; case 1: URSO_PX(TT, BN_, NST_, true, 0, true); break; \
                                                 case 2: URSO_PX(TT, BN_, NST_, false, 1, false); break; case 3: URSO_PX(TT, BN_, NST_, true, 2, false); break; \
-                                                case 4: URSO_PX(TT, BN_, NST_, false, 2, false); break; default: URSO_PX(TT, BN_, NST_, true, 0, false); }
+                                                case 4: URSO_PX(TT, BN_, NST_, false, 2, false); break; case 7: URSO_PX(TT, BN_, NST_, false, 0, true); break; default: URSO_PX(TT, BN_, NST_, true, 0, false); }
 #define URSO_PX2(TT, BN_, NST_) do { if (form == 4) URSO_KLAUNCH((pwx_kernel<TT, 5, BN_, NST_, false, 2, false, true>), grid, blk, 0, st, a); \
                                      else if (form == 6) URSO_KLAUNCH((pwx_kernel<TT, 5, BN_, NST_, false, 0, true, true>), grid, blk, 0, st, a); \
                                      else URSO_KLAUNCH((pwx_kernel<TT, 5, BN_, NST_, false, 0, false, true>), grid, blk, 0, st, a); } while (0)
diff --git a/ursonet_amd/csrc/internal.h b/ursonet_amd/csrc/internal.h
--- a/ursonet_amd/csrc/internal.h
+++ b/ursonet_amd/csrc/internal.h
@@ -13,15 +13,16 @@
 bool urso_stem_fits(const urso_conv_geom* g, int dt, int flags, const void* add, const void* mask);
 int urso_stem_launch(const urso_conv_geom* g, int dt, int relu, const void* src, const void* wgt, const float* bias, void* dst, hipStream_t st);
 bool urso_c3_fits(const urso_conv_geom* g, int dt, int flags, const void* add);
-int urso_c3_launch(const urso_conv_geom* g, int dt, int relu, const void* src, const void* wgt, const float* bias, const void* mask,
+bool urso_c3_bits_ok(const urso_conv_geom* g);
+int urso_c3_launch(const urso_conv_geom* g, int dt, int relu, const void* src, const void* wgt, const float* bias, const void* mask, int mask_bits,
                    void* dst, hipStream_t st);
 bool urso_hconv_fits(const urso_conv_geom* g, int dt, int flags, const void* add);
 int urso_hconv_launch(const urso_conv_geom* g, int dt, int relu, const void* src, const void* wgt, const float* bias, const void* add,
-                      const void* mask, void* dst, uint32_t src_bytes, uint32_t wgt_bytes, uint32_t dst_bytes, void* ws, size_t ws_bytes,
+                      const void* mask, int mask_bits, void* dst, uint32_t src_bytes, uint32_t wgt_bytes, uint32_t dst_bytes, void* ws, size_t ws_bytes,
                       hipStream_t st);
 size_t urso_hconv_ws_bytes();
 int urso_hconv2_pick(const urso_conv_geom* g, bool has_ws);
-int urso_hconv2_try_launch(const urso_conv_geom* g, int dt, int relu, const void* src, const void* wgt, const float* bias, const void* mask,
+int urso_hconv2_try_launch(const urso_conv_geom* g, int dt, int relu, const void* src, const void* wgt, const float* bias, const void* mask, int mask_bits,
                            void* dst, uint32_t src_bytes, uint32_t wgt_bytes, uint32_t dst_bytes, void* ws, bool has_ws, hipStream_t st);
 bool urso_bneck_fwd_fits(const urso_conv_geom* g, int dt, int flags, const void* add, const void* mask);
 int urso_bneck_fwd_launch(const urso_conv_geom* g, int dt, int flags, const void* src, const void* wgt, const float* bias, void* dst, hipStream_t st);
diff --git a/ursonet_amd/csrc/lds_mfma.h b/ursonet_amd/csrc/lds_mfma.h
--- a/ursonet_amd/csrc/lds_mfma.h
+++ b/ursonet_amd/csrc/lds_mfma.h
@@ -47,6 +47,43 @@
     return __builtin_bit_cast(i32x2_t, __builtin_amdgcn_ds_read_tr16_b64_v4i16((__attribute__((address_space(3))) s16x4_t*)p));
 }
 
+template <typename T> __device__ __forceinline__ uint32_t relu_bits8(const i32x4_t& v) {
+    T x[8];
+    __builtin_memcpy(x, &v, 16);
+    uint32_t b = 0;
+#pragma unroll
+    for (int e = 0; e < 8; ++e) b |= (Elem<T>::to_f(x[e]) > 0.f ? 1u : 0u) << e;
+    return b;
+}
+template <typename T> __device__ __forceinline__ i32x4_t relu_bits_apply(const i32x4_t& v, uint32_t byte) {
+    T x[8];
+    __builtin_memcpy(x, &v, 16);
+#pragma unroll
+    for (int e = 0; e < 8; ++e) x[e] = ((byte >> e) & 1u) ? x[e] : Elem<T>::from_f(0.f);
+    i32x4_t r;
+    __builtin_memcpy(&r, x, 16);
+    return r;
+}
+template <typename T> __device__ __forceinline__ i32x4_t relu_mask_apply(const i32x4_t& v, const i32x4_t& m) {
+    T x[8], y[8];
+    __builtin_memcpy(x, &v, 16); __builtin_memcpy(y, &m, 16);
+#pragma unroll
+    for (int e = 0; e < 8; ++e) x[e] = Elem<T>::to_f(y[e]) > 0.f ? x[e] : Elem<T>::from_f(0.f);
+    i32x4_t r;
+    __builtin_memcpy(&r, x, 16);
+    return r;
+}
+__device__ __forceinline__ uint32_t relu_bits_load(__amdgpu_buffer_rsrc_t rbits, uint32_t off) {
+    return __builtin_amdgcn_raw_buffer_load_b32(rbits, (off >> 4) & ~3u, 0, 0);
+}
+__device__ __forceinline__ uint32_t relu_bits_byte(uint32_t dword, uint32_t off) { return (dword >> (8u * ((off >> 4) & 3u))) & 0xFFu; }
+__device__ __forceinline__ void relu_bits_store(__amdgpu_buffer_rsrc_t rbits, uint32_t off, uint32_t byte, int lane) {
+    int x = (int)(byte << (8u * ((off >> 4) & 3u)));
+    x |= __builtin_amdgcn_mov_dpp(x, 0xB1, 0xF, 0xF, true);
+    x |= __builtin_amdgcn_mov_dpp(x, 0x4E, 0xF, 0xF, true);
+    __builtin_amdgcn_raw_buffer_store_b32(x, rbits, (lane & 3) ? URSO_OOB_SHIFT : ((off >> 4) & ~3u), 0, 0);
+}
+
 __device__ __forceinline__ uint32_t halo_rd(int row, int h) {
     const int s = (row >> 1) & 7;
     return (uint32_t)(row * 128 + ((s >> 1) << 5) + ((h ^ (s & 1)) << 4));
diff --git a/ursonet_amd/engine.py b/ursonet_amd/engine.py
--- a/ursonet_amd/engine.py
+++ b/ursonet_amd/engine.py
@@ -676,6 +676,7 @@
         dstg = X.grad_buf()
         mask = (X.bits if X.bits is not None else X.data) if X.spec.relu else None
         mflag = hip.EPI_MASK_BITS if (X.spec.relu and X.bits is not None) else 0
+        assert not (mflag and node.kh == 3 and add is not None), "a 3x3 data gradient with a bit mask takes no residual gradient (%s)" % node.name
         if lvl_n is not None and mflag == 0 and not c.gd_scatter and self._dense_multi_ok(c):
             q.add_dense_dgrad(dict(names=(node.name,), level=lvl_n, src0=G, wgt0=c.wd, K0=c.npad, N=node.cin, M=B, add=add, mask=mask, dst=dstg, flags=0))
             X.grad_written, X.pending = True, None
@@ -687,7 +688,7 @@
                 raise AssertionError("scattered dgrad into %s needs an in-place accumulate" % node.name)
         self._emit_dgrad(lambda c=c, G=G, add=add, mask=mask, dstg=dstg, mflag=mflag:
                          hip.conv_igemm_ex(c.gd, dt, mflag, G, c.wd, None, add, mask, dstg, None,
-                                           self.halo_ws if (c.halo_d and add is None and not mflag) else (self.igemm_ws if c.ws_d else None)), (node.name,))
+                                           self.halo_ws if (c.halo_d and add is None and (not mflag or c.node.kh == 3)) else (self.igemm_ws if c.ws_d else None)), (node.name,))
         X.grad_written, X.pending = True, None
 
     def _emit_dgrad(self, run, dgrad, wgrad=()):
@@ -975,6 +976,37 @@
                 continue
             if all(hip.conv_igemm_bits_ok(c.gd, dt, 0, c.ws_d) for c in cons):
                 X.bits = torch.empty(X.numel // 8, dtype=torch.uint8, device=self.device)
+        self.inblock_bits = []
+        if hip.get_option("inblock_bits") & 1:
+            self._plan_needed_gradients()
+            for X in self.acts.values():
+                if X.bits is None and self._inblock_a2a_bits_ok(X):
+                    X.bits = torch.empty(X.numel // 8, dtype=torch.uint8, device=self.device)
+                    self.inblock_bits.append([c for c in self.convs.values() if c.dst is X][0].name)
+
+    def _inblock_a2a_bits_ok(self, X):
+        dt = self.dt
+        if dt == hip.F32 or not X.spec.relu or X.numel % 8 or X.compact is not None:
+            return False
+        prod = [c for c in self.convs.values() if c.dst is X]
+        cons = [c for c in self.convs.values() if c.src is X]
+        if len(prod) != 1 or len(cons) != 1:
+            return False
+        P, c = prod[0], cons[0]
+        n = c.node
+        if (P.batch_bn or c.batch_bn or P.res is not None or not P.node.relu or P.node.dense or P.node.out_f32 or P.N % 32 or P.npad != P.N or
+                P.node.kh != 1 or P.node.kw != 1 or P.gf.SH != 1 or P.gf.SW != 1 or P.fwd is None):
+            return False
+        if c.gd is None or n.dense or n.kh != 3 or n.kw != 3 or n.stride != 1 or c.gd_scatter or not self.grad_needed[X.spec.id]:
+            return False
+        kern = hip.conv_igemm_bits_native(c.gd, dt, c.ws_d)
+        if not kern or (kern == 2 and not hip.get_option("inblock_bits") & 4):
+            return False
+        A = self.pair_first.get(P.node.name)
+        if A is not None:
+            return A.dst.bits is not None and P.fwd is A.fwd and A.name + "+" + P.name == P.fwd.label[len("fwd:"):]
+        return (P.fwd.kind == "fwd" and P.fwd.computes_only(P) and not getattr(P, "winograd", False) and
+                hip.conv_igemm_bits_ok(P.gf, dt, P.fwd_flags, P.ws_f))
 
     def _upload_param_table(self):
         self.pbatch = hip.ParamBatch(self._descs, self.device) if self._descs else None
@@ -1249,7 +1281,7 @@
                 self.shortcut_folded.append(Sc.name)
             else:
                 A.fwd.run = (lambda A=A, Bc=Bc: hip.conv_pair(A.Mpix, A.node.cin, dt, 0, A.src.data, A.wf, A.biasf, A.res.data, A.dst.bits,
-                                                             A.dst.data, Bc.wf, Bc.biasf, None, Bc.dst.data))
+                                                             A.dst.data, Bc.wf, Bc.biasf, None, Bc.dst.data, dst_bits=Bc.dst.bits))
                 self._share_forward(A, Bc)
             self.pair_first[b_node.name] = A
 
@@ -1317,7 +1349,7 @@
             op()
 
     PLAN_OPTIONS = ("cus", "wgrad_blocks", "wgrad_narrow", "wgrad_big", "hwgrad", "grid_cap", "pair", "stem", "stem_pool", "c3", "bneck", "dense",
-                    "pwx")
+                    "pwx", "inblock_bits")
 
     def check_cleared_once(self):
         bad = []
diff --git a/ursonet_amd/hip.py b/ursonet_amd/hip.py
--- a/ursonet_amd/hip.py
+++ b/ursonet_amd/hip.py
@@ -425,6 +425,10 @@
     return int(_lib.urso_conv_igemm_halo2_shape(C.byref(g), dt, flags, int(bool(has_add)), int(bool(has_ws))))
 
 
+def conv_igemm_bits_native(g, dt, ws_bytes=0):
+    return int(_lib.urso_conv_igemm_bits_ok(C.byref(g), dt, EPI_MASK_BITS, ws_bytes)) if g.KH == 3 else 0
+
+
 def conv_igemm_ex(g, dt, flags, src, wgt, bias, add, mask, dst, bits_out=None, ws=None, stream=None):
     _chk(_lib.urso_conv_igemm_ex(C.byref(g), dt, flags, ptr(src), ptr(wgt), ptr(bias), ptr(add), ptr(mask), ptr(dst), ptr(bits_out),
                                  ptr(ws), (ws.numel() * ws.element_size()) if ws is not None else 0, stream_ptr(stream)), "urso_conv_igemm_ex")
@@ -891,8 +895,12 @@
     return bool(_lib.urso_conv_pair_ok(int(M), dt, int(c_narrow), int(c_wide)))
 
 
-def conv_pair(M, c_narrow, dt, mode, src, w1, bias1, add, bits, mid, w2, bias2, mask2, dst, add_hw=None, stream=None):
+def conv_pair(M, c_narrow, dt, mode, src, w1, bias1, add, bits, mid, w2, bias2, mask2, dst, add_hw=None, stream=None, dst_bits=None):
     ah, aw = add_hw if add_hw else (0, 0)
+    if dst_bits is not None:
+        if mode != 0 or mask2 is not None:
+            raise ValueError("conv_pair: dst_bits belongs to the forward form, which takes no mask2")
+        mask2 = dst_bits
     _chk(_lib.urso_conv_pair(int(M), int(c_narrow), dt, int(mode), ptr(src), ptr(w1), ptr(bias1), ptr(add), ptr(bits), ptr(mid), ptr(w2), ptr(bias2),
                              ptr(mask2), ptr(dst), int(ah), int(aw), stream_ptr(stream)), "urso_conv_pair")
 
```

New measurement: 4679 images/sec (median of 3 runs). Within noise of the previous version (+0.1%).
